# lmb-freiburg/flownet2

Measured on AMD Instinct MI355X. Metric: image-pairs/sec FlowNetC forward at 448x320, higher is better.
Workload: dtype f32

## Files before the change

### flownet2_amd/_lib.py

```python
from __future__ import annotations

import ctypes as C
import os
import re

_HERE = os.path.dirname(os.path.abspath(__file__))
SO_PATH = os.path.join(_HERE, "libflownet2_hip.so")
INCLUDE_DIR = os.path.join(_HERE, "..", "include")

_SCALARS = {"int": C.c_int, "unsigned": C.c_uint, "float": C.c_float, "size_t": C.c_size_t, "long long": C.c_longlong, "unsigned long long": C.c_ulonglong,
            "char": C.c_char}
_POINTERS = {"float": C.c_void_p, "double": C.c_void_p, "void": C.c_void_p, "unsigned char": C.c_void_p, "char": C.c_char_p, "int": C.POINTER(C.c_int),
             "unsigned": C.POINTER(C.c_uint), "size_t": C.POINTER(C.c_size_t)}
_STRUCT_NAMES = {"fn2_l1loss_params": "L1LossParams", "fn2_l1loss_scale": "L1LossScale"}
_DECLARATOR = re.compile(r"^([\w\s*]*?)(\w+)\s*(?:\[(\d+)\])?$")
_FUNCTION = re.compile(r"^([\w\s*]+?)\b(fn2_\w+)\s*\(([^()]*)\)$")


class Fn2Error(RuntimeError):

    def __init__(self, status: int, message: str):
        super().__init__(f"[fn2 status {status}] {message}")
        self.status = status


def _ctype(spec, structs, where):
    words = [w for w in spec.replace("*", " ").split() if w != "const"]
    base, stars = " ".join(words), spec.count("*")
    if stars == 0 and base in _SCALARS:
        return _SCALARS[base]
    if stars == 1 and base in structs:
        return C.POINTER(structs[base])
    if stars == 1 and base in _POINTERS:
        return _POINTERS[base]
    if stars == 2 and base in ("float", "void"):
        return C.POINTER(C.c_void_p)
    raise ValueError(f"C header: unknown type `{spec.strip()}` in `{where}`")


def _declarator(text, structs, where):
    m = _DECLARATOR.match(text.strip())
    if not m or not m.group(1).strip():
        raise ValueError(f"C header: cannot read `{text.strip()}` in `{where}`")
    t = _ctype(m.group(1), structs, where)
    return m.group(2), (t * int(m.group(3)) if m.group(3) else t), m.group(1)


def parse_header(text, structs=None):
    structs = dict(structs or {})
    functions, constants = {}, {}
    text = re.sub(r"/\*.*?\*/", " ", text, flags=re.S)
    for name, value in re.findall(r"^[ \t]*#[ \t]*define[ \t]+(FN2_\w+)[ \t]+(-?(?:0[xX][0-9a-fA-F]+|\d+))[ \t]*$", text, flags=re.M):
        constants[name] = int(value, 0)
    text = re.sub(r"^[ \t]*#.*$", " ", text, flags=re.M)

    def enum(m):
        value = -1
        for item in filter(None, (s.strip() for s in m.group(1).split(","))):
            name, _, v = (s.strip() for s in item.partition("="))
            value = int(v, 0) if v else value + 1
            constants[name] = value
        return " "
    text = re.sub(r"(?:typedef\s+)?enum\s*\w*\s*\{([^{}]*)\}\s*\w*\s*;", enum, text)

    def struct(m):
        cname, fields = m.group(1), []
        for decl in filter(None, (s.strip() for s in m.group(2).split(";"))):
            first, *more = decl.split(",")
            name, t, spec = _declarator(first, structs, "struct " + cname)
            fields.append((name, t))
            fields += [_declarator(spec + " " + other, structs, "struct " + cname)[:2] for other in more]
        pyname = _STRUCT_NAMES.get(cname) or "".join(w.capitalize() for w in cname.split("_")[1:])
        structs[cname] = type(pyname, (C.Structure,), {"_fields_": fields, "__doc__": cname, "__module__": __name__})
        return " "
    text = re.sub(r"typedef\s+struct\s+(fn2_\w+)\s*\{([^{}]*)\}\s*\w+\s*;", struct, text)

    text = re.sub(r'extern\s*"C"\s*\{|\}', " ", text)
    for stmt in filter(None, (" ".join(s.split()) for s in text.split(";"))):
        m = _FUNCTION.match(stmt)
        if not m:
            raise ValueError(f"C header: cannot read the declaration `{stmt}`")
        params = m.group(3).strip()
        args = [] if params == "void" else [_declarator(p, structs, stmt)[1] for p in params.split(",")]
        functions[m.group(2)] = (_ctype(m.group(1), structs, stmt), args)
    return functions, structs, constants


def _parse_headers():
    per_header, structs, constants = [], {}, {}
    own = {"flownet2_hip_flow_metrics.h": {}, "flownet2_hip_flow_consistency.h": {}, "flownet2_hip_flow_visualize.h": {},
           "flownet2_hip_flow_track.h": {}}
    for h in ("flownet2_hip.h", "flownet2_hip_solver.h", "flownet2_hip_corr_route.h", "flownet2_hip_conv_general.h",
              "flownet2_hip_conv_geometry.h", "flownet2_hip_conv_volume.h", "flownet2_hip_lpq_loss.h", "flownet2_hip_flow_metrics.h",
              "flownet2_hip_flow_consistency.h", "flownet2_hip_flow_visualize.h", "flownet2_hip_flow_track.h"):
        with open(os.path.join(INCLUDE_DIR, h)) as f:
            functions, structs, c = parse_header(f.read(), structs)
        per_header.append(functions)
        own.get(h, constants).update(c)
    return (per_header, structs, constants, own["flownet2_hip_flow_metrics.h"], own["flownet2_hip_flow_consistency.h"],
            own["flownet2_hip_flow_visualize.h"], own["flownet2_hip_flow_track.h"])


(_PER_HEADER, _STRUCTS, CONSTANTS, FLOW_METRICS_CONSTANTS, FLOW_CONSISTENCY_CONSTANTS, FLOW_VISUALIZE_CONSTANTS,
 FLOW_TRACK_CONSTANTS) = _parse_headers()
(EXPORTS, SOLVER_EXPORTS, CORR_ROUTE_EXPORTS, CONV_GENERAL_EXPORTS, CONV_GEOMETRY_EXPORTS, CONV_VOLUME_EXPORTS, LPQ_LOSS_EXPORTS,
 FLOW_METRICS_EXPORTS, FLOW_CONSISTENCY_EXPORTS, FLOW_VISUALIZE_EXPORTS, FLOW_TRACK_EXPORTS) = (list(f) for f in _PER_HEADER)
PROTOTYPES = {name: proto for f in _PER_HEADER[:8] for name, proto in f.items()}
FLOW_CONSISTENCY_PROTOTYPES = dict(_PER_HEADER[8])
FLOW_VISUALIZE_PROTOTYPES = dict(_PER_HEADER[9])
FLOW_TRACK_PROTOTYPES = dict(_PER_HEADER[10])
globals().update({cls.__name__: cls for cls in _STRUCTS.values()})
_HOOKS = parse_header("""
    int fn2_debug_set_correlation_impl(int impl);
    int fn2_debug_correlation_units_plan(int N, int H, int W, int policy, unsigned* out_words, int max_words);
    int fn2_debug_set_resample_generic(int on);
    int fn2_debug_set_correlation_trace(void* device_buffer);""")[0]

_lib = None


def lib():
    global _lib
    if _lib is not None:
        return _lib
    if not os.path.exists(SO_PATH):
        raise RuntimeError(
            f"{SO_PATH} not found: the HIP extension is not built. Run `python -m flownet2_amd.build` "
            "(or __graft_entry__.build()). flownet2_amd has no CPU / PyTorch fallback.")
    L = C.CDLL(SO_PATH)
    for table, required in ((PROTOTYPES, True), (FLOW_CONSISTENCY_PROTOTYPES, True), (FLOW_VISUALIZE_PROTOTYPES, True),
                            (FLOW_TRACK_PROTOTYPES, True), (_HOOKS, False)):
        for name, (restype, argtypes) in table.items():
            if not hasattr(L, name):
                if required:
                    raise RuntimeError(f"{SO_PATH} does not export {name}")
                continue
            fn = getattr(L, name)
            fn.restype, fn.argtypes = restype, argtypes
    _lib = L
    return L


def check(status: int):
    if status != 0:
        raise Fn2Error(status, lib().fn2_last_error_string().decode())


def version() -> str:
    return lib().fn2_version().decode()
```

### flownet2_amd/csrc/conv_mfma.hip

```cpp
#include "mfma_tile.hpp"

namespace fn2 {
namespace cv {

using namespace mfma;

struct Args {
  const float* in; const float* wp; const float* bias; float* out;
  int N, Cin, Hin, Win, in_ctot, in_c0;
  int Cout, Hout, Wout, out_ctot, out_c0;
  int pad;
  int nchunks;
  int ksteps;
  int tx, ty;
  int ng;
  unsigned total;
  unsigned nbig;
  float slope; int relu;
};

template <int KS_, int S_, int MW_, int NP_, int WM_, int WNX_, int WNY_, int CQ_, int P16_ = 0, int PIN_ = 0>
struct Cfg : Window<((P16_ ? 1 : 4) * WNY_ - 1) * S_ + KS_,
                    ((P16_ ? 16 : 4) * NP_ * WNX_ - 1) * S_ + KS_ + 4,
                    CQ_, WM_ * WNX_ * WNY_> {
  static constexpr int KS = KS_, S = S_, MW = MW_, NP = NP_, WM = WM_, WNX = WNX_, WNY = WNY_, CQ = CQ_, P16 = P16_;
  static constexpr int PIN = PIN_;
  static constexpr int NW = WM * WNX * WNY, THREADS = 64 * NW;
  static constexpr int PADL = 4;
  static constexpr int TW = (P16 ? 16 : 4) * NP * WNX, TH = (P16 ? 1 : 4) * WNY;
  static_assert(!P16 || (KS == 1 && S == 1), "row tiles are for 1x1 kernels");
  static_assert(Cfg::WR == (TH - 1) * S + KS && Cfg::WC == (TW - 1) * S + KS + PADL, "window of the tile");
  static constexpr int KSC = CQ * KS * KS;
  static constexpr int NBUFA = ring_depth(KSC);
  static_assert(KSC % NBUFA == 0, "ring phase must repeat per chunk");
  static_assert(2 * Cfg::BUF * 4 <= 160 * 1024, "LDS");
};

template <class K>
__device__ __forceinline__ void conv_body(const Args& a, int g, int bx, int by, int n) {
  static_assert(K::THREADS == 256, "launch bounds");
  extern __shared__ __attribute__((aligned(16))) float smem[];
  constexpr int KS = K::KS, S = K::S, MW = K::MW, NP = K::NP;
  const int tid = threadIdx.x, lane = tid & 63;
  const int wave = __builtin_amdgcn_readfirstlane(tid >> 6);
  const int wm = wave % K::WM, wnx = (wave / K::WM) % K::WNX, wny = wave / (K::WM * K::WNX);
  const int x0 = bx * K::TW, y0 = by * K::TH;

  const size_t plane = (size_t)a.Hin * a.Win;
  const __amdgpu_buffer_rsrc_t rs = nchw_rsrc(a.in, n, a.in_ctot, a.in_c0, a.Cin, plane);
  unsigned voff[K::RPW];
  window_plan<K>(voff, wave, lane, S * y0 - a.pad, S * x0 - K::PADL, a.Hin, a.Win, plane);
  const unsigned lds_base = (unsigned)(uintptr_t)(lds_ptr_t)smem;
  const unsigned chunk_bytes = 4u * 4u * K::CQ * (unsigned)plane;
  auto stage = [&](int chunk, int buf) { stage_chunk<K>(rs, voff, lds_base + 4u * (unsigned)(buf * K::BUF), wave, (unsigned)chunk * chunk_bytes); };

  const int kq = lane >> 4, p16 = lane & 15, py = K::P16 ? 0 : p16 >> 2, px = K::P16 ? p16 : p16 & 3;
  constexpr int PW = K::P16 ? 16 : 4, PH = K::P16 ? 1 : 4;
  const int bbase = kq * K::CS + (S * (PH * wny + py)) * K::RS + S * (PW * NP * wnx + px) + K::PADL - a.pad;
  using WV = typename WVec<MW>::T;
  const int cg0 = (g * K::WM + wm) * MW;
  const float* wb = a.wp + (size_t)(cg0 / 4) * a.ksteps * 256 + (cg0 % 4);
  const unsigned wlane = 16u * (unsigned)lane;

  f32x4 acc[MW][NP];
#pragma unroll
  for (int j = 0; j < MW; ++j)
#pragma unroll
    for (int p = 0; p < NP; ++p) acc[j][p] = f32x4{0.f, 0.f, 0.f, 0.f};

  constexpr int R = K::NBUFA - 1, DMA = K::NRUN / K::NW;
  static_assert(R + DMA <= 63, "vmcnt has 6 bits");
  WV wreg[K::NBUFA];
  stage(0, 0);
  if (a.nchunks > 0) {
#pragma unroll
    for (int i = 0; i < R; ++i) wreg[i] = weight_fetch<MW>(wb + (size_t)i * 256, wlane);
  }
  auto weight_step = [&](int ks0, int ks, int rest) -> WV {
    const float* wks = wb + (size_t)(ks0 + ks + R) * 256;
    if (ks + R < K::KSC) wreg[(ks + R) % K::NBUFA] = weight_fetch<MW>(wks, wlane);
    else wreg[(ks + R) % K::NBUFA] = weight_fetch_unless_last<MW>(rest, wks, wlane);
    const int left = K::KSC - 1 - ks < R ? K::KSC - 1 - ks : R;
    if (ks < R) ring_wait_either(rest, left, R + DMA);
    else if (left < R) ring_wait_either(rest, left, R);
    else ring_wait(R);
    weight_landed(wreg[ks % K::NBUFA]);
    return wreg[ks % K::NBUFA];
  };

  for (int c = 0; c < a.nchunks; ++c) {
    const int buf = c & 1;
    const int rest = a.nchunks - 1 - c;
    wait_vmcnt<R>();
    __builtin_amdgcn_s_barrier();
    if (rest) stage(c + 1, buf ^ 1);
    const float* win = smem + buf * K::BUF + bbase;
    const int ks0 = c * K::KSC;
    if constexpr (K::PIN) {
      float b[2][NP];
      auto tap_off = [](int ks) { const int cq = ks / (KS * KS), ky = (ks / KS) % KS, kx = ks % KS; return cq * 4 * K::CS + ky * K::RS + kx; };
#pragma unroll
      for (int p = 0; p < NP; ++p) b[0][p] = win[tap_off(0) + PW * S * p];
      __builtin_amdgcn_sched_barrier(0);
#pragma unroll
      for (int ks = 0; ks < K::KSC; ++ks) {
        const WV w = weight_step(ks0, ks, rest);
#pragma unroll
        for (int p = 0; p < NP; ++p) {
#pragma unroll
          for (int j = 0; j < MW; ++j) acc[j][p] = __builtin_amdgcn_mfma_f32_16x16x4f32(b[ks & 1][p], wget<MW>(w, j), acc[j][p], 0, 0, 0);
          if (ks + 1 < K::KSC) b[(ks + 1) & 1][p] = win[tap_off(ks + 1 < K::KSC ? ks + 1 : ks) + PW * S * p];
          __builtin_amdgcn_sched_barrier(0);
        }
      }
    } else {
#pragma unroll
    for (int ks = 0; ks < K::KSC; ++ks) {
      const WV w = weight_step(ks0, ks, rest);
      const int cq = ks / (KS * KS), ky = (ks / KS) % KS, kx = ks % KS;
      float b[NP];
#pragma unroll
      for (int p = 0; p < NP; ++p) b[p] = win[cq * 4 * K::CS + ky * K::RS + kx + PW * S * p];
#pragma unroll
      for (int j = 0; j < MW; ++j)
#pragma unroll
        for (int p = 0; p < NP; ++p) acc[j][p] = __builtin_amdgcn_mfma_f32_16x16x4f32(b[p], wget<MW>(w, j), acc[j][p], 0, 0, 0);
    }
    }
  }

  wait_vmcnt<0>();
  const int y = K::P16 ? y0 + wny : y0 + 4 * wny + (lane >> 4);
  if (y < a.Hout) {
#pragma unroll
    for (int j = 0; j < MW; ++j) {
      const int co = 16 * (cg0 + j) + (lane & 15);
      const float bv = a.bias ? a.bias[co] : 0.f;
      float* orow = a.out + (((size_t)n * a.out_ctot + a.out_c0 + co) * a.Hout + y) * a.Wout;
#pragma unroll
      for (int p = 0; p < NP; ++p) {
        const int x = K::P16 ? x0 + 16 * (NP * wnx + p) + 4 * (lane >> 4) : x0 + 4 * (NP * wnx + p);
        store_row4(orow, x, a.Wout, acc[j][p], bv, a.relu, a.slope);
      }
    }
  }
}

__device__ __forceinline__ void decode_tile(const Args& a, unsigned t, int& g, int& bx, int& by, int& n) {
  g = t % a.ng; t /= a.ng;
  bx = t % a.tx; t /= a.tx;
  by = t % a.ty;
  n = t / a.ty;
}

template <class K>
__global__ void __launch_bounds__(256, 2)
conv_mfma(Args a) {
  unsigned t;
  if (!xcd_task(blockIdx.x, a.total, t)) return;
  int g, bx, by, n;
  decode_tile(a, t, g, bx, by, n);
  conv_body<K>(a, g, bx, by, n);
}

template <class K>
__global__ void __launch_bounds__(256, 2)
conv_mfma_tail(Args a) {
  using KH = Cfg<K::KS, K::S, K::MW / 2, K::NP, K::WM, K::WNX, K::WNY, K::CQ, K::P16>;
  int g, bx, by, n;
  if (blockIdx.x < a.nbig) {
    const unsigned t = (blockIdx.x % 8) * (a.nbig / 8) + blockIdx.x / 8;
    decode_tile(a, t, g, bx, by, n);
    conv_body<K>(a, g, bx, by, n);
  } else {
    unsigned u;
    if (!xcd_task(blockIdx.x - a.nbig, 2 * (a.total - a.nbig), u)) return;
    decode_tile(a, a.nbig + u / 2, g, bx, by, n);
    conv_body<KH>(a, 2 * g + (int)(u & 1), bx, by, n);
  }
}

__global__ void pack_weights(const float* __restrict__ w, float* __restrict__ wp, int Cout, int Cin, int KS, int ksteps, int kalloc) {
  const long long total = (long long)((Cout + 63) / 64) * kalloc * 256;
  for (long long i = blockIdx.x * (long long)blockDim.x + threadIdx.x; i < total; i += (long long)gridDim.x * blockDim.x) {
    const int j = (int)(i & 3), lane = (int)((i >> 2) & 63);
    long long r = i >> 8;
    const int ks = (int)(r % kalloc), grp = (int)(r / kalloc);
    const int co = 64 * grp + 16 * j + (lane & 15), kq = lane >> 4;
    const int cq = ks / (KS * KS), tap = ks % (KS * KS);
    const int ci = 4 * cq + kq;
    float v = 0.f;
    if (ks < ksteps && ci < Cin && co < Cout) v = w[((size_t)co * Cin + ci) * KS * KS + tap];
    wp[i] = v;
  }
}

template <int KS> struct PackTile {
  static constexpr int T = KS * KS;
  static constexpr int QT = KS == 1 ? 8 : KS == 3 ? 3 : KS == 4 ? 2 : 1;
  static constexpr int CIL = 4 * QT, ROW = CIL * T + 1;
  static constexpr int LDS_FLOATS = 64 * ROW;
};

template <int KS, int ORDER>
__global__ void __launch_bounds__(256) pack_weights_view(const float* __restrict__ w, float* __restrict__ wp, int ksteps, int kalloc,
                                                         int src_co, int src_ci, long long s_co, long long s_ci, int flip) {
  using P = PackTile<KS>;
  constexpr int T = P::T, QT = P::QT, CIL = P::CIL, ROW = P::ROW;
  __shared__ float tile[P::LDS_FLOATS];
  const int grp = blockIdx.x, cq0 = blockIdx.y * QT;
  const int co0 = 64 * grp, ci0 = 4 * cq0;
  const int nquads = ksteps / T;
  constexpr int TOTAL = 64 * CIL * T;
  if constexpr (ORDER == 0) {
    const float* src = w + (size_t)co0 * s_co + (size_t)ci0 * T;
#pragma unroll
    for (int i = threadIdx.x; i < TOTAL; i += 256) {
      const int col = i / (CIL * T), e = i - col * (CIL * T), c = e / T;
      tile[col * ROW + e] = (co0 + col < src_co && ci0 + c < src_ci) ? src[(size_t)col * s_co + e] : 0.f;
    }
  } else if constexpr (ORDER == 1) {
    const float* src = w + (size_t)ci0 * s_ci + (size_t)co0 * T;
#pragma unroll
    for (int i = threadIdx.x; i < TOTAL; i += 256) {
      const int c = i / (64 * T), e = i - c * (64 * T), col = e / T, t = e - col * T;
      tile[col * ROW + c * T + t] = (co0 + col < src_co && ci0 + c < src_ci) ? src[(size_t)c * s_ci + e] : 0.f;
    }
  } else {
#pragma unroll
    for (int i = threadIdx.x; i < TOTAL; i += 256) {
      const int col = i / (CIL * T), e = i - col * (CIL * T), c = e / T, t = e - c * T;
      tile[col * ROW + e] = (co0 + col < src_co && ci0 + c < src_ci) ? w[(size_t)(co0 + col) * s_co + (size_t)(ci0 + c) * s_ci + t] : 0.f;
    }
  }
  __syncthreads();
  const int nq = min(QT, nquads - cq0);
  float* dst = wp + ((size_t)grp * kalloc + (size_t)cq0 * T) * 256;
  const int j = threadIdx.x & 3, lane = threadIdx.x >> 2;
  const float* trow = tile + (16 * j + (lane & 15)) * ROW + (lane >> 4) * T;
#pragma unroll
  for (int ks = 0; ks < QT * T; ++ks) {
    const int cq = ks / T, tap = ks - cq * T;
    if (cq < nq) dst[ks * 256 + threadIdx.x] = trow[4 * cq * T + (flip ? T - 1 - tap : tap)];
  }
  if (cq0 + QT >= nquads)
    for (int i = threadIdx.x; i < (kalloc - ksteps) * 256; i += 256) wp[((size_t)grp * kalloc + ksteps) * 256 + i] = 0.f;
}

template <int KS>
static void launch_pack_view(const float* w, float* wp, int Cout, int ksteps, int kalloc, int src_co, int src_ci, long long s_co, long long s_ci, int flip,
                             hipStream_t st) {
  using P = PackTile<KS>;
  const dim3 grid((unsigned)((Cout + 63) / 64), (unsigned)cdiv(ksteps / P::T, P::QT));
  if (s_ci == (long long)P::T) hipLaunchKernelGGL((pack_weights_view<KS, 0>), grid, dim3(256), 0, st, w, wp, ksteps, kalloc, src_co, src_ci, s_co, s_ci, flip);
  else if (s_co == (long long)P::T) hipLaunchKernelGGL((pack_weights_view<KS, 1>), grid, dim3(256), 0, st, w, wp, ksteps, kalloc, src_co, src_ci, s_co, s_ci, flip);
  else hipLaunchKernelGGL((pack_weights_view<KS, 2>), grid, dim3(256), 0, st, w, wp, ksteps, kalloc, src_co, src_ci, s_co, s_ci, flip);
}

constexpr int kSpare = 8;
constexpr int kChunkQuads = 2;

inline int chunk_quads(int KS) { return KS == 1 ? 8 : kChunkQuads; }
inline int ksteps_for(int Cin, int KS) { return cdiv(cdiv(Cin, 4), chunk_quads(KS)) * chunk_quads(KS) * KS * KS; }

template <class K>
static void set_geometry(Args& a) {
  if constexpr (K::P16) {
    a.Win *= a.Hin; a.Hin = 1; a.Wout *= a.Hout; a.Hout = 1;
  }
  a.tx = cdiv(a.Wout, K::TW); a.ty = cdiv(a.Hout, K::TH);
  a.ng = a.Cout / (16 * K::MW * K::WM);
  a.nchunks = cdiv(cdiv(a.Cin, 4), K::CQ);
}

inline long long tiles_of(const Args& a) { return (long long)a.N * a.tx * a.ty * a.ng; }

template <class K>
static int launch(const Args& base, hipStream_t st) {
  Args a = base;
  set_geometry<K>(a);
  a.nbig = (unsigned)tiles_of(a);
  return launch_tiles<&conv_mfma<K>>(a, tiles_of(a), K::THREADS, (int)(sizeof(float) * 2 * K::BUF), "conv_mfma", "conv_mfma_forward", st);
}

inline unsigned whole_rounds(long long tiles) { return (unsigned)(tiles / 256 * 256); }

template <class K>
static int launch_tail(const Args& base, hipStream_t st) {
  if constexpr (K::MW < 2) {
    return fail(FN2_ERR_UNSUPPORTED, "conv_mfma: variant has no split tail");
  } else {
    Args a = base;
    set_geometry<K>(a);
    if (tiles_of(a) > 0x1fffff00ll) return fail(FN2_ERR_UNSUPPORTED, "conv_mfma: grid too large");
    a.total = (unsigned)tiles_of(a); a.nbig = whole_rounds(a.total);
    const unsigned nsm = 2 * (a.total - a.nbig);
    const unsigned grid = a.nbig + 8 * ((nsm + 7) / 8);
    constexpr size_t lds = sizeof(float) * 2 * K::BUF;
    set_dynamic_lds_once<&conv_mfma_tail<K>>((int)lds);
    hipLaunchKernelGGL((conv_mfma_tail<K>), dim3(grid), dim3(K::THREADS), lds, st, a);
    return check_launch("conv_mfma_forward");
  }
}

struct Variant {
  int ks, s, mw, np, wm, wnx, wny, p16;
  int (*fn)(const Args&, hipStream_t);
  int (*fn_tail)(const Args&, hipStream_t);
};

#define FN2_CV_LIST(X) \
   \
  X(1, 1, 2, 7, 2, 2, 1, 8, 1) X(1, 1, 2, 7, 2, 1, 2, 8, 1) X(1, 1, 4, 7, 1, 2, 2, 8, 0) X(1, 1, 4, 7, 1, 1, 4, 8, 0) X(1, 1, 2, 6, 2, 2, 1, 8, 1) \
  X(1, 1, 2, 4, 2, 2, 1, 8, 1) X(1, 1, 2, 7, 1, 2, 2, 8, 0) X(1, 1, 2, 7, 1, 4, 1, 8, 0) X(1, 1, 2, 4, 1, 2, 2, 8, 0) X(1, 1, 4, 4, 1, 2, 2, 8, 0) \
   \
  X(3, 1, 2, 7, 2, 2, 1, 2, 1) X(3, 1, 2, 7, 2, 1, 2, 2, 1) X(3, 1, 4, 7, 1, 2, 2, 2, 0) X(3, 1, 4, 7, 1, 1, 4, 2, 0) \
  X(3, 1, 2, 6, 2, 2, 1, 2, 1) X(3, 1, 4, 6, 1, 2, 2, 2, 0) X(3, 1, 4, 4, 1, 2, 2, 2, 0) X(3, 1, 2, 4, 2, 2, 1, 2, 1) \
   \
  X(3, 2, 2, 7, 2, 1, 2, 2, 1) X(3, 2, 4, 7, 1, 1, 4, 2, 0) X(3, 2, 2, 6, 2, 2, 1, 2, 1) X(3, 2, 4, 6, 1, 2, 2, 2, 0) X(3, 2, 2, 4, 2, 2, 1, 2, 1) \
   \
  X(4, 2, 2, 7, 2, 2, 1, 2, 1) X(4, 2, 2, 7, 2, 1, 2, 2, 1) X(4, 2, 4, 7, 1, 2, 2, 2, 0) X(4, 2, 2, 6, 2, 2, 1, 2, 1) X(4, 2, 4, 4, 1, 2, 2, 2, 0) X(4, 2, 2, 4, 2, 2, 1, 2, 1) \
   \
  X(5, 2, 2, 7, 2, 2, 1, 1, 1) X(5, 2, 2, 7, 2, 1, 2, 1, 1) X(5, 2, 4, 7, 1, 2, 2, 1, 0) X(5, 2, 4, 7, 1, 1, 4, 1, 0) \
  X(5, 2, 2, 6, 2, 2, 1, 1, 1) X(5, 2, 4, 6, 1, 2, 2, 1, 0) X(5, 2, 4, 4, 1, 2, 2, 1, 0) \
   \
  X(7, 2, 2, 6, 2, 2, 1, 1, 1) X(7, 2, 2, 7, 2, 2, 1, 1, 1) X(7, 2, 4, 4, 1, 2, 2, 1, 0) X(7, 2, 4, 6, 1, 2, 2, 1, 0) X(7, 2, 2, 4, 2, 2, 1, 1, 1)

template <class K, int TAIL> struct TailFn { static constexpr int (*fn)(const Args&, hipStream_t) = nullptr; };
template <class K> struct TailFn<K, 1> { static constexpr int (*fn)(const Args&, hipStream_t) = &launch_tail<K>; };

#define FN2_CV_ROW(KS, S, MW, NP, WM, WNX, WNY, CQ, TAIL) \
  {KS, S, MW, NP, WM, WNX, WNY, 0, &launch<Cfg<KS, S, MW, NP, WM, WNX, WNY, CQ>>, TailFn<Cfg<KS, S, MW, NP, WM, WNX, WNY, CQ>, TAIL>::fn},
#define FN2_CV_ROW16(MW, NP, WM, WNX, WNY, TAIL) \
  {1, 1, MW, NP, WM, WNX, WNY, 1, &launch<Cfg<1, 1, MW, NP, WM, WNX, WNY, 8, 1>>, TailFn<Cfg<1, 1, MW, NP, WM, WNX, WNY, 8, 1>, TAIL>::fn},
#define FN2_CV_PIN(KS, S, MW, NP, WM, WNX, WNY, CQ, P16, TAIL) \
  {KS, S, MW, NP, WM, WNX, WNY, P16, &launch<Cfg<KS, S, MW, NP, WM, WNX, WNY, CQ, P16, 1>>, TailFn<Cfg<KS, S, MW, NP, WM, WNX, WNY, CQ, P16, 1>, TAIL>::fn},
static const Variant kVariants[] = {FN2_CV_LIST(FN2_CV_ROW)
  FN2_CV_ROW16(2, 7, 2, 2, 1, 1) FN2_CV_ROW16(2, 7, 4, 1, 1, 1) FN2_CV_ROW16(4, 7, 1, 4, 1, 0) FN2_CV_ROW16(4, 7, 2, 2, 1, 0) FN2_CV_ROW16(2, 5, 2, 2, 1, 1)
  FN2_CV_ROW16(2, 4, 2, 2, 1, 1) FN2_CV_ROW16(2, 7, 1, 4, 1, 0) FN2_CV_ROW16(2, 5, 1, 4, 1, 0) FN2_CV_ROW16(4, 5, 1, 4, 1, 0) FN2_CV_ROW16(2, 4, 1, 4, 1, 0)
  FN2_CV_ROW16(4, 5, 2, 2, 1, 0) FN2_CV_ROW16(4, 4, 2, 2, 1, 0)
  FN2_CV_ROW16(2, 9, 4, 1, 1, 1) FN2_CV_ROW16(2, 9, 2, 2, 1, 1) FN2_CV_ROW16(2, 3, 2, 2, 1, 1) FN2_CV_ROW16(4, 3, 1, 4, 1, 0)
  FN2_CV_ROW16(4, 9, 4, 1, 1, 0) FN2_CV_ROW16(4, 9, 2, 2, 1, 0) FN2_CV_ROW16(4, 7, 4, 1, 1, 0)
  FN2_CV_PIN(5, 2, 2, 7, 2, 2, 1, 1, 0, 1) FN2_CV_PIN(5, 2, 2, 7, 2, 1, 2, 1, 0, 1)
  FN2_CV_PIN(1, 1, 4, 9, 4, 1, 1, 8, 1, 0) FN2_CV_PIN(1, 1, 2, 9, 4, 1, 1, 8, 1, 1) FN2_CV_PIN(1, 1, 2, 5, 2, 2, 1, 8, 1, 1) FN2_CV_PIN(1, 1, 4, 7, 4, 1, 1, 8, 1, 0)
  FN2_CV_PIN(1, 1, 2, 7, 2, 2, 1, 8, 1, 1) FN2_CV_PIN(1, 1, 2, 3, 2, 2, 1, 8, 1, 1)
  FN2_CV_PIN(3, 1, 2, 7, 2, 2, 1, 2, 0, 1) FN2_CV_PIN(3, 1, 2, 6, 2, 2, 1, 2, 0, 1) FN2_CV_PIN(3, 2, 2, 7, 2, 1, 2, 2, 0, 1) FN2_CV_PIN(3, 2, 2, 6, 2, 2, 1, 2, 0, 1)
  FN2_CV_PIN(4, 2, 2, 7, 2, 2, 1, 2, 0, 1) FN2_CV_PIN(4, 2, 2, 6, 2, 2, 1, 2, 0, 1) FN2_CV_PIN(5, 2, 2, 6, 2, 2, 1, 1, 0, 1)
  FN2_CV_PIN(7, 2, 2, 6, 2, 2, 1, 1, 0, 1) FN2_CV_PIN(7, 2, 4, 6, 1, 2, 2, 1, 0, 0)};
constexpr int kNumVariants = sizeof(kVariants) / sizeof(kVariants[0]);

int g_forced_variant = -1;

static double variant_cost(const Variant& v, const Args& a, bool tail) {
  const int tw = (v.p16 ? 16 : 4) * v.np * v.wnx, th = (v.p16 ? 1 : 4) * v.wny;
  const long long wgs = v.p16 ? (long long)a.N * cdiv(a.Wout * a.Hout, tw) * (a.Cout / (16 * v.mw * v.wm))
                              : (long long)a.N * cdiv(a.Wout, tw) * cdiv(a.Hout, th) * (a.Cout / (16 * v.mw * v.wm));
  double rounds = (double)((wgs + 255) / 256);
  if (tail) {
    const long long r = wgs % 256;
    if (wgs < 256 || r == 0 || r > 128) return 1e30;
    rounds = (double)(wgs / 256) + 0.5 * 1.12;
  }
  const double eff = 1.0 / (1.0 + 0.08 * (4.0 / v.mw - 1.0) + 0.02 * (7.0 / v.np - 1.0));
  return rounds * v.mw * v.np / eff;
}

static bool variant_applies(const Variant& v, const Args& a, int KS, int S) {
  if (!v.p16 && a.Win % 4 != 0) return false;
  return v.ks == KS && v.s == S && a.Cout % (16 * v.mw * v.wm) == 0;
}

}
}

using namespace fn2;

FN2_API size_t fn2_conv_mfma_packed_floats(int Cout, int Cin, int kernel) {
  if (Cout <= 0 || Cout % 32 != 0 || Cin <= 0 || kernel <= 0) return 0;
  return (size_t)((Cout + 63) / 64) * (cv::ksteps_for(Cin, kernel) + cv::kSpare) * 256;
}

FN2_API int fn2_conv_mfma_pack_weights_view(const float* weight, float* packed, int Cout, int Cin, int kernel, int src_cout, int src_cin,
                                            long long stride_cout, long long stride_cin, int flip, void* stream);

FN2_API int fn2_conv_mfma_pack_weights(const float* weight, float* packed, int Cout, int Cin, int kernel, void* stream) {
  if (!weight || !packed) return fail(FN2_ERR_INVALID_ARG, "conv_mfma_pack_weights: null blob");
  if (Cout <= 0 || Cout % 32 != 0 || Cin <= 0 || (kernel != 1 && kernel != 3 && kernel != 4 && kernel != 5 && kernel != 7))
    return fail(FN2_ERR_UNSUPPORTED, "conv_mfma_pack_weights: needs Cout %% 32 == 0 and kernel_size 1, 3, 4, 5 or 7 (got Cout %d, kernel %d)", Cout, kernel);
  return fn2_conv_mfma_pack_weights_view(weight, packed, Cout, Cin, kernel, Cout, Cin, (long long)Cin * kernel * kernel, (long long)kernel * kernel, 0, stream);
}

FN2_API int fn2_conv_mfma_pack_weights_view(const float* weight, float* packed, int Cout, int Cin, int kernel, int src_cout, int src_cin,
                                            long long stride_cout, long long stride_cin, int flip, void* stream) {
  if (!weight || !packed) return fail(FN2_ERR_INVALID_ARG, "conv_mfma_pack_weights_view: null blob");
  if (Cout <= 0 || Cout % 32 != 0 || Cin <= 0 || (kernel != 1 && kernel != 3 && kernel != 4 && kernel != 5 && kernel != 7))
    return fail(FN2_ERR_UNSUPPORTED, "conv_mfma_pack_weights_view: needs Cout %% 32 == 0 and kernel_size 1, 3, 4, 5 or 7 (got Cout %d, kernel %d)", Cout, kernel);
  if (src_cout < 1 || src_cout > Cout || src_cin < 1 || src_cin > Cin || stride_cout < 1 || stride_cin < 1)
    return fail(FN2_ERR_INVALID_ARG, "conv_mfma_pack_weights_view: bad source view (%d of %d, %d of %d channels, strides %lld / %lld)", src_cout, Cout,
                src_cin, Cin, stride_cout, stride_cin);
  const int ksteps = cv::ksteps_for(Cin, kernel), kalloc = ksteps + cv::kSpare;
  hipStream_t st = as_stream(stream);
  switch (kernel) {
    case 1: cv::launch_pack_view<1>(weight, packed, Cout, ksteps, kalloc, src_cout, src_cin, stride_cout, stride_cin, flip ? 1 : 0, st); break;
    case 3: cv::launch_pack_view<3>(weight, packed, Cout, ksteps, kalloc, src_cout, src_cin, stride_cout, stride_cin, flip ? 1 : 0, st); break;
    case 4: cv::launch_pack_view<4>(weight, packed, Cout, ksteps, kalloc, src_cout, src_cin, stride_cout, stride_cin, flip ? 1 : 0, st); break;
    case 5: cv::launch_pack_view<5>(weight, packed, Cout, ksteps, kalloc, src_cout, src_cin, stride_cout, stride_cin, flip ? 1 : 0, st); break;
    default: cv::launch_pack_view<7>(weight, packed, Cout, ksteps, kalloc, src_cout, src_cin, stride_cout, stride_cin, flip ? 1 : 0, st); break;
  }
  return check_launch("conv_mfma_pack_weights_view");
}

FN2_API int fn2_conv_mfma_supported(int Cin, int Hin, int Win, int Cout, int kernel, int stride, int pad) {
  if (Cin <= 0 || Hin <= 0 || Win <= 0 || Cout <= 0 || Cout % 32 != 0) return 0;
  if (kernel == 1 ? ((long long)Hin * Win) % 4 != 0 : Win % 4 != 0) return 0;
  if (!((kernel == 1 && stride == 1) || (kernel == 3 && (stride == 1 || stride == 2)) || (kernel == 4 && stride == 2) || (kernel == 5 && stride == 2) || (kernel == 7 && stride == 2))) return 0;
  if (pad < 0 || pad > 4 || pad > kernel - 1) return 0;
  if ((long long)Cin * Hin * Win >= (1ll << 28)) return 0;
  const int Hout = (Hin + 2 * pad - kernel) / stride + 1, Wout = (Win + 2 * pad - kernel) / stride + 1;
  if (Hout < 1 || Wout < 1) return 0;
  cv::Args a{};
  a.Win = Win; a.Cout = Cout;
  for (int i = 0; i < cv::kNumVariants; ++i)
    if (cv::variant_applies(cv::kVariants[i], a, kernel, stride)) return 1;
  return 0;
}

FN2_API int fn2_debug_set_conv_variant(int v) { cv::g_forced_variant = v; return FN2_OK; }
FN2_API int fn2_conv_mfma_num_variants(void) { return cv::kNumVariants; }

FN2_API int fn2_conv_mfma_forward(const float* bottom, const float* packed_weight, const float* bias, float* top,
                                  int N, int Cin, int Hin, int Win, int bottom_channels, int bottom_c0,
                                  int Cout, int top_channels, int top_c0, int kernel, int stride, int pad,
                                  int relu, float negative_slope, void* stream) {
  if (N < 0) return fail(FN2_ERR_INVALID_ARG, "conv_mfma: bad batch");
  if (N == 0) return FN2_OK;
  if (const int rc = mfma::check_conv_args("conv_mfma", bottom, packed_weight, top, Cin, bottom_channels, bottom_c0, Cout, top_channels, top_c0, [&] {
        return fn2_conv_mfma_supported(Cin, Hin, Win, Cout, kernel, stride, pad) ? FN2_OK
            : fail(FN2_ERR_UNSUPPORTED, "conv_mfma: unsupported geometry (Cin %d, %dx%d, Cout %d, k %d s %d p %d)", Cin, Hin, Win, Cout, kernel, stride, pad);
      }))
    return rc;
  cv::Args a{};
  a.in = bottom; a.wp = packed_weight; a.bias = bias; a.out = top;
  a.N = N; a.Cin = Cin; a.Hin = Hin; a.Win = Win; a.in_ctot = bottom_channels; a.in_c0 = bottom_c0;
  a.Cout = Cout; a.Hout = (Hin + 2 * pad - kernel) / stride + 1; a.Wout = (Win + 2 * pad - kernel) / stride + 1;
  a.out_ctot = top_channels; a.out_c0 = top_c0; a.pad = pad;
  a.ksteps = cv::ksteps_for(Cin, kernel) + cv::kSpare;
  a.slope = negative_slope; a.relu = relu;
  hipStream_t st = as_stream(stream);
  static TuneCache cache("conv_mfma", cv::kNumVariants);
  const TuneKey key{N, Cin, Hin, Win, Cout, kernel, stride, pad, bottom_channels == Cin, top_channels == Cout};
  mfma::Pick p;
  if (const int rc = mfma::pick_variant(p, "conv_mfma", cv::g_forced_variant, cv::kNumVariants, true, cache, key, st,
                                        [&](int i) { return cv::variant_applies(cv::kVariants[i], a, kernel, stride); },
                                        [&](int i, bool tail) { return cv::variant_cost(cv::kVariants[i], a, tail); },
                                        [&](int i, bool tail) { return tail ? cv::kVariants[i].fn_tail(a, st) : cv::kVariants[i].fn(a, st); },
                                        [&](int i) { return cv::kVariants[i].fn_tail != nullptr; }))
    return rc;
  return p.tail ? cv::kVariants[p.variant].fn_tail(a, st) : cv::kVariants[p.variant].fn(a, st);
}
```

### flownet2_amd/csrc/flow_head.hip

```cpp
#include "fn2_common.hpp"

namespace fn2 {

constexpr int kHeadPix = 64;

template <int G>
__global__ void __launch_bounds__(kHeadPix* G) conv3x3_c2_taps(const float* __restrict__ in, const float* __restrict__ w,
                                                                float* __restrict__ P, int N, int C, int H, int W, int nsplit) {
  __shared__ float red[G][18][kHeadPix];
  const int lane_pix = threadIdx.x % kHeadPix;
  const int grp = __builtin_amdgcn_readfirstlane(threadIdx.x / kHeadPix);
  const size_t plane = (size_t)H * W;
  const long long total = (long long)N * H * W;
  const long long p = (long long)blockIdx.x * kHeadPix + lane_pix;
  const bool live = p < total;
  const int n = live ? (int)(p / (long long)plane) : 0;
  const unsigned pix = live ? (unsigned)(p - (long long)n * plane) : 0u;
  const float* src = in + (size_t)n * C * plane + pix;
  float a[18];
#pragma unroll
  for (int k = 0; k < 18; ++k) a[k] = 0.f;
  const int ngroups = G * nsplit;
  const int c_per = (C + ngroups - 1) / ngroups;
  const int c_lo = min(C, ((int)blockIdx.y * G + grp) * c_per), c_hi = min(C, c_lo + c_per);
  for (int c = c_lo; c < c_hi; c += 8) {
    float v[8];
#pragma unroll
    for (int cc = 0; cc < 8; ++cc) v[cc] = (c + cc < c_hi) ? src[(size_t)(c + cc) * plane] : 0.f;
    __builtin_amdgcn_sched_barrier(0);
#pragma unroll
    for (int cc = 0; cc < 8; ++cc) {
      if (c + cc < c_hi) {
        const float* w0 = w + (size_t)(c + cc) * 9;
        const float* w1 = w + ((size_t)C + c + cc) * 9;
#pragma unroll
        for (int t = 0; t < 9; ++t) {
          a[t] = fmaf(w0[t], v[cc], a[t]);
          a[9 + t] = fmaf(w1[t], v[cc], a[9 + t]);
        }
      }
    }
  }
#pragma unroll
  for (int k = 0; k < 18; ++k) red[grp][k][lane_pix] = a[k];
  __syncthreads();
  if (live) {
    float* dst = P + ((size_t)blockIdx.y * N + n) * 18 * plane + pix;
    for (int k = grp; k < 18; k += G) {
      float sacc = 0.f;
#pragma unroll
      for (int g = 0; g < G; ++g) sacc += red[g][k][lane_pix];
      dst[(size_t)k * plane] = sacc;
    }
  }
}

template <int NSPLIT>
__global__ void __launch_bounds__(256) conv3x3_c2_gather(const float* __restrict__ P, const float* __restrict__ bias,
                                                          float* __restrict__ out, int N, int H, int W) {
  const unsigned plane = (unsigned)H * W;
  const unsigned pix = blockIdx.x * 256u + threadIdx.x;
  if (pix >= plane) return;
  const int y = pix / W, x = pix - y * W;
  const unsigned no = blockIdx.y;
  const unsigned n = no >> 1, o = no & 1;
  float v[NSPLIT][9];
#pragma unroll
  for (int sp = 0; sp < NSPLIT; ++sp) {
    const float* Pn = P + (((size_t)sp * N + n) * 18 + o * 9) * plane;
#pragma unroll
    for (int dy = 0; dy < 3; ++dy)
#pragma unroll
      for (int dx = 0; dx < 3; ++dx) {
        const int yy = y + dy - 1, xx = x + dx - 1;
        const bool ok = yy >= 0 && yy < H && xx >= 0 && xx < W;
        v[sp][dy * 3 + dx] = ok ? Pn[(size_t)(dy * 3 + dx) * plane + (unsigned)yy * W + xx] : 0.f;
      }
  }
  float sacc = bias ? bias[o] : 0.f;
#pragma unroll
  for (int sp = 0; sp < NSPLIT; ++sp)
#pragma unroll
    for (int t = 0; t < 9; ++t) sacc += v[sp][t];
  out[(size_t)no * plane + pix] = sacc;
}

__global__ void __launch_bounds__(256) deconv4x4s2_c2(const float* __restrict__ in, const float* __restrict__ w,
                                                       const float* __restrict__ bias, float* __restrict__ out,
                                                       int N, int H, int W, int out_ctot, int out_c0) {
  const int Ho = 2 * H, Wo = 2 * W;
  const long long total = (long long)N * Ho * Wo;
  for (long long idx = blockIdx.x * (long long)blockDim.x + threadIdx.x; idx < total; idx += (long long)gridDim.x * blockDim.x) {
    const int X = (int)(idx % Wo), Y = (int)((idx / Wo) % Ho), n = (int)(idx / ((long long)Wo * Ho));
    float a0 = bias ? bias[0] : 0.f, a1 = bias ? bias[1] : 0.f;
#pragma unroll
    for (int ty = 0; ty < 2; ++ty) {
      const int ky = ((Y + 1) & 1) + 2 * ty;
      const int iy = (Y + 1 - ky) / 2;
      if (Y + 1 - ky < 0 || iy >= H) continue;
#pragma unroll
      for (int tx = 0; tx < 2; ++tx) {
        const int kx = ((X + 1) & 1) + 2 * tx;
        const int ix = (X + 1 - kx) / 2;
        if (X + 1 - kx < 0 || ix >= W) continue;
#pragma unroll
        for (int c = 0; c < 2; ++c) {
          const float v = in[(((size_t)n * 2 + c) * H + iy) * W + ix];
          a0 = fmaf(w[((c * 2 + 0) * 4 + ky) * 4 + kx], v, a0);
          a1 = fmaf(w[((c * 2 + 1) * 4 + ky) * 4 + kx], v, a1);
        }
      }
    }
    out[(((size_t)n * out_ctot + out_c0 + 0) * Ho + Y) * Wo + X] = a0;
    out[(((size_t)n * out_ctot + out_c0 + 1) * Ho + Y) * Wo + X] = a1;
  }
}

}

using namespace fn2;

constexpr int kHeadG = 16;

static int head_splits(int N, int C, int H, int W) {
  const long long blocks = ((long long)order_batch(N) * H * W + kHeadPix - 1) / kHeadPix;
  int nsplit = 1;
  while (nsplit < 8 && blocks * kHeadG * nsplit < 4096 && C >= 8 * kHeadG * nsplit * 2) nsplit *= 2;
  return nsplit;
}

FN2_API size_t fn2_predict_flow_conv_workspace_bytes(int N, int C, int H, int W) {
  if (N < 1 || C < 1 || H < 1 || W < 1) return 0;
  return sizeof(float) * (size_t)head_splits(N, C, H, W) * N * 18 * H * W;
}

FN2_API int fn2_predict_flow_conv_forward(const float* in, const float* weight, const float* bias, float* out,
                                          int N, int C, int H, int W, void* workspace, size_t workspace_bytes, void* stream) {
  if (N < 0 || C < 1 || H < 1 || W < 1) return fail(FN2_ERR_INVALID_ARG, "predict_flow_conv: bad shape [%d,%d,%d,%d]", N, C, H, W);
  if (N == 0) return FN2_OK;
  if (!in || !weight || !out) return fail(FN2_ERR_INVALID_ARG, "predict_flow_conv: NULL blob pointer");
  if ((long long)H * W >= (1ll << 31) || 2ll * N > 65535) return fail(FN2_ERR_UNSUPPORTED, "predict_flow_conv: blob too large");
  const size_t need = fn2_predict_flow_conv_workspace_bytes(N, C, H, W);
  if (!workspace || workspace_bytes < need) return fail(FN2_ERR_WORKSPACE, "predict_flow_conv: workspace too small (%zu < %zu)", workspace_bytes, need);
  const long long total = (long long)N * H * W;
  const unsigned blocks = (unsigned)((total + kHeadPix - 1) / kHeadPix);
  const int nsplit = head_splits(N, C, H, W);
  hipStream_t st = as_stream(stream);
  float* P = reinterpret_cast<float*>(workspace);
  hipLaunchKernelGGL(conv3x3_c2_taps<kHeadG>, dim3(blocks, nsplit), dim3(kHeadPix * kHeadG), 0, st, in, weight, P, N, C, H, W, nsplit);
  const dim3 g2(((unsigned)H * W + 255) / 256, 2 * N);
  switch (nsplit) {
    case 1: hipLaunchKernelGGL(conv3x3_c2_gather<1>, g2, dim3(256), 0, st, P, bias, out, N, H, W); break;
    case 2: hipLaunchKernelGGL(conv3x3_c2_gather<2>, g2, dim3(256), 0, st, P, bias, out, N, H, W); break;
    case 4: hipLaunchKernelGGL(conv3x3_c2_gather<4>, g2, dim3(256), 0, st, P, bias, out, N, H, W); break;
    default: hipLaunchKernelGGL(conv3x3_c2_gather<8>, g2, dim3(256), 0, st, P, bias, out, N, H, W); break;
  }
  return check_launch("predict_flow_conv_forward");
}

FN2_API int fn2_upsample_flow_deconv_forward(const float* in, const float* weight, const float* bias, float* out,
                                             int N, int H, int W, void* stream) {
  if (N < 0 || H < 1 || W < 1) return fail(FN2_ERR_INVALID_ARG, "upsample_flow_deconv: bad shape");
  if (N == 0) return FN2_OK;
  if (!in || !weight || !out) return fail(FN2_ERR_INVALID_ARG, "upsample_flow_deconv: NULL blob pointer");
  const long long total = (long long)N * 4 * H * W;
  hipLaunchKernelGGL(deconv4x4s2_c2, dim3(blocks_for(total, 256, 4096)), dim3(256), 0, as_stream(stream), in, weight, bias, out, N, H, W, 2, 0);
  return check_launch("upsample_flow_deconv_forward");
}

FN2_API int fn2_upsample_flow_deconv_forward_into(const float* in, const float* weight, const float* bias, float* top,
                                                  int N, int H, int W, int top_channels, int top_c0, void* stream) {
  if (N < 0 || H < 1 || W < 1) return fail(FN2_ERR_INVALID_ARG, "upsample_flow_deconv: bad shape");
  if (top_c0 < 0 || top_c0 + 2 > top_channels) return fail(FN2_ERR_INVALID_ARG, "upsample_flow_deconv: channel slice outside the blob");
  if (N == 0) return FN2_OK;
  if (!in || !weight || !top) return fail(FN2_ERR_INVALID_ARG, "upsample_flow_deconv: NULL blob pointer");
  const long long total = (long long)N * 4 * H * W;
  hipLaunchKernelGGL(deconv4x4s2_c2, dim3(blocks_for(total, 256, 4096)), dim3(256), 0, as_stream(stream), in, weight, bias, top, N, H, W, top_channels, top_c0);
  return check_launch("upsample_flow_deconv_forward_into");
}
```

### flownet2_amd/csrc/mfma_tile.hpp

```cpp
#pragma once

#include "autotune.hpp"
#include "fn2_common.hpp"

namespace fn2 {
namespace mfma {

using f32x4 = __attribute__((ext_vector_type(4))) float;
using f32x2 = __attribute__((ext_vector_type(2))) float;
using lds_ptr_t = __attribute__((address_space(3))) void*;

constexpr int cdiv(int a, int b) { return (a + b - 1) / b; }
constexpr int up_mod(int v, int r, int m) { return v + ((r - v % m) + m) % m; }

constexpr unsigned kOOB = 0x7ffffff0u;
constexpr int kRsrcWord3 = 0x00020000;

template <int N>
__device__ __forceinline__ void wait_vmcnt() {
  asm volatile("s_waitcnt vmcnt(%0)" ::"n"(N) : "memory");
}

__device__ __forceinline__ __amdgpu_buffer_rsrc_t nchw_rsrc(const float* blob, int n, int ctot, int c0, int C, size_t plane) {
  return __builtin_amdgcn_make_buffer_rsrc(const_cast<float*>(blob + ((size_t)n * ctot + c0) * plane), 0, (unsigned)(4u * C * plane), kRsrcWord3);
}

template <int MW> struct WVec;
template <> struct WVec<1> { using T = float; };
template <> struct WVec<2> { using T = f32x2; };
template <> struct WVec<4> { using T = f32x4; };

template <int MW>
__device__ __forceinline__ float wget(const typename WVec<MW>::T& v, int j) {
  if constexpr (MW == 1) return v; else return v[j];
}

template <int WR_, int WC_, int CQ_, int NW_>
struct Window {
  static constexpr int WR = WR_, WC = WC_;
  static constexpr int RS = up_mod(cdiv(WC, 4) * 4, 4, 16);
  static constexpr int CS = up_mod(WR * RS, 16, 32);
  static constexpr int SLOTS_C = CS / 4;
  static constexpr int SLOTS = 4 * CQ_ * SLOTS_C;
  static constexpr int NRUN = cdiv(SLOTS, 64);
  static constexpr int RPW = cdiv(NRUN, NW_);
  static constexpr int BUF = NRUN * 256;
};

constexpr int ring_depth(int KSC) { return (KSC % 6 == 0) ? 6 : (KSC % 5 == 0) ? 5 : (KSC % 7 == 0) ? 7 : (KSC % 4 == 0) ? 4 : 3; }

template <class K>
__device__ __forceinline__ void window_plan(unsigned (&voff)[K::RPW], int wave, int lane, int y_first, int x_first, int Hin, int Win, size_t plane) {
#pragma unroll
  for (int i = 0; i < K::RPW; ++i) {
    const int s = (i * K::NW + wave) * 64 + lane;
    voff[i] = kOOB;
    if (s < K::SLOTS) {
      const int c = s / K::SLOTS_C, rem = s % K::SLOTS_C;
      const int row = rem / (K::RS / 4), gq = rem % (K::RS / 4);
      const int yi = y_first + row, xi = x_first + 4 * gq;
      if (row < K::WR && 4 * gq < K::WC && yi >= 0 && yi < Hin && xi >= 0 && xi < Win)
        voff[i] = 4u * (unsigned)(c * plane + (size_t)yi * Win + xi);
    }
  }
}

template <class K>
__device__ __forceinline__ void stage_chunk(__amdgpu_buffer_rsrc_t rs, const unsigned (&voff)[K::RPW], unsigned dst, int wave, unsigned soff) {
#pragma unroll
  for (int i = 0; i < K::RPW; ++i) {
    const int r = i * K::NW + wave;
    if (r < K::NRUN)
      __builtin_amdgcn_raw_ptr_buffer_load_lds(rs, (lds_ptr_t)(uintptr_t)(dst + 1024u * (unsigned)r), 16, voff[i], soff, 0, 0);
  }
}

template <class K>
struct ChunkStage {
  const __amdgpu_buffer_rsrc_t& rs; const unsigned (&voff)[K::RPW]; const unsigned& chunk_bytes; const unsigned& dst; const int& wave;
  __device__ void operator()(int chunk) const {
    unsigned vc[K::RPW];
#pragma unroll
    for (int i = 0; i < K::RPW; ++i) vc[i] = voff[i] == kOOB ? kOOB : voff[i] + (unsigned)chunk * chunk_bytes;
    stage_chunk<K>(rs, vc, dst, wave, 0u);
  }
};

__device__ __forceinline__ const float* weight_lane(const float* wp, int cg0, int ksteps, int lane) {
  return wp + ((size_t)(cg0 / 4) * ksteps * 64 + lane) * 4 + (cg0 % 4);
}

template <int MW>
__device__ __forceinline__ typename WVec<MW>::T weight_load(const float* wl, int ks) {
  return *reinterpret_cast<const typename WVec<MW>::T*>(wl + (size_t)ks * 256);
}

template <int MW>
__device__ __forceinline__ typename WVec<MW>::T weight_fetch(const float* base, unsigned lane_bytes) {
  typename WVec<MW>::T w;
  if constexpr (MW == 1) asm volatile("global_load_dword %0, %1, %2" : "=v"(w) : "v"(lane_bytes), "s"(base));
  else if constexpr (MW == 2) asm volatile("global_load_dwordx2 %0, %1, %2" : "=v"(w) : "v"(lane_bytes), "s"(base));
  else asm volatile("global_load_dwordx4 %0, %1, %2" : "=v"(w) : "v"(lane_bytes), "s"(base));
  return w;
}

template <class T>
__device__ __forceinline__ void weight_landed(T& w) { asm volatile("" : "+v"(w)); }

constexpr int vmcnt_clamp(int n) { return n < 63 ? n : 63; }

__device__ __forceinline__ void ring_wait(int n) { asm volatile("s_waitcnt vmcnt(%0)" ::"i"(vmcnt_clamp(n))); }

__device__ __forceinline__ void ring_wait_either(int rest, int n_last, int n_else) {
  asm volatile(
      "s_cmp_eq_u32 %0, 0\n\t"
      "s_cbranch_scc1 .Lrwt_%=\n\t"
      "s_waitcnt vmcnt(%2)\n\t"
      "s_branch .Lrwe_%=\n"
      ".Lrwt_%=:\n\t"
      "s_waitcnt vmcnt(%1)\n"
      ".Lrwe_%=:"
      :
      : "s"(rest), "i"(vmcnt_clamp(n_last)), "i"(vmcnt_clamp(n_else))
      : "scc");
}

template <int MW>
__device__ __forceinline__ typename WVec<MW>::T weight_fetch_unless_last(int rest, const float* base, unsigned lane_bytes) {
  typename WVec<MW>::T w;
#define FN2_FETCH_UNLESS(INSN) \
  asm volatile("s_cmp_eq_u32 %3, 0\n\ts_cbranch_scc1 .Lwfs_%=\n\t" INSN " %0, %1, %2\n.Lwfs_%=:" : "=v"(w) : "v"(lane_bytes), "s"(base), "s"(rest) : "scc")
  if constexpr (MW == 1) FN2_FETCH_UNLESS("global_load_dword");
  else if constexpr (MW == 2) FN2_FETCH_UNLESS("global_load_dwordx2");
  else FN2_FETCH_UNLESS("global_load_dwordx4");
#undef FN2_FETCH_UNLESS
  return w;
}

__device__ __forceinline__ bool xcd_task(unsigned block, unsigned total, unsigned& task) {
  const unsigned per_xcd = (total + 7) / 8;
  task = (block % 8) * per_xcd + block / 8;
  return !(block / 8 >= per_xcd || task >= total);
}

__device__ __forceinline__ f32x4 bias_relu4(f32x4 v, float bias, int relu, float slope) {
#pragma unroll
  for (int r = 0; r < 4; ++r) {
    float s = v[r] + bias;
    if (relu) s = s > 0.f ? s : s * slope;
    v[r] = s;
  }
  return v;
}

__device__ __forceinline__ void store4(float* orow, int x, int Wout, f32x4 v) {
  if (x + 3 < Wout) *reinterpret_cast<f32x4*>(orow + x) = v;
  else {
#pragma unroll
    for (int r = 0; r < 4; ++r) if (x + r < Wout) orow[x + r] = v[r];
  }
}

__device__ __forceinline__ void store_row4(float* orow, int x, int Wout, f32x4 v, float bias, int relu, float slope) {
  store4(orow, x, Wout, bias_relu4(v, bias, relu, slope));
}

template <auto Kernel>
inline void set_dynamic_lds_once(int bytes) {
  static bool attr_set = false;
  if (!attr_set) {
    (void)hipFuncSetAttribute(reinterpret_cast<const void*>(Kernel), hipFuncAttributeMaxDynamicSharedMemorySize, bytes);
    attr_set = true;
  }
}

template <auto Kernel, class Args>
int launch_tiles(Args& a, long long tiles, int threads, int lds_bytes, const char* what, const char* checked, hipStream_t st) {
  if (tiles > 0x3fffff00ll) return fail(FN2_ERR_UNSUPPORTED, "%s: grid too large", what);
  a.total = (unsigned)tiles;
  set_dynamic_lds_once<Kernel>(lds_bytes);
  hipLaunchKernelGGL(Kernel, dim3(8 * ((a.total + 7) / 8)), dim3(threads), lds_bytes, st, a);
  return check_launch(checked);
}

template <class Geometry>
int check_conv_args(const char* what, const float* bottom, const float* packed, const float* top, int Cin, int bottom_channels, int bottom_c0,
                    int Cout, int top_channels, int top_c0, Geometry geometry) {
  if (!bottom || !packed || !top) return fail(FN2_ERR_INVALID_ARG, "%s: null blob", what);
  if (const int rc = geometry()) return rc;
  if (bottom_c0 < 0 || bottom_c0 + Cin > bottom_channels || top_c0 < 0 || top_c0 + Cout > top_channels)
    return fail(FN2_ERR_INVALID_ARG, "%s: channel slice outside the blob", what);
  if (((reinterpret_cast<uintptr_t>(bottom) | reinterpret_cast<uintptr_t>(top) | reinterpret_cast<uintptr_t>(packed)) & 15) != 0)
    return fail(FN2_ERR_UNSUPPORTED, "%s: blobs must be 16-byte aligned", what);
  return FN2_OK;
}

struct Pick { int variant = -1; bool tail = false; };

template <class Applies, class Cost, class Run, class HasTail>
int pick_variant(Pick& p, const char* what, int forced, int nvariants, bool split_tail, TuneCache& cache, const TuneKey& key, hipStream_t st,
                 Applies applies, Cost cost, Run run, HasTail has_tail) {
  p = Pick{};
  if (forced >= 0) {
    p.tail = split_tail && forced >= 1000;
    p.variant = split_tail ? forced % 1000 : forced;
    if (p.variant >= nvariants || !applies(p.variant) || (p.tail && !has_tail(p.variant)))
      return fail(FN2_ERR_UNSUPPORTED, "%s: forced variant %d does not apply", what, forced);
    return FN2_OK;
  }
  int picked = -1;
  if (autotune_enabled(st)) {
    auto usable = [&](int c) -> bool {
      const int i = split_tail ? c / 2 : c;
      return applies(i) && (!(split_tail && (c & 1)) || (has_tail(i) && cost(i, true) < 1e29));
    };
    picked = autotune_pick(cache, key, split_tail ? 2 * nvariants : nvariants, st, [&](int c) -> int {
      return usable(c) ? run(split_tail ? c / 2 : c, split_tail && (c & 1)) : FN2_ERR_UNSUPPORTED;
    }, usable);
  }
  if (picked >= 0) {
    p.variant = split_tail ? picked / 2 : picked;
    p.tail = split_tail && (picked & 1);
  } else {
    double bc = 0;
    for (int i = 0; i < nvariants; ++i) {
      if (!applies(i)) continue;
      for (int t = 0; t < (split_tail && has_tail(i) ? 2 : 1); ++t) {
        const double c = cost(i, t == 1);
        if (p.variant < 0 || c < bc) { p.variant = i; bc = c; p.tail = t == 1; }
      }
    }
  }
  if (p.variant < 0) return fail(FN2_ERR_UNSUPPORTED, "%s: no kernel variant for this geometry", what);
  return FN2_OK;
}

}
}
```

### flownet2_amd/functional.py

```python
from __future__ import annotations

import collections
import os

import torch

from . import ops


_BATCH_INVARIANT = [False]


def set_batch_invariant(on: bool = True):
    _BATCH_INVARIANT[0] = bool(on)
    ops.set_batch_invariant(bool(on))


def batch_invariant() -> bool:
    return _BATCH_INVARIANT[0]


LIBRARY_FALLBACKS = [0]


# ... 214 lines not shown

def downsample(x, top_height, top_width):
    with torch.no_grad():
        return ops.downsample_forward(x.detach().contiguous(), top_height, top_width)


def downsample_ahead(x, sizes):
    with torch.no_grad():
        x = x.detach().contiguous()
        many = (lambda: ops.downsample_forward_multi(x, sizes)) if ops.downsample_multi_supported(x.shape, sizes) and x.shape[0] > 0 else \
            (lambda: [ops.downsample_forward(x, h, w) for h, w in sizes])
        if not x.is_cuda:
            return [ops.downsample_forward(x, h, w) for h, w in sizes], None
        main = torch.cuda.current_stream(x.device)
        side = _WGRAD_SIDE["streams"].get(x.device)
        if side is None:
            side = _WGRAD_SIDE["streams"][x.device] = torch.cuda.Stream(device=x.device)
        side.wait_stream(main)
        with torch.cuda.stream(side):
            outs = many()
            ev = torch.cuda.Event()
            ev.record(side)
        x.record_stream(side)
        for t in outs:
            t.record_stream(main)
        return outs, ev


def wait_ahead(event):
    if event is not None:
        torch.cuda.current_stream().wait_event(event)


class _ChannelNorm(torch.autograd.Function):
    @staticmethod
    def forward(ctx, x):
        top = ops.channel_norm_forward(x)
        ctx.save_for_backward(x, top)
        return top

    @staticmethod
    def backward(ctx, g):
        x, top = ctx.saved_tensors
        return ops.channel_norm_backward(x, top, g.contiguous())


def channel_norm(x):
    return _ChannelNorm.apply(x.contiguous())


class _L1Loss(torch.autograd.Function):
    @staticmethod
    def forward(ctx, b0, b1, params):
        loss, ws = ops.l1loss_forward(params, b0, b1)
        ctx.params, ctx.ws = params, ws
        ctx.save_for_backward(b0, b1)
        return loss

    @staticmethod
    def backward(ctx, g):
        b0, b1 = ctx.saved_tensors
        d0, d1 = ops.l1loss_backward(ctx.params, b0, b1, float(g), ctx.ws)
        return (d0 if ctx.needs_input_grad[0] else None), (d1 if (b1 is not None and ctx.needs_input_grad[1]) else None), None


def l1_loss(b0, b1=None, l2_per_location=False, l2_prescale_by_channels=False, normalize_by_num_entries=False,
            epsilon=1e-2, plateau=0.0):
    p = ops.l1_params(l2_per_location, l2_prescale_by_channels, normalize_by_num_entries, epsilon, plateau)
    return _L1Loss.apply(b0.contiguous(), b1.contiguous() if b1 is not None else None, p)


class _L1LossMulti(torch.autograd.Function):

    @staticmethod
    def forward(ctx, params, weights, n, *blobs):
        b0, b1 = list(blobs[:n]), list(blobs[n:])
        total, losses, ws = ops.l1loss_forward_multi(params, b0, b1, weights)
        ctx.params, ctx.weights, ctx.n, ctx.ws = params, weights, n, ws
        ctx.save_for_backward(*blobs)
        ctx.mark_non_differentiable(losses)
        return total, losses

    @staticmethod
    def backward(ctx, g, _g_losses):
        n = ctx.n
        blobs = ctx.saved_tensors
        b0, b1 = list(blobs[:n]), list(blobs[n:])
        need1 = any(ctx.needs_input_grad[3 + n:])
        d0, d1 = ops.l1loss_backward_multi(ctx.params, b0, b1, ctx.weights, g.contiguous(), ctx.ws, need1=need1)
        grads = [d if ctx.needs_input_grad[3 + k] else None for k, d in enumerate(d0)]
        grads += [d if ctx.needs_input_grad[3 + n + k] else None for k, d in enumerate(d1)]
        return (None, None, None) + tuple(grads)


def l1_loss_multi(preds, targets, weights, l2_per_location=False, l2_prescale_by_channels=False, normalize_by_num_entries=False,
                  epsilon=1e-2, plateau=0.0):
    p = ops.l1_params(l2_per_location, l2_prescale_by_channels, normalize_by_num_entries, epsilon, plateau)
    blobs = [t.contiguous() for t in preds] + [t.contiguous() for t in targets]
    return _L1LossMulti.apply(p, tuple(float(w) for w in weights), len(preds), *blobs)


class _LpqLoss(torch.autograd.Function):
    @staticmethod
    def forward(ctx, b0, b1, params):
        loss, ws = ops.lpq_loss_forward(params, b0, b1)
        ctx.params, ctx.ws = params, ws
        ctx.save_for_backward(b0, b1)
        return loss

    @staticmethod
    def backward(ctx, g):
        b0, b1 = ctx.saved_tensors
        d0, d1 = ops.lpq_loss_backward(ctx.params, b0, b1, float(g), ctx.ws)
        return (d0 if ctx.needs_input_grad[0] else None), (d1 if (b1 is not None and ctx.needs_input_grad[1]) else None), None


def lpq_loss(b0, b1=None, p=1.0, q=1.0, p_epsilon=0.0, q_epsilon=1e-2, l2_prescale_by_channels=False, normalize_by_num_entries=False):
    params = ops.lpq_params(p, q, p_epsilon, q_epsilon, l2_prescale_by_channels, normalize_by_num_entries)
    return _LpqLoss.apply(b0.contiguous(), b1.contiguous() if b1 is not None else None, params)


class _LpqLossMulti(torch.autograd.Function):

    @staticmethod
    def forward(ctx, params, weights, n, *blobs):
        b0, b1 = list(blobs[:n]), list(blobs[n:])
        total, losses, ws = ops.lpq_loss_forward_multi(params, b0, b1, weights)
        ctx.params, ctx.weights, ctx.n, ctx.ws = params, weights, n, ws
        ctx.save_for_backward(*blobs)
        ctx.mark_non_differentiable(losses)
        return total, losses

    @staticmethod
    def backward(ctx, g, _g_losses):
        n = ctx.n
        blobs = ctx.saved_tensors
        b0, b1 = list(blobs[:n]), list(blobs[n:])
        need1 = any(ctx.needs_input_grad[3 + n:])
        d0, d1 = ops.lpq_loss_backward_multi(ctx.params, b0, b1, ctx.weights, g.contiguous(), ctx.ws, need1=need1)
        grads = [d if ctx.needs_input_grad[3 + k] else None for k, d in enumerate(d0)]
        grads += [d if ctx.needs_input_grad[3 + n + k] else None for k, d in enumerate(d1)]
        return (None, None, None) + tuple(grads)


def lpq_loss_multi(preds, targets, weights, p=1.0, q=1.0, p_epsilon=0.0, q_epsilon=1e-2, l2_prescale_by_channels=False,
                   normalize_by_num_entries=False):
    params = ops.lpq_params(p, q, p_epsilon, q_epsilon, l2_prescale_by_channels, normalize_by_num_entries)
    blobs = [t.contiguous() for t in preds] + [t.contiguous() for t in targets]
    return _LpqLossMulti.apply(params, tuple(float(w) for w in weights), len(preds), *blobs)


def flow_metrics(pred, gt, valid=None, occ=None, *, outlier=(3.0, 0.05), bands=(10.0, 40.0), epe_map=False):
    from .evaluate import FlowMetrics
    if torch.is_grad_enabled() and any(t is not None and t.requires_grad for t in (pred, gt, valid, occ)):
        raise RuntimeError("flow_metrics is not differentiable: detach the inputs or call it under torch.no_grad() (the training loss is "
                           "l1_loss / lpq_loss)")
    results, emap = ops.flow_metrics(pred, gt, valid, occ, outlier=outlier, bands=bands, epe_map=epe_map)
    return FlowMetrics(results[:-1].cpu().numpy(), epe_map=emap)


def flow_consistency(fw, bw, *, alpha=(0.01, 0.5), beta=(0.01, 0.002), flags=False, err=False, warped=False):
    from .evaluate import FlowConsistency
    if torch.is_grad_enabled() and any(isinstance(t, torch.Tensor) and t.requires_grad for t in (fw, bw)):
        raise RuntimeError("flow_consistency is not differentiable: detach the inputs or call it under torch.no_grad()")
    results, occ, fl, er, wa = ops.flow_consistency(fw, bw, alpha=alpha, beta=beta, flags=flags, err=err, warped=warped)
    rows = results[:, :-1].cpu().numpy()
    return FlowConsistency(rows[0], rows[1], occ=occ, flags=fl, err=er, warped=wa, alpha=alpha, beta=beta)


def _no_grad_inputs(what, tensors):
    if torch.is_grad_enabled() and any(isinstance(t, torch.Tensor) and t.requires_grad for t in tensors):
        raise RuntimeError(f"{what} is not differentiable: detach the inputs or call it under torch.no_grad()")


def flow_track_grid(N, H, W, cell=1, device=None):
    P = -(-int(H) // int(cell)) * -(-int(W) // int(cell))
    device = torch.device("cuda", torch.cuda.current_device()) if device is None else device
    points = torch.zeros((int(N), 2, P), dtype=torch.float32, device=device)
    state = torch.ones((int(N), P), dtype=torch.uint8, device=device)
    ops.flow_track_reseed(points, state, (H, W), cell, born=False)
    return points


def flow_track_reseed(points, state, size, cell):
    _no_grad_inputs("flow_track_reseed", (points,))
    return ops.flow_track_reseed(points, state, size, cell, born=True)


def flow_track(fw, bw, points=None, state=None, stop=None, stop_mask=None, alpha=(0.01, 0.5), tracks=True):
    from .evaluate import CONSISTENCY_FLAGS, FlowTracks
    _no_grad_inputs("flow_track", (fw, bw, points))
    if isinstance(fw, torch.Tensor) and fw.dim() == 4:
        fw = fw.unsqueeze(1)
    if isinstance(bw, torch.Tensor) and bw.dim() == 4:
        bw = bw.unsqueeze(1)
    if isinstance(stop, torch.Tensor) and stop.dim() == 4:
        stop = stop.unsqueeze(1)
    if not isinstance(fw, torch.Tensor) or fw.dim() != 5:
        raise ValueError("flow_track: fw must be [N,T,2,H,W] or [N,2,H,W]")
    N, T, _, H, W = fw.shape
    if points is None:
        ops._chk(fw, "fw", 5)
        points = flow_track_grid(N, H, W, 1, device=fw.device)
    elif isinstance(points, torch.Tensor) and points.dim() == 4:
        points = points.reshape(points.shape[0], points.shape[1], -1)
    mask = CONSISTENCY_FLAGS["BOUNDARY"] if stop_mask is None else int(stop_mask)
    results, tr, p_out, s_out, st = ops.flow_track(fw, bw, points, state=state, stop=stop, stop_mask=mask, alpha=alpha, tracks=tracks)
    return FlowTracks(results[:-1].cpu().numpy(), tracks=tr, points=p_out, state=s_out, steps=st, start=points.contiguous(), size=(H, W), alpha=alpha)


def flow_to_color(flow, max_flow=None, norm="sample"):
    _no_grad_inputs("flow_to_color", (flow,))
    if norm not in ("sample", "batch"):
        raise ValueError(f"flow_to_color: norm must be 'sample' or 'batch', got {norm!r}")
    return ops.flow_color(flow, norm="fixed" if max_flow is not None else norm, max_flow=max_flow)[0]


def flow_error_map(pred, gt, valid=None, occ=None, abs_thresh=3.0, rel_thresh=0.05):
    _no_grad_inputs("flow_error_map", (pred, gt, valid, occ))
    return ops.flow_error_map(pred, gt, valid, occ, abs_thresh=abs_thresh, rel_thresh=rel_thresh)


def add_loss_flags(ap):
    ap.add_argument("--loss", choices=("l1", "lpq"), default="l1", help="l1: L1Loss{l2_per_location} (the default); lpq: LpqLoss with --lpq-p / --lpq-q")
    ap.add_argument("--lpq-p", type=float, nargs="+", default=[2.0], metavar="P", help="p of every episode (one value: constant)")
    ap.add_argument("--lpq-q", type=float, nargs="+", default=[0.2], metavar="Q", help="q of every episode")
    ap.add_argument("--lpq-starts", type=int, nargs="+", default=[], metavar="ITER", help="iteration at which each episode starts (the first is 0)")
    ap.add_argument("--lpq-p-epsilon", type=float, default=0.0)
    ap.add_argument("--lpq-q-epsilon", type=float, default=1e-2)


def loss_schedule(args):
    from .lpq_schedule import LpqSchedule
    return LpqSchedule(args.lpq_starts, args.lpq_p, args.lpq_q) if args.loss == "lpq" else None


class _PredictFlow(torch.autograd.Function):

    @staticmethod
    def forward(ctx, x, weight, bias):
        ctx.save_for_backward(x, weight)
        ctx.has_bias = bias is not None
        return ops.predict_flow_conv_forward(x.contiguous(), weight.contiguous(), bias)

    @staticmethod
    def backward(ctx, g):
        x, w = ctx.saved_tensors
        blob, c0 = _channel_slice(x)
        g = g.contiguous()
        need_x, need_w, need_b = ctx.needs_input_grad[0], ctx.needs_input_grad[1], ctx.has_bias and ctx.needs_input_grad[2]
        side = _wgrad_side_stream(g, x, w) if (need_w or need_b) and need_x else None
        if side is None:
            return ops.predict_flow_conv_backward((blob, c0, x.shape[1]), w, g, need_x, need_w, need_b)
        dx, _, _ = ops.predict_flow_conv_backward((blob, c0, x.shape[1]), w, g, True, False, False)
        main = torch.cuda.current_stream(g.device)
        side.wait_stream(main)
        with torch.cuda.stream(side):
            _, dw, db = ops.predict_flow_conv_backward((blob, c0, x.shape[1]), w, g, False, need_w, need_b)
        for t in (g, blob):
            t.record_stream(side)
        for t in (dw, db):
            if t is not None:
                t.record_stream(main)
        if dw is not None:
            _SIDE_PENDING.append((w, dw.data_ptr()))
        return dx, dw, db


class _UpsampleFlow(torch.autograd.Function):

    @staticmethod
    def forward(ctx, x, weight, bias, into=None):
        ctx.save_for_backward(x, weight)
        ctx.has_bias = bias is not None
        if into is None:
            return ops.upsample_flow_deconv_forward(x.contiguous(), weight.contiguous(), bias)
        ops.upsample_flow_deconv_forward(x.contiguous(), weight.contiguous(), bias, out=into[0], out_c0=into[1])
        return into[0][:, into[1]:into[1] + 2]

    @staticmethod
    def backward(ctx, g):
        x, w = ctx.saved_tensors
        dx, dw, db = ops.upsample_flow_deconv_backward(x.contiguous(), w, g.contiguous(), ctx.needs_input_grad[0], ctx.needs_input_grad[1],
                                                       ctx.has_bias and ctx.needs_input_grad[2])
        return dx, dw, db, None


def predict_flow_conv(x, weight, bias=None):
    run = lambda xx, ww, bb: ops.predict_flow_conv_forward(xx.contiguous(), ww.contiguous(), bb)
    if _needs_grad(x, weight, bias):
        if ops.predict_flow_conv_backward_supported(x.shape[0], x.shape[1], x.shape[2], x.shape[3]):
            return _PredictFlow.apply(x, weight, bias)
        return _OwnForwardConv.apply(x, weight, bias, run, 1, 1, 0.0, False, False)
    return run(x, weight, bias)


def upsample_flow_deconv(x, weight, bias=None, out=None, out_c0=0):
    if out is not None and not _needs_grad(x, weight, bias):
        return ops.upsample_flow_deconv_forward(x.contiguous(), weight.contiguous(), bias, out=out, out_c0=out_c0)
    run = lambda xx, ww, bb: ops.upsample_flow_deconv_forward(xx.contiguous(), ww.contiguous(), bb)
    if _needs_grad(x, weight, bias):
        return _UpsampleFlow.apply(x, weight, bias, None if out is None else (out, out_c0))
    return run(x, weight, bias)


class _BiasLeakyReLU(torch.autograd.Function):

    @staticmethod
    def forward(ctx, y, bias, negative_slope):
        ctx.mark_dirty(y)
        ops.bias_leaky_relu_(y, bias, negative_slope)
        ctx.slope = negative_slope
        ctx.has_bias = bias is not None
        ctx.save_for_backward(y)
        return y

    @staticmethod
    def backward(ctx, g):
        (y,) = ctx.saved_tensors
        d, db = ops.bias_leaky_relu_backward(y, g.contiguous(), ctx.slope, ctx.has_bias and ctx.needs_input_grad[1])
        return d, db, None


def conv_bias_leaky_relu(y, bias, negative_slope=0.1):
    if not y.is_contiguous():
        if bias is not None:
            y = y + bias.view(1, -1, 1, 1)
        return torch.nn.functional.leaky_relu(y, negative_slope)
    if torch.is_grad_enabled() and (y.requires_grad or (bias is not None and bias.requires_grad)):
        return _BiasLeakyReLU.apply(y, bias, negative_slope)
    return ops.bias_leaky_relu_(y, bias, negative_slope)


def invalidate_weight_caches():
    _bump_weight_generation()
    _PACKED_T.clear()


_WEIGHT_GENERATION = [0]


def weight_generation() -> int:
    return _WEIGHT_GENERATION[0]


def _bump_weight_generation(*_a, **_k):
    _WEIGHT_GENERATION[0] += 1


try:
    from torch.optim.optimizer import register_optimizer_step_post_hook as _reg_step_hook
    _reg_step_hook(_bump_weight_generation)
    _HAVE_STEP_HOOK = True
except Exception:
    _HAVE_STEP_HOOK = False


def _cached(cache, key, w, make):
    import weakref
    if w.requires_grad and (not _HAVE_STEP_HOOK or (w.is_cuda and torch.cuda.is_current_stream_capturing())):
        cache.pop(key, None)
        return make()
    gen = _WEIGHT_GENERATION[0] if w.requires_grad else -1
    hit = cache.get(key)
    if hit is None or hit[0]() is not w or hit[1] != w._version or hit[3] != gen:
        hit = (weakref.ref(w, lambda _r, k=key: cache.pop(k, None)), w._version, make(), gen)
        cache[key] = hit
    return hit[2]


_ROUTE_FORCE = [False]


def set_route_force(on: bool = True):
    _ROUTE_FORCE[0] = bool(on)


ArithSwitch = collections.namedtuple("ArithSwitch", "key env setter getter what of report covers")
ARITH_SWITCHES = (
    ArithSwitch("conv", "FN2_CONV_ARITH", "set_conv_arithmetic", "conv_arithmetic", "conv", "convolution forward", "convolution forward",
                "split-bf16 on the direct 5x5 / 2 layers"),
    ArithSwitch("deconv", "FN2_DECONV_ARITH", "set_deconv_arithmetic", "deconv_arithmetic", "deconv", "deconvolution forward", "deconvolution forward",
                "split-bf16 in the GEMM of the 4x4 / 2 layers"),
    ArithSwitch("wino", "FN2_WINO_ARITH", "set_winograd_arithmetic", "winograd_arithmetic", "winograd", "Winograd 3x3 forward", "winograd forward",
                "split-bf16 on the 3x3 / 1 layers with Cout % 64 == 0"),
    ArithSwitch("corr", "FN2_CORR_ARITH", "set_correlation_arithmetic", "correlation_arithmetic", "correlation", "correlation forward", "correlation forward",
                "split-bf16 in the FlowNetC correlation (same fp64 bound as the exact kernel; measured times: profiles/corr_bf16x3_bench.md)"),
    ArithSwitch("dgrad", "FN2_DGRAD_ARITH", "set_conv_backward_arithmetic", "conv_backward_arithmetic", "conv backward", "convolution data gradient",
                "data-gradient", "split-bf16 on the 5x5 / 2 layers"),
    ArithSwitch("wgrad", "FN2_WGRAD_ARITH", "set_conv_weight_gradient_arithmetic", "conv_weight_gradient_arithmetic", "conv weight gradient",
                "convolution weight gradient", "weight-gradient", "split-bf16 on the 5x5 / 2 layers"),
)
_CONV_ARITHMETICS = ("fp32", "bf16x3")
_ARITH_SWITCH = {s.key: s for s in ARITH_SWITCHES}
_ARITH = {s.key: "fp32" for s in ARITH_SWITCHES}


def _set_arithmetic(key: str, name: str):
    if name not in _CONV_ARITHMETICS:
        raise ValueError("%s arithmetic must be one of %s, got %r" % (_ARITH_SWITCH[key].what, ", ".join(_CONV_ARITHMETICS), name))
    _ARITH[key] = name


def arithmetic(key: str) -> str:
    return _ARITH[key]


def _bf16x3(key: str) -> bool:
    return _ARITH[key] == "bf16x3"


for _s in ARITH_SWITCHES:
    if os.environ.get(_s.env):
        _set_arithmetic(_s.key, os.environ[_s.env])


def set_conv_arithmetic(name: str = "fp32"):
    _set_arithmetic("conv", name)


def conv_arithmetic() -> str:
    return arithmetic("conv")


def set_deconv_arithmetic(name: str = "fp32"):
    _set_arithmetic("deconv", name)


def deconv_arithmetic() -> str:
    return arithmetic("deconv")


def set_winograd_arithmetic(name: str = "fp32"):
    _set_arithmetic("wino", name)


def winograd_arithmetic() -> str:
    return arithmetic("wino")


get_winograd_arithmetic = winograd_arithmetic


def set_conv_backward_arithmetic(name: str):
    _set_arithmetic("dgrad", name)


def conv_backward_arithmetic() -> str:
    return arithmetic("dgrad")


def set_conv_weight_gradient_arithmetic(name: str):
    _set_arithmetic("wgrad", name)


def conv_weight_gradient_arithmetic() -> str:
    return arithmetic("wgrad")


def set_correlation_arithmetic(name: str = "fp32"):
    _set_arithmetic("corr", name)


def correlation_arithmetic() -> str:
    return arithmetic("corr")


def arithmetic_flags(keys=None):
    return ["--%s-arith" % s.key for s in ARITH_SWITCHES if keys is None or s.key in keys]


def add_arithmetic_flags(ap, keys, notes=None):
    for key in keys:
        s = _ARITH_SWITCH[key]
        text = "arithmetic of the %s (default: $%s, else fp32); bf16x3: %s%s" % (s.of, s.env, s.covers, (notes or {}).get(key, ""))
        ap.add_argument("--%s-arith" % key, choices=list(_CONV_ARITHMETICS), default=None, help=text.replace("%", "%%"))


def apply_arithmetic_flags(args, keys):
    for key in keys:
        name = getattr(args, "%s_arith" % key)
        if name:
            _set_arithmetic(key, name)


def print_arithmetics(keys):
    for key in keys:
        print("%s arithmetic: %s" % (_ARITH_SWITCH[key].report, _ARITH[key]))


def _channel_slice(x):
    if x.is_contiguous():
        return x, 0
    b = x._base
    if (b is not None and b.dim() == 4 and b.is_contiguous() and x.dim() == 4 and x.stride() == b.stride() and x.shape[0] == b.shape[0]
            and x.shape[2:] == b.shape[2:]):
        plane = b.shape[2] * b.shape[3]
        off = x.storage_offset() - b.storage_offset()
        if off % plane == 0 and 0 <= off // plane and off // plane + x.shape[1] <= b.shape[1]:
            return b, off // plane
    return x.contiguous(), 0


class _OwnForwardConv(torch.autograd.Function):

    @staticmethod
    def forward(ctx, x, weight, bias, runner, stride, pad, negative_slope, act, transposed, into=None, relu_chain=None):
        if into is None:
            y = runner(x, weight, bias)
        else:
            runner(x, weight, bias, into[0], into[1])
            co = weight.shape[1] if transposed else weight.shape[0]
            y = into[0][:, into[1]:into[1] + co]
        ctx.cfg = (stride, pad, negative_slope, act, bias is not None, transposed)
        ctx.into = into
        ctx.relu_chain, ctx.chain_cell = (int(relu_chain[0]), relu_chain[1]) if relu_chain else (0, None)
        if ctx.relu_chain & 1:
            ctx.chain_cell["armed"] = True
        elif ctx.relu_chain & 2 and not ctx.chain_cell.get("armed"):
            raise RuntimeError("relu_chain: the layer in front of this one is not a chain producer (it would undo its ReLU twice)")
        ctx.save_for_backward(x, weight, (into[0] if into is not None else y) if act else None)
        return y

    @staticmethod
    def backward(ctx, g):
        x, w, y = ctx.saved_tensors
        stride, pad, slope, act, has_bias, transposed = ctx.cfg
        if act and ctx.into is not None:
            y = (y, ctx.into[1], w.shape[1] if transposed else w.shape[0])
        premasked = False
        if ctx.relu_chain & 1:
            if not ctx.chain_cell.get("masked"):
                raise RuntimeError("relu_chain: the consumer of this layer did not fold the ReLU derivative into its data gradient")
            ctx.chain_cell["masked"] = False
            premasked = True
        gx, gw, db = conv_backward(x, w, y if act else None, g, stride, pad, slope, transposed, bool(ctx.needs_input_grad[0]),
                                   bool(ctx.needs_input_grad[1]), has_bias and ctx.needs_input_grad[2], premasked=premasked,
                                   mask_bottom=(ctx.chain_cell["slope"] if (ctx.relu_chain & 2) else None))
        if ctx.relu_chain & 2:
            ctx.chain_cell["masked"] = True
        return (gx, gw, db) + (None,) * (len(ctx.needs_input_grad) - 3)


_GRAD_SLOT = [None]


def set_grad_slots(fn=None):
    _GRAD_SLOT[0] = fn


def _grad_slot(w):
    fn = _GRAD_SLOT[0]
    if fn is None or w.grad is not None:
        return None
    return fn(w)


_WGRAD_SIDE = {"pixels": 0, "streams": {}}
_SIDE_TASK = [-1]
_SIDE_PENDING = []


def set_wgrad_side_stream(max_pixels: int = 0):
    _WGRAD_SIDE["pixels"] = int(max_pixels)


def side_stream_for_collective(device):
    if not _WGRAD_SIDE["pixels"]:
        return None
    st = _WGRAD_SIDE["streams"].get(device)
    if st is None:
        return None
    st.wait_stream(torch.cuda.current_stream(device))
    return st


def _wgrad_side_stream(d, x, w):
    if not _WGRAD_SIDE["pixels"] or not d.is_cuda or w.grad is not None or max(d.shape[2] * d.shape[3], x.shape[2] * x.shape[3]) > _WGRAD_SIDE["pixels"]:
        return None
    task = torch._C._current_graph_task_id()
    if task < 0:
        return None
    if task != _SIDE_TASK[0]:
        if _SIDE_PENDING:
            _SIDE_PENDING.clear()
            for dev, st in _WGRAD_SIDE["streams"].items():
                torch.cuda.current_stream(dev).wait_stream(st)
        torch.autograd.Variable._execution_engine.queue_callback(join_side_streams)
        _SIDE_TASK[0] = task
    st = _WGRAD_SIDE["streams"].get(d.device)
    if st is None:
        st = _WGRAD_SIDE["streams"][d.device] = torch.cuda.Stream(device=d.device)
    return st


def join_side_streams():
    _SIDE_TASK[0] = -1
    if not _SIDE_PENDING:
        return
    for dev, st in _WGRAD_SIDE["streams"].items():
        torch.cuda.current_stream(dev).wait_stream(st)
    pending = list(_SIDE_PENDING)
    _SIDE_PENDING.clear()
    if _GRAD_SLOT[0] is not None:
        return
    for w, ptr in pending:
# ... 217 lines not shown
```

### flownet2_amd/graph_backend.py

```python
from __future__ import annotations

import contextlib
import types

import torch.nn.functional as F

NEG_SLOPE = 0.1

_LISTENERS = []


@contextlib.contextmanager
def listening(fn):
    _LISTENERS.append(fn)
    try:
        yield fn
    finally:
        _LISTENERS.remove(fn)


def _declines(*args, **kwargs):
    return None


class GraphBackend:
    FORWARDED = ("correlation", "resample", "flow_warp", "channel_norm", "downsample", "l1_loss", "scale_shift", "resample_slices",
                 "flow_warp_slices", "channel_norm_slices", "l1_loss_multi", "downsample_ahead", "wait_ahead", "lpq_loss", "lpq_loss_multi")

    def __init__(self, obj):
        get = lambda name: getattr(obj, name, None)
        self.obj = obj
        for name in self.FORWARDED:
            if get(name) is not None:
                setattr(self, name, get(name))
        self.own_conv, self.own_deconv = get("conv_mfma_relu") or _declines, get("deconv_relu") or _declines
        self.own_correlation_relu_into = get("correlation_relu_into") or _declines
        self._predict, self._upsample = get("predict_flow_conv"), get("upsample_flow_deconv")
        self._bias_act = get("conv_bias_leaky_relu")
        self._conv2d = get("lib_conv2d") or (lambda x, w, b, s, p: F.conv2d(x, w, b, stride=s, padding=p))
        self._deconv2d = get("lib_conv_transpose2d") or (lambda x, w, b, s, p: F.conv_transpose2d(x, w, b, stride=s, padding=p))
        self._act = get("leaky_relu") or (lambda y, slope, name: F.leaky_relu(y, slope))
        self.conv_route_name, self.relu_chain_supported = get("conv_route_name"), get("relu_chain_supported")
        self.writes_slices = self.own_conv is not _declines
        self.fuses_correlation = self.own_correlation_relu_into is not _declines
        self.has_slices = get("resample_slices") is not None
        self.has_scale_shift = get("scale_shift") is not None
        self.trains_in_place = get("conv_backward") is not None
        self.has_stem_chain = self.trains_in_place and self.conv_route_name is not None and self.relu_chain_supported is not None
        self.has_multi_loss = get("l1_loss_multi") is not None
        self.has_multi_lpq_loss = get("lpq_loss_multi") is not None
        self.targets_ahead = get("downsample_ahead") is not None

    def __getattr__(self, name):
        if name in self.FORWARDED:
            return getattr(self.obj, name)
        raise AttributeError(name)

    def _ran(self, name, y, **info):
        for fn in list(_LISTENERS):
            fn(name, y, dict(info, backend=self))

    def wrote(self, kind, name, y, out, out_c0, channels, x, w=None, stride=1, pad=0):
        if _LISTENERS:
            self._ran(name, y if y.requires_grad else out[:, out_c0:out_c0 + channels], kind=kind, act=True, x=x, w=w, stride=stride, pad=pad,
                      own=True, into=True)

    def conv_wb(self, x, w, b, stride, pad, act=True, slope=NEG_SLOPE, name=None, relu_chain=None):
        y = self.own_conv(x, w, b, stride, pad, slope, act, relu_chain=relu_chain)
        own = y is not None
        if not own:
            if relu_chain is not None:
                raise RuntimeError("relu_chain: no own kernel takes this layer (its consumer was told the stem kernel would)")
            if act and self._bias_act is not None:
                y = self._bias_act(self._conv2d(x, w, None, stride, pad), b, slope)
            else:
                y = self._conv2d(x, w, b, stride, pad)
                if act:
                    y = self._act(y, slope, name)
        if _LISTENERS:
            self._ran(name, y, kind="conv", act=act, x=x, w=w, stride=stride, pad=pad, own=own, into=False)
        return y

    def conv(self, x, P, name, stride, pad, act=True, relu_chain=None):
        return self.conv_wb(x, P[name + ".w"], P[name + ".b"], stride, pad, act, NEG_SLOPE, name, relu_chain)

    def deconv_wb(self, x, w, b, act=True, slope=NEG_SLOPE, name=None):
        y = self.own_deconv(x, w, b, slope, act)
        own = y is not None
        if not own:
            if act and self._bias_act is not None:
                y = self._bias_act(self._deconv2d(x, w, None, 2, 1), b, slope)
            else:
                y = self._deconv2d(x, w, b, 2, 1)
                if act:
                    y = self._act(y, slope, name)
        if _LISTENERS:
            self._ran(name, y, kind="deconv", act=act, x=x, w=w, stride=2, pad=1, own=own, into=False)
        return y

    def deconv(self, x, P, name, act=True):
        return self.deconv_wb(x, P[name + ".w"], P[name + ".b"], act, NEG_SLOPE, name)

    def predict_flow(self, x, P, name):
        if self._predict is not None:
            return self._predict(x, P[name + ".w"], P[name + ".b"])
        return self.conv(x, P, name, 1, 1, act=False)

    def upsample_flow(self, x, P, name, out=None, out_c0=0):
        if self._upsample is None:
            return None if out is not None else self.deconv(x, P, name, act=False)
        if out is not None:
            return self._upsample(x, P[name + ".w"], P[name + ".b"], out=out, out_c0=out_c0)
        return self._upsample(x, P[name + ".w"], P[name + ".b"])

    def leaky_relu(self, x, name, slope=NEG_SLOPE):
        y = self._act(x, slope, name)
        if _LISTENERS:
            self._ran(name, y, kind="relu", act=True, x=x, own=False, into=False)
        return y


_MODULE_ADAPTERS = {}


def backend_of(obj) -> GraphBackend:
    if isinstance(obj, GraphBackend):
        return obj
    if obj is None or isinstance(obj, types.ModuleType):
        be = _MODULE_ADAPTERS.get(obj)
        if be is None:
            be = _MODULE_ADAPTERS[obj] = GraphBackend(obj)
        return be
    return GraphBackend(obj)
```

### flownet2_amd/nets.py

```python
from __future__ import annotations

import math
import os
from typing import Dict, Optional

import torch

from .graph_backend import NEG_SLOPE, GraphBackend, backend_of, listening

FLOW_SCALE = 20.0
SD_FLOW_SCALE = 0.05
LOSS_WEIGHTS = {6: 0.32, 5: 0.08, 4: 0.02, 3: 0.01, 2: 0.005}

_ENC_TAIL = [("conv4", 256, 512, 3, 2, 1), ("conv4_1", 512, 512, 3, 1, 1), ("conv5", 512, 512, 3, 2, 1),
             ("conv5_1", 512, 512, 3, 1, 1), ("conv6", 512, 1024, 3, 2, 1), ("conv6_1", 1024, 1024, 3, 1, 1)]
_DEC = [("Convolution1", "conv", 1024, 2), ("deconv5", "deconv", 1024, 512), ("upsample_flow6to5", "deconv", 2, 2),
        ("Convolution2", "conv", 1026, 2), ("deconv4", "deconv", 1026, 256), ("upsample_flow5to4", "deconv", 2, 2),
        ("Convolution3", "conv", 770, 2), ("deconv3", "deconv", 770, 128), ("upsample_flow4to3", "deconv", 2, 2),
        ("Convolution4", "conv", 386, 2), ("deconv2", "deconv", 386, 64), ("upsample_flow3to2", "deconv", 2, 2),
        ("Convolution5", "conv", 194, 2)]


def layer_table(kind: str = "C", in_channels: int = 6):
    t = []
    if kind == "C":
        t += [("conv1", "conv", 3, 64, 7, 2, 3), ("conv2", "conv", 64, 128, 5, 2, 2), ("conv3", "conv", 128, 256, 5, 2, 2),
              ("conv_redir", "conv", 256, 32, 1, 1, 0), ("conv3_1", "conv", 473, 256, 3, 1, 1)]
    else:
        t += [("conv1", "conv", in_channels, 64, 7, 2, 3), ("conv2", "conv", 64, 128, 5, 2, 2), ("conv3", "conv", 128, 256, 5, 2, 2),
              ("conv3_1", "conv", 256, 256, 3, 1, 1)]
    t += [(n, "conv", ci, co, k, s, p) for (n, ci, co, k, s, p) in _ENC_TAIL]
    for (n, k, ci, co) in _DEC:
        t.append((n, k, ci, co, 3, 1, 1) if k == "conv" else (n, k, ci, co, 4, 2, 1))
    return t


def init_params(kind: str = "C", seed: int = 0, device="cpu", in_channels: int = 6) -> Dict[str, torch.Tensor]:
    g = torch.Generator().manual_seed(seed)
    params = {}
    for (name, k, ci, co, ks, s, p) in layer_table(kind, in_channels):
        shape = (co, ci, ks, ks) if k == "conv" else (ci, co, ks, ks)
        fan_in = ci * ks * ks if k == "conv" else ci * ks * ks / (s * s)
        std = math.sqrt(2.0 / ((1 + NEG_SLOPE ** 2) * fan_in))
        if name.startswith("Convolution"):
            std *= 0.5
        if name.startswith("upsample_flow"):
            std = 0.25
        params[name + ".w"] = (torch.randn(shape, generator=g) * std).to(device)
        params[name + ".b"] = torch.zeros(co).to(device)
    return params


def num_params(params) -> int:
    return sum(int(v.numel()) for v in params.values())


def conv_forward(x, w, b, stride, pad, act, backend, slope=None, relu_chain=None):
    return backend_of(backend).conv_wb(x, w, b, stride, pad, act, NEG_SLOPE if slope is None else slope, relu_chain=relu_chain)


_LAST_ROUTE = [""]


def _note_route(name, y, info):
    if info["kind"] != "conv":
        return
    be, x, w = info["backend"], info["x"], info["w"]
    if not info["own"]:
        _LAST_ROUTE[0] = "library conv2d"
    elif be.conv_route_name is None:
        _LAST_ROUTE[0] = "own kernel"
    else:
        _LAST_ROUTE[0] = "fn2 %s" % be.conv_route_name(x.shape, w, info["stride"], info["pad"], info["act"], not info["into"])


def _trace_route(name, y, info):
    if info["kind"] == "conv":
        _note_route(name, y, info)
        print("conv route %-16s in %-22s k%d s%d act=%d -> %s%s" % (name, tuple(info["x"].shape), info["w"].shape[2], info["stride"], info["act"],
                                                                  _LAST_ROUTE[0], " (into its Concat blob)" if info["into"] else ""))


if os.environ.get("FN2_TRACE_CONV") == "1":
    listening(_trace_route).__enter__()


_CONSTS: Dict[tuple, torch.Tensor] = {}


def _const(device, values):
    key = (str(device), tuple(float(v) for v in values))
    if key not in _CONSTS:
        _CONSTS[key] = torch.tensor(key[1], device=device, dtype=torch.float32)
    return _CONSTS[key]


def deconv_forward(x, w, b, act=True, backend=None, slope=None):
    return backend_of(backend).deconv_wb(x, w, b, act, NEG_SLOPE if slope is None else slope)


def _conv_into_concat(x, P, name, stride, pad, extra_channels, be, relu_chain=None):
    w = P[name + ".w"]
    training = torch.is_grad_enabled() and (x.requires_grad or _any_requires_grad(P))
    if be.writes_slices and w.shape[2] in (3, 5) and (be.trains_in_place or not training):
        k = w.shape[2]
        ho, wo = (x.shape[2] + 2 * pad - k) // stride + 1, (x.shape[3] + 2 * pad - k) // stride + 1
        blob = torch.empty((x.shape[0], w.shape[0] + extra_channels, ho, wo), device=x.device, dtype=x.dtype)
        y = be.own_conv(x, w, P[name + ".b"], stride, pad, NEG_SLOPE, True, out=blob, out_c0=0, relu_chain=relu_chain)
        if y is not None:
            be.wrote("conv", name, y, blob, 0, w.shape[0], x, w, stride, pad)
            return blob, (y if (training and y.requires_grad) else blob[:, :w.shape[0]])
    if relu_chain is not None:
        raise RuntimeError("relu_chain: conv '%s' left the own-kernel route after its producer was told it would fold the ReLU derivative" % name)
    return None, be.conv(x, P, name, stride, pad)


def _any_requires_grad(P) -> bool:
    vals = P.P.values() if isinstance(P, _Prefixed) else P.values()
    return any(v.requires_grad for v in vals)


def _refine_stage(P, skip, x, dname, flow, uname, be):
    blob, s = skip if isinstance(skip, tuple) else (None, skip)
    if blob is None:
        return torch.cat([s, be.deconv(x, P, dname), be.upsample_flow(flow, P, uname)], 1)
    wd, bd = P[dname + ".w"], P[dname + ".b"]
    cs, cd = s.shape[1], wd.shape[1]
    assert blob.shape[1] == cs + cd + 2
    d = be.own_deconv(x, wd, bd, NEG_SLOPE, True, out=blob, out_c0=cs)
    if d is not None:
        be.wrote("deconv", dname, d, blob, cs, cd, x, wd, 2, 1)
    stage_params = [wd, bd, P[uname + ".w"], P[uname + ".b"]]
    if torch.is_grad_enabled() and (s.requires_grad or x.requires_grad or flow.requires_grad or any(p.requires_grad for p in stage_params)):
        u = be.upsample_flow(flow, P, uname, out=blob, out_c0=cs + cd) if d is not None else None
        if d is None or u is None:
            return torch.cat([s, be.deconv(x, P, dname), be.upsample_flow(flow, P, uname)], 1)
        part = lambda t, c0, c: t if t.requires_grad else blob[:, c0:c0 + c]
        return _ConcatInPlace.apply(blob, s, part(d, cs, cd), part(u, cs + cd, 2))
    if d is None:
        blob[:, cs:cs + cd].copy_(be.deconv(x, P, dname))
    if be.upsample_flow(flow, P, uname, out=blob, out_c0=cs + cd) is None:
        blob[:, cs + cd:].copy_(be.upsample_flow(flow, P, uname))
    return blob


def _decoder(P, conv6_1, conv5_1, conv4_1, conv3_1, conv2, be):
    flow6 = be.predict_flow(conv6_1, P, "Convolution1")
    c5 = _refine_stage(P, conv5_1, conv6_1, "deconv5", flow6, "upsample_flow6to5", be)
    flow5 = be.predict_flow(c5, P, "Convolution2")
    c4 = _refine_stage(P, conv4_1, c5, "deconv4", flow5, "upsample_flow5to4", be)
    flow4 = be.predict_flow(c4, P, "Convolution3")
    c3 = _refine_stage(P, conv3_1, c4, "deconv3", flow4, "upsample_flow4to3", be)
    flow3 = be.predict_flow(c3, P, "Convolution4")
    c2 = _refine_stage(P, conv2, c3, "deconv2", flow3, "upsample_flow3to2", be)
    flow2 = be.predict_flow(c2, P, "Convolution5")
    return {2: flow2, 3: flow3, 4: flow4, 5: flow5, 6: flow6}


def _skip_conv(x, P, name, stride, pad, dname, be, relu_chain=None):
    return _conv_into_concat(x, P, name, stride, pad, P[dname + ".w"].shape[1] + 2, be, relu_chain=relu_chain)


RELU_CHAIN = [True]


def _stem_chain(P, x, be):
    if not (RELU_CHAIN[0] and be.has_stem_chain and torch.is_grad_enabled() and x.is_cuda):
        return None, None
    w1, w2 = P["conv1.w"], P["conv2.w"]
    if not (w1.requires_grad and w2.requires_grad and P["conv1.b"].requires_grad) or x.requires_grad:
        return None, None
    if be.conv_route_name(x.shape, w1, 2, 3) != "stem":
        return None, None
    c1_shape = (x.shape[0], w1.shape[0], (x.shape[2] - 1) // 2 + 1, (x.shape[3] - 1) // 2 + 1)
    if not be.relu_chain_supported(c1_shape, w2, 2, 2):
        return None, None
    cell = {"masked": False, "slope": NEG_SLOPE}
    return (1, cell), (2, cell)


class _ConcatInPlace(torch.autograd.Function):

    @staticmethod
    def forward(ctx, blob, *parts):
        ctx.cuts = [p.shape[1] for p in parts]
        assert sum(ctx.cuts) == blob.shape[1] and all(p.data_ptr() >= blob.data_ptr() for p in parts)
        return blob.view_as(blob)

    @staticmethod
    def backward(ctx, g):
        out, c0 = [None], 0
        for c in ctx.cuts:
            out.append(g[:, c0:c0 + c])
            c0 += c
        return tuple(out)


class _SplitTowers(torch.autograd.Function):

    @staticmethod
    def forward(ctx, x):
        n = x.shape[0] // 2
        return x[:n], x[n:]

    @staticmethod
    def backward(ctx, ga, gb):
        return torch.cat([ga, gb], 0)


class _StackedAndFirstTower(torch.autograd.Function):

    @staticmethod
    def forward(ctx, x):
        return x.view_as(x), x[:x.shape[0] // 2]

    @staticmethod
    def backward(ctx, g_all, g_first):
        if g_all._base is not None or not g_all.is_contiguous():
            g_all = g_all.clone(memory_format=torch.contiguous_format)
        g_all[:g_first.shape[0]].add_(g_first)
        return g_all


_CORR = dict(pad=20, kernel_size=1, max_displacement=20, stride_1=1, stride_2=2)


def flownet_c_core(P, img0, img1, backend, towers=None):
    be = backend_of(backend)
    x = towers if towers is not None else torch.cat([img0, img1], 0)
    n = x.shape[0] // 2
    chain1, chain2 = _stem_chain(P, x, be)
    c1 = be.conv(x, P, "conv1", 2, 3, relu_chain=chain1)
    blob2, c2 = _skip_conv(c1, P, "conv2", 2, 2, "deconv2", be, relu_chain=chain2)
    training = torch.is_grad_enabled() and c2.requires_grad
    c2_first = None
    if training:
        c2, c2_first = _StackedAndFirstTower.apply(c2)
    c3 = be.conv(c2, P, "conv3", 2, 2)
    c3a, c3b = _SplitTowers.apply(c3) if (training and c3.requires_grad) else (c3[:n], c3[n:])
    wr, br = P["conv_redir.w"], P["conv_redir.b"]
    cr = wr.shape[0]
    cat = None
    if be.fuses_correlation:
        cat = torch.empty((n, cr + 441, c3a.shape[2], c3a.shape[3]), device=c3a.device, dtype=c3a.dtype)
        if be.trains_in_place and torch.is_grad_enabled() and (c3a.requires_grad or c3b.requires_grad):
            redir = be.own_conv(c3a, wr, br, 1, 0, NEG_SLOPE, True, out=cat, out_c0=0)
            if redir is not None:
                be.wrote("conv", "conv_redir", redir, cat, 0, cr, c3a, wr, 1, 0)
            corr = be.own_correlation_relu_into(c3a, c3b, cat, cr, NEG_SLOPE, training=True, **_CORR)
            be.wrote("relu", "relu", corr, cat, cr, 441, c3a)
            if redir is not None and redir.requires_grad:
                cat = _ConcatInPlace.apply(cat, redir, corr)
            else:
                cat = torch.cat([be.conv(c3a, P, "conv_redir", 1, 0), corr], 1)
        else:
            corr = be.own_correlation_relu_into(c3a, c3b, cat, cr, NEG_SLOPE, **_CORR)
            if corr is None:
                cat = None
            else:
                be.wrote("relu", "relu", corr, cat, cr, 441, c3a)
                redir = None
                if not (torch.is_grad_enabled() and _any_requires_grad(P)):
                    redir = be.own_conv(c3a, wr, br, 1, 0, NEG_SLOPE, True, out=cat, out_c0=0)
                if redir is None:
                    cat[:, :cr].copy_(be.conv(c3a, P, "conv_redir", 1, 0))
                else:
                    be.wrote("conv", "conv_redir", redir, cat, 0, cr, c3a, wr, 1, 0)
    if cat is None:
        redir = be.conv(c3a, P, "conv_redir", 1, 0)
        corr = be.correlation(c3a, c3b, **_CORR)
        cat = torch.cat([redir, be.leaky_relu(corr, "relu")], 1)
    blob3, c31 = _skip_conv(cat, P, "conv3_1", 1, 1, "deconv3", be)
    c4 = be.conv(c31, P, "conv4", 2, 1)
    blob4, c41 = _skip_conv(c4, P, "conv4_1", 1, 1, "deconv4", be)
    c5 = be.conv(c41, P, "conv5", 2, 1)
    blob5, c51 = _skip_conv(c5, P, "conv5_1", 1, 1, "deconv5", be)
    c6 = be.conv(c51, P, "conv6", 2, 1)
    c61 = be.conv(c6, P, "conv6_1", 1, 1)
    c2s = c2_first if c2_first is not None else c2[:n]
    skip2 = (blob2[:n], c2s) if blob2 is not None else c2s
    return _decoder(P, c61, (blob5, c51), (blob4, c41), (blob3, c31), skip2, be)


def flownet_s_core(P, x, backend=None):
    be = backend_of(backend)
    c1 = be.conv(x, P, "conv1", 2, 3)
    blob2, c2 = _skip_conv(c1, P, "conv2", 2, 2, "deconv2", be)
    c3 = be.conv(c2, P, "conv3", 2, 2)
    blob3, c31 = _skip_conv(c3, P, "conv3_1", 1, 1, "deconv3", be)
    c4 = be.conv(c31, P, "conv4", 2, 1)
    blob4, c41 = _skip_conv(c4, P, "conv4_1", 1, 1, "deconv4", be)
    c5 = be.conv(c41, P, "conv5", 2, 1)
    blob5, c51 = _skip_conv(c5, P, "conv5_1", 1, 1, "deconv5", be)
    c6 = be.conv(c51, P, "conv6", 2, 1)
    c61 = be.conv(c6, P, "conv6_1", 1, 1)
    return _decoder(P, c61, (blob5, c51), (blob4, c41), (blob3, c31), (blob2, c2), be)


def adapted_size(h: int, w: int, divisor: int = 64):
    return int(math.ceil(h / divisor) * divisor), int(math.ceil(w / divisor) * divisor)


def deploy_forward(kind: str, P, img0, img1, backend, mean: Optional[torch.Tensor] = None):
    backend = backend_of(backend)
    N, _, H, W = img0.shape
    ah, aw = adapted_size(H, W)
    neg_default = mean is None
    if mean is None:
        mean = _const(img0.device, (0.411, 0.433, 0.45))
    if (ah, aw) == (H, W) and img0.is_cuda and not torch.is_grad_enabled() and backend.has_scale_shift:
        neg_mean = _const(img0.device, (-0.411, -0.433, -0.45)) if neg_default else (-mean).contiguous()
        if kind == "C":
            x = torch.empty((2 * N, 3, H, W), device=img0.device, dtype=torch.float32)
            backend.scale_shift(img0, 1.0 / 255.0, neg_mean, out=x[:N])
            backend.scale_shift(img1, 1.0 / 255.0, neg_mean, out=x[N:])
            flows = flownet_c_core(P, None, None, backend, towers=x)
        else:
            x = torch.empty((N, 6, H, W), device=img0.device, dtype=torch.float32)
            backend.scale_shift(img0, 1.0 / 255.0, neg_mean, out=x, out_c0=0)
            backend.scale_shift(img1, 1.0 / 255.0, neg_mean, out=x, out_c0=3)
            flows = flownet_s_core(P, x, backend)
    else:
        pre = []
        for im in (img0, img1):
            x = im * (1.0 / 255.0)
            if (ah, aw) != (H, W):
                x = backend.resample(x, ah, aw)
            pre.append(x - mean.view(1, 3, 1, 1))
        if kind == "C":
            flows = flownet_c_core(P, pre[0], pre[1], backend)
        else:
            flows = flownet_s_core(P, torch.cat(pre, 1), backend)
    if img0.is_cuda and not torch.is_grad_enabled() and backend.has_slices:
        flow = backend.resample_slices(flows[2], H, W, in_scale=FLOW_SCALE)
        if (ah, aw) == (H, W):
            return flow
    else:
        flow = flows[2] * FLOW_SCALE
        flow = backend.resample(flow, H, W)
    scale = _const(flow.device, (W / float(aw), H / float(ah)))
    return flow * scale.view(1, 2, 1, 1)


def loss_targets_ahead(gt_flow, backend, divisors=None):
    backend = backend_of(backend)
    if not (backend.targets_ahead and gt_flow.is_cuda):
        return None
    H, W = gt_flow.shape[2], gt_flow.shape[3]
    divisors = divisors or {s: 2 ** s for s in LOSS_WEIGHTS}
    gt = gt_flow * (1.0 / FLOW_SCALE)
    sizes = [(H // divisors[s], W // divisors[s]) for s in LOSS_WEIGHTS]
    tgts, ev = backend.downsample_ahead(gt, sizes)
    return {"targets": dict(zip(LOSS_WEIGHTS, tgts)), "event": ev, "sizes": dict(zip(LOSS_WEIGHTS, sizes))}


FINAL_FLOW_GT_SCALE = {"SD": 1.0 / SD_FLOW_SCALE, "fusion": 1.0}


def _lpq_kwargs(loss):
    if not (isinstance(loss, (tuple, list)) and 3 <= len(loss) <= 5 and loss[0] == "lpq"):
        raise ValueError('loss: None or ("lpq", p, q[, p_epsilon[, q_epsilon]]), got %r' % (loss,))
    p_eps, q_eps = (tuple(loss[3:]) + (0.0, 1e-2)[len(loss) - 3:])
    return dict(p=float(loss[1]), q=float(loss[2]), p_epsilon=float(p_eps), q_epsilon=float(q_eps), normalize_by_num_entries=True)


def final_flow_loss(flow, gt_flow, backend, scale, loss=None):
    backend = backend_of(backend)
    tgt = backend.downsample(gt_flow * scale, flow.shape[2], flow.shape[3])
    if loss is not None:
        return backend.lpq_loss(flow, tgt, **_lpq_kwargs(loss))
    return backend.l1_loss(flow, tgt, l2_per_location=True, normalize_by_num_entries=True)


def multiscale_loss(flows, gt_flow, backend, targets=None, loss=None):
    backend = backend_of(backend)
    lpq = _lpq_kwargs(loss) if loss is not None else None
    if (backend.has_multi_loss if lpq is None else backend.has_multi_lpq_loss) and gt_flow.is_cuda:
        scales = list(LOSS_WEIGHTS.items())
        preds = [flows[s] for s, _ in scales]
        if targets is not None and all(tuple(targets["sizes"][s]) == tuple(flows[s].shape[2:]) for s, _ in scales):
            backend.wait_ahead(targets["event"])
            tgts = [targets["targets"][s] for s, _ in scales]
        else:
            gt = gt_flow * (1.0 / FLOW_SCALE)
            tgts = [backend.downsample(gt, p.shape[2], p.shape[3]) for p in preds]
        if lpq is not None:
            return backend.lpq_loss_multi(preds, tgts, [w for _, w in scales], **lpq)[0]
        return backend.l1_loss_multi(preds, tgts, [w for _, w in scales], l2_per_location=True, normalize_by_num_entries=True)[0]
    gt = gt_flow * (1.0 / FLOW_SCALE)
    total = 0.0
    for s, w in LOSS_WEIGHTS.items():
        pred = flows[s]
        tgt = backend.downsample(gt, pred.shape[2], pred.shape[3])
        if lpq is not None:
            total = total + w * backend.lpq_loss(pred, tgt, **lpq)
        else:
            total = total + w * backend.l1_loss(pred, tgt, l2_per_location=True, normalize_by_num_entries=True)
    return total


def conv_flops(kind: str, h: int, w: int, in_channels: int = 6) -> float:
    fl = 0.0
    size = {}
    hh, ww = h, w
    res = {"conv1": 2, "conv2": 4, "conv3": 8, "conv_redir": 8, "conv3_1": 8, "conv4": 16, "conv4_1": 16, "conv5": 32, "conv5_1": 32,
           "conv6": 64, "conv6_1": 64, "Convolution1": 64, "deconv5": 32, "upsample_flow6to5": 32, "Convolution2": 32,
           "deconv4": 16, "upsample_flow5to4": 16, "Convolution3": 16, "deconv3": 8, "upsample_flow4to3": 8, "Convolution4": 8,
           "deconv2": 4, "upsample_flow3to2": 4, "Convolution5": 4}
    for (name, k, ci, co, ks, s, p) in layer_table(kind, in_channels):
        oh, ow = hh // res[name], ww // res[name]
        macs = oh * ow * co * ci * ks * ks if k == "conv" else (oh // 2) * (ow // 2) * ci * co * ks * ks
        mult = 2 if (kind == "C" and name in ("conv1", "conv2", "conv3")) else 1
        fl += 2.0 * macs * mult
    return fl


_SD_TABLE = [("conv0", "conv", 6, 64, 3, 1, 1), ("conv1", "conv", 64, 64, 3, 2, 1), ("conv1_1", "conv", 64, 128, 3, 1, 1),
             ("conv2", "conv", 128, 128, 3, 2, 1), ("conv2_1", "conv", 128, 128, 3, 1, 1), ("conv3", "conv", 128, 256, 3, 2, 1),
             ("conv3_1", "conv", 256, 256, 3, 1, 1), ("conv4", "conv", 256, 512, 3, 2, 1), ("conv4_1", "conv", 512, 512, 3, 1, 1),
             ("conv5", "conv", 512, 512, 3, 2, 1), ("conv5_1", "conv", 512, 512, 3, 1, 1), ("conv6", "conv", 512, 1024, 3, 2, 1),
             ("conv6_1", "conv", 1024, 1024, 3, 1, 1),
             ("Convolution1", "conv", 1024, 2, 3, 1, 1), ("deconv5", "deconv", 1024, 512, 4, 2, 1), ("upsample_flow6to5", "deconv", 2, 2, 4, 2, 1),
             ("interconv5", "conv", 1026, 512, 3, 1, 1), ("Convolution2", "conv", 512, 2, 3, 1, 1),
             ("deconv4", "deconv", 1026, 256, 4, 2, 1), ("upsample_flow5to4", "deconv", 2, 2, 4, 2, 1),
             ("interconv4", "conv", 770, 256, 3, 1, 1), ("Convolution3", "conv", 256, 2, 3, 1, 1),
             ("deconv3", "deconv", 770, 128, 4, 2, 1), ("upsample_flow4to3", "deconv", 2, 2, 4, 2, 1),
             ("interconv3", "conv", 386, 128, 3, 1, 1), ("Convolution4", "conv", 128, 2, 3, 1, 1),
             ("deconv2", "deconv", 386, 64, 4, 2, 1), ("upsample_flow3to2", "deconv", 2, 2, 4, 2, 1),
             ("interconv2", "conv", 194, 64, 3, 1, 1), ("Convolution5", "conv", 64, 2, 3, 1, 1)]
_FUSE_TABLE = [("conv0", "conv", 11, 64, 3, 1, 1), ("conv1", "conv", 64, 64, 3, 2, 1), ("conv1_1", "conv", 64, 128, 3, 1, 1),
               ("conv2", "conv", 128, 128, 3, 2, 1), ("conv2_1", "conv", 128, 128, 3, 1, 1),
               ("Convolution5", "conv", 128, 2, 3, 1, 1), ("deconv1", "deconv", 128, 32, 4, 2, 1), ("upsample_flow2to1", "deconv", 2, 2, 4, 2, 1),
               ("interconv1", "conv", 162, 32, 3, 1, 1), ("Convolution6", "conv", 32, 2, 3, 1, 1),
               ("deconv0", "deconv", 162, 16, 4, 2, 1), ("upsample_flow1to0", "deconv", 2, 2, 4, 2, 1),
               ("interconv0", "conv", 82, 16, 3, 1, 1), ("Convolution7", "conv", 16, 2, 3, 1, 1)]


_SD_RES = {"conv0": 1, "conv1": 2, "conv1_1": 2, "conv2": 4, "conv2_1": 4, "conv3": 8, "conv3_1": 8, "conv4": 16, "conv4_1": 16, "conv5": 32,
           "conv5_1": 32, "conv6": 64, "conv6_1": 64, "Convolution1": 64, "deconv5": 32, "upsample_flow6to5": 32, "interconv5": 32,
           "Convolution2": 32, "deconv4": 16, "upsample_flow5to4": 16, "interconv4": 16, "Convolution3": 16, "deconv3": 8,
           "upsample_flow4to3": 8, "interconv3": 8, "Convolution4": 8, "deconv2": 4, "upsample_flow3to2": 4, "interconv2": 4, "Convolution5": 4}
_FUSE_RES = {"conv0": 1, "conv1": 2, "conv1_1": 2, "conv2": 4, "conv2_1": 4, "Convolution5": 4, "deconv1": 2, "upsample_flow2to1": 2,
             "interconv1": 2, "Convolution6": 2, "deconv0": 1, "upsample_flow1to0": 1, "interconv0": 1, "Convolution7": 1}


def _table_flops(table, res, h, w):
    fl = 0.0
    for (name, k, ci, co, ks, s, p) in table:
        oh, ow = h // res[name], w // res[name]
        fl += 2.0 * (oh * ow * co * ci * ks * ks if k == "conv" else (oh // 2) * (ow // 2) * ci * co * ks * ks)
    return fl


def flownet2_conv_flops(h: int, w: int) -> float:
    return conv_flops("C", h, w) + 2 * conv_flops("S", h, w, 12) + _table_flops(_SD_TABLE, _SD_RES, h, w) + _table_flops(_FUSE_TABLE, _FUSE_RES, h, w)


# ... 217 lines not shown
```

### flownet2_amd/ops.py

```python
from __future__ import annotations

import ctypes as C

import torch

from . import _lib
from ._lib import CorrParams, L1LossParams, check


def _consts(*names):
    return tuple(_lib.CONSTANTS["FN2_" + n] for n in names)


MULTIPLY, SUBTRACT = _consts("CORR_MULTIPLY", "CORR_SUBTRACT")
FILL_ZERO, FILL_NAN = _consts("FILL_ZERO", "FILL_NAN")
NEAREST, LINEAR, CUBIC, AREA = _consts("RESAMPLE_NEAREST", "RESAMPLE_LINEAR", "RESAMPLE_CUBIC", "RESAMPLE_AREA")


def _stream():
    return C.c_void_p(torch.cuda.current_stream().cuda_stream)


def _chk(t: torch.Tensor, name: str, ndim: int = 4):
    if not isinstance(t, torch.Tensor) or not t.is_cuda:
# ... 312 lines not shown
    b1 = _chk_opt(bottom1, "bottom[1]")
    N, Cc, H, W = b0.shape
    d0 = torch.empty_like(b0)
    d1 = torch.empty_like(b0) if b1 is not None else None
    check(_lib.lib().fn2_lpq_loss_backward(_ptr(b0), _ptr(b1), C.c_float(float(top_diff)), _ptr(d0), _ptr(d1), N, Cc, H, W, *params,
                                           _ptr(workspace), workspace.numel(), _stream()))
    return d0, d1


_LPQ_SYNC = {}


def _lpq_scales(bottoms0, bottoms1, weights):
    n = len(bottoms0)
    b0s = [_chk(b, "bottom[0]") for b in bottoms0]
    b1s = [_chk_opt(bottoms1[k], "bottom[1]") if bottoms1 is not None else None for k in range(n)]
    for b0, b1 in zip(b0s, b1s):
        if b1 is not None and b1.shape != b0.shape:
            raise ValueError("LpqLoss: bottom blobs must have the same shape")
    shapes = (C.c_int * (4 * n))(*[int(d) for b in b0s for d in b.shape])
    return _ptr_array(b0s), _ptr_array(b1s), shapes, (C.c_float * n)(*[float(w) for w in weights]), b0s, b1s


def _ptr_array(tensors):
    return (C.c_void_p * len(tensors))(*[t.data_ptr() if t is not None else None for t in tensors])


def lpq_loss_forward_multi(params, bottoms0, bottoms1, weights):
    n = len(bottoms0)
    dev = bottoms0[0].device
    _, ws_bytes, sync_bytes = lpq_loss_sizes(n)
    ws = torch.empty(ws_bytes, dtype=torch.uint8, device=dev)
    key = (dev.index, int(torch.cuda.current_stream().cuda_stream))
    sync = _LPQ_SYNC.get(key)
    if sync is None:
        sync = _LPQ_SYNC[key] = torch.zeros(sync_bytes, dtype=torch.uint8, device=dev)
    losses = torch.empty((n,), device=dev, dtype=torch.float32)
    total = torch.empty((), device=dev, dtype=torch.float32)
    p0, p1, shapes, lw, _b0s, _b1s = _lpq_scales(bottoms0, bottoms1, weights)
    check(_lib.lib().fn2_lpq_loss_forward_multi(n, p0, p1, shapes, lw, *params, _ptr(losses), _ptr(total), _ptr(ws), ws.numel(), _ptr(sync),
                                                _stream()))
    return total, losses, ws


def lpq_loss_backward_multi(params, bottoms0, bottoms1, weights, total_diff, workspace, need1=False):
    n = len(bottoms0)
    p0, p1, shapes, lw, b0s, b1s = _lpq_scales(bottoms0, bottoms1, weights)
    d0 = [torch.empty_like(b) for b in b0s]
    d1 = [torch.empty_like(b) if (need1 and b1s[k] is not None) else None for k, b in enumerate(b0s)]
    td = _chk(total_diff.reshape(1), "total_diff", ndim=1) if total_diff is not None else None
    check(_lib.lib().fn2_lpq_loss_backward_multi(n, p0, p1, _ptr_array(d0), _ptr_array(d1), shapes, lw, *params, _ptr(td), _ptr(workspace),
                                                 workspace.numel(), _stream()))
    return d0, d1


_FLOW_METRICS_K = _lib.FLOW_METRICS_CONSTANTS["FN2_FLOW_METRICS_K"]


def flow_metrics_sizes(N: int, H: int, W: int):
    nbytes, k = C.c_size_t(), C.c_int()
    check(_lib.lib().fn2_flow_metrics_sizes(int(N), int(H), int(W), C.byref(nbytes), C.byref(k)))
    return nbytes.value, k.value


def flow_metrics(pred, gt, valid=None, occ=None, outlier=(3.0, 0.05), bands=(10.0, 40.0), epe_map=False):
    p, g = _chk(pred, "pred"), _chk(gt, "gt")
    if p.shape != g.shape or p.shape[1] != 2:
        raise ValueError(f"flow_metrics: pred {tuple(p.shape)} and gt {tuple(g.shape)} must both be [N,2,H,W]")
    N, _, H, W = p.shape
    v, o = _chk_opt(valid, "valid"), _chk_opt(occ, "occ")
    for name, m in (("valid", v), ("occ", o)):
        if m is not None and tuple(m.shape) != (N, 1, H, W):
            raise ValueError(f"flow_metrics: {name} {tuple(m.shape)} must be [{N},1,{H},{W}]")
    ws = torch.empty(flow_metrics_sizes(N, H, W)[0], dtype=torch.uint8, device=p.device)
    results = torch.empty((N + 1, _FLOW_METRICS_K), dtype=torch.float64, device=p.device)
    emap = torch.empty((N, 1, H, W), dtype=torch.float32, device=p.device) if epe_map else None
    check(_lib.lib().fn2_flow_metrics(_ptr(p), _ptr(g), _ptr(v), _ptr(o), N, H, W, C.c_float(float(outlier[0])), C.c_float(float(outlier[1])),
                                      C.c_float(float(bands[0])), C.c_float(float(bands[1])), _ptr(results), _ptr(emap), _ptr(ws), ws.numel(),
                                      _stream()))
    return results, emap


_FLOW_CONSISTENCY_K = _lib.FLOW_CONSISTENCY_CONSTANTS["FN2_FLOW_CONSISTENCY_K"]


def flow_consistency_sizes(N: int, H: int, W: int):
    nbytes, k = C.c_size_t(), C.c_int()
    check(_lib.lib().fn2_flow_consistency_sizes(int(N), int(H), int(W), C.byref(nbytes), C.byref(k)))
    return nbytes.value, k.value


def flow_consistency(fw, bw, alpha=(0.01, 0.5), beta=(0.01, 0.002), flags=False, err=False, warped=False):
    f, b = _chk(fw, "fw"), _chk(bw, "bw")
    if f.shape != b.shape or f.shape[1] != 2:
        raise ValueError(f"flow_consistency: fw {tuple(f.shape)} and bw {tuple(b.shape)} must both be [N,2,H,W]")
    if f.device != b.device:
        raise ValueError(f"flow_consistency: fw on {f.device}, bw on {b.device}")
    N, _, H, W = f.shape
    ws = torch.empty(flow_consistency_sizes(N, H, W)[0], dtype=torch.uint8, device=f.device)
    results = torch.empty((2, N + 1, _FLOW_CONSISTENCY_K), dtype=torch.float64, device=f.device)
    pair = lambda want, ch, dtype: tuple(torch.empty((N, ch, H, W), dtype=dtype, device=f.device) for _ in range(2)) if want else None
    occ, fl, er, wa = pair(True, 1, torch.float32), pair(flags, 1, torch.uint8), pair(err, 1, torch.float32), pair(warped, 2, torch.float32)
    two = lambda p: (_ptr(p[0]), _ptr(p[1])) if p is not None else (_ptr(None), _ptr(None))
    check(_lib.lib().fn2_flow_consistency(_ptr(f), _ptr(b), N, H, W, C.c_float(float(alpha[0])), C.c_float(float(alpha[1])),
                                          C.c_float(float(beta[0])), C.c_float(float(beta[1])), _ptr(results), *two(fl), *two(occ), *two(er),
                                          *two(wa), _ptr(ws), ws.numel(), _stream()))
    return results, occ, fl, er, wa


_FLOW_TRACK_K = _lib.FLOW_TRACK_CONSTANTS["FN2_FLOW_TRACK_K"]


def flow_track_sizes(N: int, T: int, H: int, W: int, P: int):
    nbytes, k = C.c_size_t(), C.c_int()
    check(_lib.lib().fn2_flow_track_sizes(int(N), int(T), int(H), int(W), int(P), C.byref(nbytes), C.byref(k)))
    return nbytes.value, k.value


def _chk_bytes(t, name: str, shape):
    if not isinstance(t, torch.Tensor) or not t.is_cuda:
        raise ValueError(f"{name}: expected a CUDA (HIP) tensor; flownet2_amd has no CPU path")
    if t.dtype != torch.uint8 or tuple(t.shape) != tuple(shape):
        raise ValueError(f"{name}: expected uint8 {list(shape)}, got {t.dtype} {list(t.shape)}")
    return t.contiguous()


def flow_track(fw, bw, points, state=None, stop=None, stop_mask=8, alpha=(0.01, 0.5), tracks=True, steps=True):
    f, b = _chk(fw, "fw", 5), _chk(bw, "bw", 5)
    if f.shape != b.shape or f.shape[2] != 2:
        raise ValueError(f"flow_track: fw {tuple(f.shape)} and bw {tuple(b.shape)} must both be [N,T,2,H,W]")
    N, T, _, H, W = f.shape
    p = _chk(points, "points", None)
    if p.dim() < 3 or p.shape[0] != N or p.shape[1] != 2:
        raise ValueError(f"flow_track: points {tuple(p.shape)} must be [{N},2,P]")
    if f.device != b.device or f.device != p.device:
        raise ValueError(f"flow_track: fw on {f.device}, bw on {b.device}, points on {p.device}")
    P = p[0, 0].numel()
    s_in = _chk_bytes(state, "state", (N, P)) if state is not None else None
    s_map = _chk_bytes(stop, "stop", (N, T, 1, H, W)) if stop is not None else None
    ws = torch.empty(flow_track_sizes(N, T, H, W, P)[0], dtype=torch.uint8, device=f.device)
    results = torch.empty((N + 1, _FLOW_TRACK_K), dtype=torch.float64, device=f.device)
    tr = torch.empty((N, T + 1, 2, P), dtype=torch.float32, device=f.device) if tracks else None
    p_out = torch.empty((N, 2, P), dtype=torch.float32, device=f.device)
    s_out = torch.empty((N, P), dtype=torch.uint8, device=f.device)
    st = torch.empty((N, P), dtype=torch.int32, device=f.device) if steps else None
    check(_lib.lib().fn2_flow_track(_ptr(f), _ptr(b), _ptr(s_map), int(stop_mask), _ptr(p), _ptr(s_in), N, T, H, W, P, C.c_float(float(alpha[0])),
                                    C.c_float(float(alpha[1])), _ptr(results), _ptr(tr), _ptr(p_out), _ptr(s_out),
                                    C.cast(_ptr(st), C.POINTER(C.c_int)), _ptr(ws), ws.numel(), _stream()))
    return results, tr, p_out, s_out, st


def flow_track_reseed(points, state, size, cell, born=True):
    H, W = int(size[0]), int(size[1])
    cell = int(cell)
    if cell < 1 or H < 1 or W < 1:
        raise ValueError(f"flow_track_reseed: bad size ({H}, {W}) or cell {cell}")
    P = -(-H // cell) * -(-W // cell)
    if not isinstance(points, torch.Tensor) or not points.is_cuda:
        raise ValueError("points: expected a CUDA (HIP) tensor; flownet2_amd has no CPU path")
    N = points.shape[0]
    if points.dtype != torch.float32 or tuple(points.shape) != (N, 2, P) or not points.is_contiguous():
        raise ValueError(f"flow_track_reseed: points must be contiguous float32 [N,2,{P}] for size ({H}, {W}) and cell {cell}, got {tuple(points.shape)}")
    if not isinstance(state, torch.Tensor) or state.dtype != torch.uint8 or tuple(state.shape) != (N, P) or not state.is_contiguous() \
            or state.device != points.device:
        raise ValueError(f"flow_track_reseed: state must be contiguous uint8 [{N},{P}] on {points.device}")
    ws = torch.empty(max(N * P, 1), dtype=torch.uint8, device=points.device)
    b = torch.empty((N, P), dtype=torch.uint8, device=points.device) if born else None
    check(_lib.lib().fn2_flow_track_reseed(_ptr(points), _ptr(state), _ptr(b), N, H, W, cell, _ptr(ws), ws.numel(), _stream()))
    return b


_FLOW_COLOR_NORMS = {n[len("FN2_FLOW_COLOR_NORM_"):].lower(): v for n, v in _lib.FLOW_VISUALIZE_CONSTANTS.items()}


def flow_visualize_sizes(N: int, H: int, W: int):
    nbytes = C.c_size_t()
    check(_lib.lib().fn2_flow_visualize_sizes(int(N), int(H), int(W), C.byref(nbytes)))
    return nbytes.value


def flow_color(flow, norm="sample", max_flow=None, maxrad=False):
    f = _chk(flow, "flow")
    if f.shape[1] != 2:
        raise ValueError(f"flow_color: flow {tuple(f.shape)} must be [N,2,H,W]")
    if norm not in _FLOW_COLOR_NORMS:
        raise ValueError(f"flow_color: norm must be one of {sorted(_FLOW_COLOR_NORMS)}, got {norm!r}")
    fixed = norm == "fixed"
    if fixed and max_flow is None:
        raise ValueError("flow_color: norm='fixed' needs max_flow")
    N, _, H, W = f.shape
    ws = None if fixed else torch.empty(flow_visualize_sizes(N, H, W), dtype=torch.uint8, device=f.device)
    rgb = torch.empty((N, H, W, 3), dtype=torch.uint8, device=f.device)
    used = torch.empty((N,), dtype=torch.float32, device=f.device) if maxrad else None
    check(_lib.lib().fn2_flow_color(_ptr(f), N, H, W, _FLOW_COLOR_NORMS[norm], C.c_float(float(max_flow) if fixed else 0.0), _ptr(rgb), _ptr(used),
                                    _ptr(ws), ws.numel() if ws is not None else 0, _stream()))
    return rgb, used


def flow_error_map(pred, gt, valid=None, occ=None, abs_thresh=3.0, rel_thresh=0.05):
    p, g = _chk(pred, "pred"), _chk(gt, "gt")
    if p.shape != g.shape or p.shape[1] != 2:
        raise ValueError(f"flow_error_map: pred {tuple(p.shape)} and gt {tuple(g.shape)} must both be [N,2,H,W]")
    if p.device != g.device:
        raise ValueError(f"flow_error_map: pred on {p.device}, gt on {g.device}")
    N, _, H, W = p.shape
    v, o = _chk_opt(valid, "valid"), _chk_opt(occ, "occ")
    for name, m in (("valid", v), ("occ", o)):
        if m is not None and tuple(m.shape) != (N, 1, H, W):
            raise ValueError(f"flow_error_map: {name} {tuple(m.shape)} must be [{N},1,{H},{W}]")
    rgb = torch.empty((N, H, W, 3), dtype=torch.uint8, device=p.device)
    check(_lib.lib().fn2_flow_error_map(_ptr(p), _ptr(g), _ptr(v), _ptr(o), N, H, W, C.c_float(float(abs_thresh)), C.c_float(float(rel_thresh)),
                                        _ptr(rgb), _stream()))
    return rgb


def channel_norm_forward(x):
    x = _chk(x, "bottom[0]")
    N, Cc, H, W = x.shape
    out = torch.empty((N, 1, H, W), device=x.device, dtype=torch.float32)
    check(_lib.lib().fn2_channel_norm_forward(_ptr(x), _ptr(out), N, Cc, H, W, _stream()))
    return out


def channel_norm_forward_slices(x, minus=None, out=None):
    b, bctot, bc0, Cc = _as_slice(x, "bottom[0]")
    N, _, H, W = b.shape
    m, mctot, mc0 = None, 0, 0
    if minus is not None:
        m, mctot, mc0, Cm = _as_slice(minus, "bottom[1]")
        if Cm != Cc or tuple(m.shape[2:]) != (H, W) or m.shape[0] != N:
            raise ValueError("channel_norm: the subtrahend does not match the bottom")
    if out is None:
        out = torch.empty((N, 1, H, W), device=b.device, dtype=torch.float32)
    top, tctot, tc0, Ct = _as_slice(out, "top[0]")
    if Ct != 1 or top.shape[0] != N or tuple(top.shape[2:]) != (H, W):
        raise ValueError("channel_norm: top slice must be one channel of the bottom's size")
    check(_lib.lib().fn2_channel_norm_forward_slices(_ptr(b), bctot, bc0, _ptr(m), mctot, mc0, _ptr(top), tctot, tc0, N, Cc, H, W, _stream()))
    return top


def channel_norm_backward(x, top, top_diff):
    x, top, td = _chk(x, "bottom[0]"), _chk(top, "top"), _chk(top_diff, "top.diff")
    N, Cc, H, W = x.shape
    d = torch.empty_like(x)
    check(_lib.lib().fn2_channel_norm_backward(_ptr(x), _ptr(top), _ptr(td), _ptr(d), N, Cc, H, W, _stream()))
    return d


def downsample_forward(x, top_height, top_width):
    x = _chk(x, "bottom[0]")
    N, Cc, H, W = x.shape
    if top_height < 1 or top_width < 1:
        raise ValueError("DownsampleLayer must have top_height > 0 and top_width > 0")
    out = torch.empty((N, Cc, int(top_height), int(top_width)), device=x.device, dtype=torch.float32)
    check(_lib.lib().fn2_downsample_forward(_ptr(x), _ptr(out), N, Cc, H, W, int(top_height), int(top_width), _stream()))
    return out


def downsample_forward_multi(x, sizes):
    x = _chk(x, "bottom[0]")
    N, Cc, H, W = x.shape
    sizes = [(int(h), int(w)) for h, w in sizes]
    outs = [torch.empty((N, Cc, h, w), device=x.device, dtype=torch.float32) for h, w in sizes]
    n = len(sizes)
    ptrs = (C.c_void_p * n)(*[_ptr(o) for o in outs])
    hs, ws = (C.c_int * n)(*[h for h, _ in sizes]), (C.c_int * n)(*[w for _, w in sizes])
    check(_lib.lib().fn2_downsample_forward_multi(_ptr(x), ptrs, hs, ws, n, N, Cc, H, W, _stream()))
    return outs


def downsample_multi_supported(x_shape, sizes) -> bool:
    H, W = int(x_shape[2]), int(x_shape[3])
    return 1 <= len(sizes) <= 8 and all(int(h) >= 2 and int(w) >= 2 and (int(h), int(w)) != (H, W) for h, w in sizes)


def predict_flow_conv_forward(x, weight, bias=None):
    x, w = _chk(x, "bottom[0]"), _chk(weight, "weight")
    N, Cc, H, W = x.shape
    if tuple(w.shape) != (2, Cc, 3, 3):
        raise ValueError(f"predict_flow weight must be [2,{Cc},3,3], got {tuple(w.shape)}")
    b = _chk(bias, "bias", ndim=1) if bias is not None else None
    out = torch.empty((N, 2, H, W), device=x.device, dtype=torch.float32)
    nbytes = _lib.lib().fn2_predict_flow_conv_workspace_bytes(N, Cc, H, W)
    ws = torch.empty(nbytes, dtype=torch.uint8, device=x.device) if nbytes else None
    check(_lib.lib().fn2_predict_flow_conv_forward(_ptr(x), _ptr(w), _ptr(b), _ptr(out), N, Cc, H, W, _ptr(ws), nbytes, _stream()))
    return out


def upsample_flow_deconv_forward(x, weight, bias=None, out=None, out_c0=0):
    x, w = _chk(x, "bottom[0]"), _chk(weight, "weight")
    N, Cc, H, W = x.shape
    if Cc != 2 or tuple(w.shape) != (2, 2, 4, 4):
        raise ValueError("upsample_flow expects a 2-channel flow and a [2,2,4,4] weight")
    b = _chk(bias, "bias", ndim=1) if bias is not None else None
    if out is not None:
        _chk(out, "top[0]")
        if out.shape[0] != N or tuple(out.shape[2:]) != (2 * H, 2 * W):
            raise ValueError(f"upsample_flow: top blob {tuple(out.shape)} does not match [{N},*,{2 * H},{2 * W}]")
        check(_lib.lib().fn2_upsample_flow_deconv_forward_into(_ptr(x), _ptr(w), _ptr(b), _ptr(out), N, H, W, out.shape[1], int(out_c0), _stream()))
        return out[:, out_c0:out_c0 + 2]
    out = torch.empty((N, 2, 2 * H, 2 * W), device=x.device, dtype=torch.float32)
    check(_lib.lib().fn2_upsample_flow_deconv_forward(_ptr(x), _ptr(w), _ptr(b), _ptr(out), N, H, W, _stream()))
    return out


def bias_leaky_relu_(x, bias=None, negative_slope=0.1):
    if not (isinstance(x, torch.Tensor) and x.is_cuda and x.dtype == torch.float32 and x.dim() == 4 and x.is_contiguous()):
        raise ValueError("bias_leaky_relu_: expected a contiguous float32 CUDA (HIP) NCHW tensor")
    N, Cc, H, W = x.shape
    b = _chk_opt(bias, "bias", 1)
    if b is not None and b.numel() != Cc:
        raise ValueError(f"bias must have {Cc} entries, got {b.numel()}")
    check(_lib.lib().fn2_bias_leaky_relu_forward(_ptr(x), _ptr(b), N, Cc, H, W, C.c_float(float(negative_slope)), _stream()))
    return x


def scale_shift_forward(x, scale, shift=None, out=None, out_c0=0):
    x = _chk(x, "bottom[0]")
    N, Cc, H, W = x.shape
    if out is None:
        out = torch.empty_like(x)
    else:
        _chk(out, "top[0]")
        if out.shape[0] != N or tuple(out.shape[2:]) != (H, W):
            raise ValueError("scale_shift: top blob does not match the bottom")
    s = _chk_opt(shift, "shift", 1)
    check(_lib.lib().fn2_scale_shift_forward(_ptr(x), _ptr(out), _ptr(s), N, Cc, H, W, out.shape[1], out_c0, C.c_float(float(scale)), _stream()))
    return out


def predict_flow_conv_backward_supported(N, C, H, W) -> bool:
    return bool(_lib.lib().fn2_predict_flow_conv_backward_supported(int(N), int(C), int(H), int(W)))


def _head_diffs(what, out, needs, shapes, device):
    if out is None:
        return tuple(torch.empty(s, device=device, dtype=torch.float32) if need else None for need, s in zip(needs, shapes))
    if len(out) != 3:
        raise ValueError(what + ": out must be (bottom_diff, weight_diff, bias_diff)")
    for t, need, s, name in zip(out, needs, shapes, ("bottom.diff", "weight.diff", "bias.diff")):
        if (t is not None) != bool(need):
            raise ValueError(f"{what}: out holds a {name} exactly where that gradient is needed")
        if t is not None and (_chk(t, name, ndim=len(s)) is not t or tuple(t.shape) != tuple(s)):
            raise ValueError(f"{what}: {name} must be a contiguous {list(s)} blob")
    return tuple(out)


def predict_flow_conv_backward(x, weight, top_diff, need_x=True, need_w=True, need_b=True, out=None, accumulate=False):
    xb, xctot, xc0, Cc = _as_slice(x, "bottom[0]")
    w, g = _chk(weight, "weight"), _chk(top_diff, "top.diff")
    N, _, H, W = xb.shape
    if tuple(w.shape) != (2, Cc, 3, 3) or tuple(g.shape) != (N, 2, H, W):
        raise ValueError("predict_flow_conv_backward: weight must be [2,C,3,3] and top_diff [N,2,H,W]")
    if accumulate and out is None:
        raise ValueError("predict_flow_conv_backward: accumulate needs the gradients to add to (out)")
    dx, dw, db = _head_diffs("predict_flow_conv_backward", out, (need_x, need_w, need_b), ((N, Cc, H, W), tuple(w.shape), (2,)), g.device)
    nbytes = _lib.lib().fn2_predict_flow_conv_backward_workspace_bytes(N, Cc, H, W) if (need_w or need_b) else 0
    ws = torch.empty(max(nbytes, 4), dtype=torch.uint8, device=g.device)
    check(_lib.lib().fn2_predict_flow_conv_backward(_ptr(xb), xctot, xc0, _ptr(w), _ptr(g), _ptr(dx), _ptr(dw), _ptr(db), N, Cc, H, W,
                                                    int(bool(accumulate)), _ptr(ws), nbytes, _stream()))
    return dx, dw, db


def upsample_flow_deconv_backward(x, weight, top_diff, need_x=True, need_w=True, need_b=True, out=None, accumulate=False):
    x, w, g = _chk(x, "bottom[0]"), _chk(weight, "weight"), _chk(top_diff, "top.diff")
    N, Cc, H, W = x.shape
    if Cc != 2 or tuple(w.shape) != (2, 2, 4, 4) or tuple(g.shape) != (N, 2, 2 * H, 2 * W):
        raise ValueError("upsample_flow_deconv_backward: bottom [N,2,H,W], weight [2,2,4,4], top_diff [N,2,2H,2W]")
    if accumulate and out is None:
        raise ValueError("upsample_flow_deconv_backward: accumulate needs the gradients to add to (out)")
    dx, dw, db = _head_diffs("upsample_flow_deconv_backward", out, (need_x, need_w, need_b), (tuple(x.shape), (2, 2, 4, 4), (2,)), g.device)
    nbytes = _lib.lib().fn2_upsample_flow_deconv_backward_workspace_bytes(N, H, W) if (need_w or need_b) else 0
    ws = torch.empty(max(nbytes, 4), dtype=torch.uint8, device=g.device)
    check(_lib.lib().fn2_upsample_flow_deconv_backward(_ptr(x), _ptr(w), _ptr(g), _ptr(dx), _ptr(dw), _ptr(db), N, H, W, int(bool(accumulate)),
                                                       _ptr(ws), nbytes, _stream()))
    return dx, dw, db


def conv_k7s2_relu_supported(Cin, Hin, Win, Cout) -> bool:
    return bool(_lib.lib().fn2_conv_k7s2_relu_supported(int(Cin), int(Hin), int(Win), int(Cout)))


def conv_k7s2_wgrad_supported(N, Cin, Hin, Win, Cout) -> bool:
    return bool(_lib.lib().fn2_conv_k7s2_wgrad_supported(int(N), int(Cin), int(Hin), int(Win), int(Cout)))


def conv_k7s2_wgrad_ksplit(N, Cin, Hin, Win, Cout) -> int:
    return int(_lib.lib().fn2_conv_k7s2_wgrad_ksplit(int(N), int(Cin), int(Hin), int(Win), int(Cout)))


def conv_k7s2_wgrad(top_diff, bottom):
    d, x = _chk(top_diff, "top.diff"), _chk(bottom, "bottom[0]")
    N, Cin, H, W = x.shape
    Cout = d.shape[1]
    if tuple(d.shape) != (N, Cout, (H - 1) // 2 + 1, (W - 1) // 2 + 1):
        raise ValueError(f"conv_k7s2_wgrad: top_diff {tuple(d.shape)} does not belong to a bottom of {tuple(x.shape)}")
    dw = torch.empty((Cout, Cin, 7, 7), device=x.device, dtype=torch.float32)
    ws, need = _scratch(x.device, _lib.lib().fn2_conv_k7s2_wgrad_workspace_bytes(N, Cin, H, W, Cout))
    check(_lib.lib().fn2_conv_k7s2_wgrad(_ptr(d), _ptr(x), _ptr(dw), N, Cin, H, W, Cout, 0, _ptr(ws), need, _stream()))
    return dw


def conv_k7s2_relu_forward(x, weight, bias=None, negative_slope=0.1):
    x, w = _chk(x, "bottom[0]"), _chk(weight, "weight")
    N, Cin, H, W = x.shape
    Cout = w.shape[0]
    if tuple(w.shape) != (Cout, Cin, 7, 7):
        raise ValueError(f"stem weight must be [Cout,{Cin},7,7], got {tuple(w.shape)}")
    b = _chk_opt(bias, "bias", 1)
    out = torch.empty((N, Cout, (H - 1) // 2 + 1, (W - 1) // 2 + 1), device=x.device, dtype=torch.float32)
    check(_lib.lib().fn2_conv_k7s2_relu_forward(_ptr(x), _ptr(w), _ptr(b), _ptr(out), N, Cin, H, W, Cout,
                                                C.c_float(float(negative_slope)), _stream()))
    return out


CONV_ROUTE_NONE, CONV_ROUTE_DIRECT, CONV_ROUTE_WINOGRAD, CONV_ROUTE_PLANE, CONV_ROUTE_STEM, CONV_ROUTE_HEAD = _consts(
    "CONV_ROUTE_NONE", "CONV_ROUTE_DIRECT", "CONV_ROUTE_WINOGRAD", "CONV_ROUTE_PLANE", "CONV_ROUTE_STEM", "CONV_ROUTE_HEAD")
DECONV_ROUTE_NONE, DECONV_ROUTE_GEMM, DECONV_ROUTE_PLANE, DECONV_ROUTE_HEAD = _consts("DECONV_ROUTE_NONE", "DECONV_ROUTE_GEMM", "DECONV_ROUTE_PLANE",
                                                                                      "DECONV_ROUTE_HEAD")
ROUTE_FORCE, ROUTE_BF16X3, ROUTE_WINO_BF16X3 = _consts("ROUTE_FORCE", "ROUTE_BF16X3", "ROUTE_WINO_BF16X3")
CONV_ARITH_BF16X3, = _consts("CONV_ARITH_BF16X3")
CONV_FWD_ROUTES = {0: None, 1: "direct", 2: "wino", 3: "plane", 4: "stem", 5: "head"}
DECONV_FWD_ROUTES = {0: None, 1: "gemm", 2: "plane", 3: "head"}
CONV_ROUTES = {0: None, 1: "direct", 2: "wino", 3: "plane", 4: None, 5: None}
DECONV_ROUTES = {0: None, 1: "gemm", 2: "plane", 3: None}


def conv_route(N, Cin, Hin, Win, Cout, kernel, stride, pad, force=False):
    return CONV_ROUTES[conv_forward_route(conv_desc(N, Cin, Hin, Win, Cout, kernel, stride, pad), force)]


def deconv_route(N, Cin, Hin, Win, Cout, kernel=4, stride=2, pad=1):
    return DECONV_ROUTES[deconv_forward_route(conv_desc(N, Cin, Hin, Win, Cout, kernel, stride, pad))]


BWD_ROUTES = {0: None, 1: "wino", 2: "tconv", 3: "plane", 4: "direct", 5: "deconv_plane"}


def conv_desc(N, Cin, Hin, Win, Cout, kernel, stride, pad):
    return _lib.ConvDesc(int(N), int(Cin), int(Hin), int(Win), int(Cout), int(kernel), int(stride), int(pad))


def conv_forward_route(desc, force=False, bf16x3=False, wino_bf16x3=False) -> int:
    flags = (ROUTE_FORCE if force else 0) | (ROUTE_BF16X3 if bf16x3 else 0) | (ROUTE_WINO_BF16X3 if wino_bf16x3 else 0)
    return int(_lib.lib().fn2_conv_route(C.byref(desc), flags))


def deconv_forward_route(desc, bf16x3=False) -> int:
    return int(_lib.lib().fn2_deconv_route(C.byref(desc), ROUTE_BF16X3 if bf16x3 else 0))


def conv_pack_weights(weight, desc, route, transposed=False):
    w = _chk(weight, "weight")
    L = _lib.lib()
    floats, pack = (L.fn2_deconv_packed_weight_floats, L.fn2_deconv_pack_weights) if transposed else (L.fn2_conv_packed_weight_floats, L.fn2_conv_pack_weights)
    n = int(floats(C.byref(desc), int(route)))
    k = desc.kernel
    if n == 0 or tuple(w.shape) != ((desc.Cin, desc.Cout, k, k) if transposed else (desc.Cout, desc.Cin, k, k)):
        raise ValueError("conv_pack_weights: route %d has no operand for a weight of shape %s" % (route, tuple(w.shape)))
    packed = torch.empty(n, device=w.device, dtype=torch.float32)
    check(pack(C.byref(desc), int(route), _ptr(w), _ptr(packed), _stream()))
    return packed


def conv_forward(x, packed, bias, desc, route, transposed=False, relu=True, negative_slope=0.1, out=None, out_c0=0, in_c0=0):
    x = _chk(x, "bottom[0]")
    N, Ctot, H, W = x.shape
    k, s, p = desc.kernel, desc.stride, desc.pad
    if (N, H, W) != (desc.N, desc.Hin, desc.Win) or in_c0 < 0 or in_c0 + desc.Cin > Ctot:
        raise ValueError(f"conv_forward: bottom blob {tuple(x.shape)} does not hold the layer's [{desc.N},{desc.Cin},{desc.Hin},{desc.Win}] at channel {in_c0}")
    Ho, Wo = (2 * H, 2 * W) if transposed else ((H + 2 * p - k) // s + 1, (W + 2 * p - k) // s + 1)
    if out is None:
        out = torch.empty((N, desc.Cout, Ho, Wo), device=x.device, dtype=torch.float32)
    else:
        _chk(out, "top[0]")
        if not out.is_contiguous() or out.shape[0] != N or tuple(out.shape[2:]) != (Ho, Wo) or out_c0 < 0 or out_c0 + desc.Cout > out.shape[1]:
            raise ValueError(f"conv_forward: top blob {tuple(out.shape)} does not match [{N},>={out_c0 + desc.Cout},{Ho},{Wo}]")
    b = _chk(bias, "bias", ndim=1) if bias is not None else None
    pw = _chk(packed, "packed weight", ndim=None)
    L = _lib.lib()
    if pw.numel() != int((L.fn2_deconv_packed_weight_floats if transposed else L.fn2_conv_packed_weight_floats)(C.byref(desc), int(route))):
        raise ValueError("conv_forward: the operand has %d floats, not what route %d reads for this layer" % (pw.numel(), route))
    need = int((L.fn2_deconv_workspace_bytes if transposed else L.fn2_conv_workspace_bytes)(C.byref(desc), int(route)))
    if transposed and (route & ~CONV_ARITH_BF16X3) == DECONV_ROUTE_GEMM:
        ws = torch.empty((need + 3) // 4, device=x.device, dtype=torch.float32)
    else:
        ws = _plane_workspace(x.device, need) if need else None
    check((L.fn2_deconv_forward if transposed else L.fn2_conv_forward)(
        C.byref(desc), int(route), _ptr(x), Ctot, int(in_c0), _ptr(pw), _ptr(b), _ptr(out), out.shape[1], int(out_c0),
        int(bool(relu)), C.c_float(float(negative_slope)), _ptr(ws), need, _stream()))
    return out


def conv_backward_data_route(desc, transposed=False, bf16x3=False) -> int:
    if not bf16x3:
        return int(_lib.lib().fn2_conv_backward_data_route(C.byref(desc), int(bool(transposed))))
    return int(_lib.lib().fn2_conv_backward_data_route_flags(C.byref(desc), int(bool(transposed)), ROUTE_BF16X3))


def _check_dgrad_operand(what, packed, desc, tr, route):
    n = int(_lib.lib().fn2_conv_backward_data_packed_weight_floats(C.byref(desc), tr, int(route)))
    if n == 0:
        raise ValueError("%s: route %d is not this layer's" % (what, route))
    if packed.numel() != n:
        raise ValueError("%s: the operand has %d floats, route %d of this layer needs %d (packed for another route?)" % (what, packed.numel(), route, n))


def conv_backward_data_pack_weights(weight, desc, transposed, route):
    w = _chk(weight, "weight")
    L, tr = _lib.lib(), int(bool(transposed))
    n = int(L.fn2_conv_backward_data_packed_weight_floats(C.byref(desc), tr, int(route)))
    if n == 0:
        raise ValueError("conv_backward_data_pack_weights: route %d is not this layer's" % route)
    packed = torch.empty(n, device=w.device, dtype=torch.float32)
    need = int(L.fn2_conv_backward_data_pack_workspace_bytes(C.byref(desc), tr, int(route)))
    ws = torch.empty(need // 4, device=w.device, dtype=torch.float32) if need else None
    check(L.fn2_conv_backward_data_pack_weights(C.byref(desc), tr, int(route), _ptr(w), _ptr(packed), _ptr(ws), need, _stream()))
    return packed


def conv_backward_data(top_diff, packed_weight, desc, transposed, route, top_c0=0):
    d = _chk(top_diff, "top_diff")
    L, tr = _lib.lib(), int(bool(transposed))
    Cp = int(L.fn2_conv_backward_data_computed_channels(C.byref(desc), tr, int(route)))
    if Cp == 0:
        raise ValueError("conv_backward_data: route %d is not this layer's" % route)
    _check_dgrad_operand("conv_backward_data", packed_weight, desc, tr, route)
    out = torch.empty((desc.N, Cp, desc.Hin, desc.Win), device=d.device, dtype=torch.float32)
    need = int(L.fn2_conv_backward_data_workspace_bytes_with_room(C.byref(desc), tr, int(route), Cp))
    ws = _plane_workspace(d.device, need) if need else None
    check(L.fn2_conv_backward_data(C.byref(desc), tr, int(route), _ptr(d), d.shape[1], int(top_c0), _ptr(packed_weight), _ptr(out), Cp, 0, Cp,
                                   _ptr(ws), need, _stream()))
    return out[:, :desc.Cin] if Cp != desc.Cin else out


def conv_backward_weights_supported(desc, transposed=False) -> bool:
    return bool(_lib.lib().fn2_conv_backward_weights_supported(C.byref(desc), int(bool(transposed))))


def conv_backward_weights_arith(desc, transposed=False, bf16x3=False) -> int:
    return int(_lib.lib().fn2_conv_backward_weights_arith(C.byref(desc), int(bool(transposed)), ROUTE_BF16X3 if bf16x3 else 0))


def conv_backward_weights(bottom, top_diff, desc, transposed=False, out=None, accumulate=False, bottom_c0=0, top_c0=0, bf16x3=False):
    x, d = _chk(bottom, "bottom"), _chk(top_diff, "top_diff")
    L, tr = _lib.lib(), int(bool(transposed))
    k = desc.kernel
    shape = (desc.Cin, desc.Cout, k, k) if transposed else (desc.Cout, desc.Cin, k, k)
    if out is None:
        out = torch.empty(shape, device=x.device, dtype=torch.float32)
        accumulate = False
    else:
        out = _chk(out, "weight diff")
        if tuple(out.shape) != shape:
            raise ValueError("conv_backward_weights: weight diff has the wrong shape")
    arith = conv_backward_weights_arith(desc, transposed, True) if bf16x3 else 0
    if arith:
        need = int(L.fn2_conv_backward_weights_workspace_bytes_arith(C.byref(desc), tr, arith))
        ws = _plane_workspace(x.device, need) if need else None
        check(L.fn2_conv_backward_weights_arith_run(C.byref(desc), tr, arith, _ptr(x), x.shape[1], int(bottom_c0), _ptr(d), d.shape[1], int(top_c0),
                                                    _ptr(out), int(bool(accumulate)), _ptr(ws), need, _stream()))
        return out
    need = int(L.fn2_conv_backward_weights_workspace_bytes(C.byref(desc), tr))
    ws = _plane_workspace(x.device, need) if need else None
    check(L.fn2_conv_backward_weights(C.byref(desc), tr, _ptr(x), x.shape[1], int(bottom_c0), _ptr(d), d.shape[1], int(top_c0), _ptr(out),
                                      int(bool(accumulate)), _ptr(ws), need, _stream()))
    return out


def conv_backward_data_masked_supported(desc, transposed, route) -> bool:
    return bool(_lib.lib().fn2_conv_backward_data_masked_supported(C.byref(desc), int(bool(transposed)), int(route)))


def conv_backward_data_masked(top_diff, packed, desc, transposed, route, bottom_data, negative_slope, top_c0=0, data_c0=0):
    d, y = _chk(top_diff, "top_diff"), _chk(bottom_data, "bottom data")
    _check_dgrad_operand("conv_backward_data_masked", packed, desc, int(bool(transposed)), route)
    out = torch.empty((desc.N, desc.Cin, desc.Hin, desc.Win), device=d.device, dtype=torch.float32)
    check(_lib.lib().fn2_conv_backward_data_masked(C.byref(desc), int(bool(transposed)), int(route), _ptr(d), d.shape[1], int(top_c0), _ptr(packed),
                                                   _ptr(out), desc.Cin, 0, _ptr(y), y.shape[1], int(data_c0), C.c_float(float(negative_slope)), _stream()))
    return out


def conv_backward_weights_bias_fused(desc, transposed=False) -> bool:
    return bool(_lib.lib().fn2_conv_backward_weights_bias_fused(C.byref(desc), int(bool(transposed))))


def conv_backward_weights_bias(bottom, top_diff, desc, transposed=False, out=None):
    x, d = _chk(bottom, "bottom"), _chk(top_diff, "top_diff")
    L, tr = _lib.lib(), int(bool(transposed))
    k = desc.kernel
    dw = out if out is not None else torch.empty((desc.Cout, desc.Cin, k, k), device=x.device, dtype=torch.float32)
    db = torch.empty(desc.Cout, device=x.device, dtype=torch.float32)
    need = int(L.fn2_conv_backward_weights_workspace_bytes(C.byref(desc), tr))
    ws = _plane_workspace(x.device, need) if need else None
    check(L.fn2_conv_backward_weights_bias(C.byref(desc), tr, _ptr(x), _ptr(d), _ptr(dw), _ptr(db), 0, _ptr(ws), need, _stream()))
    return dw, db


def conv_backward_bias(top_diff, C_, top_c0=0, out=None, accumulate=False):
    d = _chk(top_diff, "top_diff")
    N, Ctot, H, W = d.shape
    if out is None:
        out = torch.empty(C_, device=d.device, dtype=torch.float32)
        accumulate = False
    need = int(_lib.lib().fn2_bias_leaky_relu_backward_workspace_bytes(N, C_, H, W))
    ws = _plane_workspace(d.device, need)
# ... 668 lines not shown
```

Before: 3597.

## Fuse flow prediction gather with 2x flow upsampling and add 1x1 conv tail handling

Adds a fused kernel that reduces the split 3x3 predict-flow partials and applies the 4x4 stride-2 flow upsampling deconvolution from a shared-memory tile, writing straight into the decoder concat blob. This removes one kernel launch and a global round trip of the low-resolution flow at each of four decoder stages. It also restructures the 1x1 MFMA conv path so the last partial K chunk is handled separately, with early exit and a predicated weight prefetch, and it registers several new tile variants. The added complexity in the inline-asm wait logic risks correctness or scheduling regressions.

```diff
diff --git a/flownet2_amd/_lib.py b/flownet2_amd/_lib.py
--- a/flownet2_amd/_lib.py
+++ b/flownet2_amd/_lib.py
@@ -92,7 +92,7 @@
            "flownet2_hip_flow_track.h": {}}
     for h in ("flownet2_hip.h", "flownet2_hip_solver.h", "flownet2_hip_corr_route.h", "flownet2_hip_conv_general.h",
               "flownet2_hip_conv_geometry.h", "flownet2_hip_conv_volume.h", "flownet2_hip_lpq_loss.h", "flownet2_hip_flow_metrics.h",
-              "flownet2_hip_flow_consistency.h", "flownet2_hip_flow_visualize.h", "flownet2_hip_flow_track.h"):
+              "flownet2_hip_flow_consistency.h", "flownet2_hip_flow_visualize.h", "flownet2_hip_flow_track.h", "flownet2_hip_flow_head.h"):
         with open(os.path.join(INCLUDE_DIR, h)) as f:
             functions, structs, c = parse_header(f.read(), structs)
         per_header.append(functions)
@@ -104,11 +104,12 @@
 (_PER_HEADER, _STRUCTS, CONSTANTS, FLOW_METRICS_CONSTANTS, FLOW_CONSISTENCY_CONSTANTS, FLOW_VISUALIZE_CONSTANTS,
  FLOW_TRACK_CONSTANTS) = _parse_headers()
 (EXPORTS, SOLVER_EXPORTS, CORR_ROUTE_EXPORTS, CONV_GENERAL_EXPORTS, CONV_GEOMETRY_EXPORTS, CONV_VOLUME_EXPORTS, LPQ_LOSS_EXPORTS,
- FLOW_METRICS_EXPORTS, FLOW_CONSISTENCY_EXPORTS, FLOW_VISUALIZE_EXPORTS, FLOW_TRACK_EXPORTS) = (list(f) for f in _PER_HEADER)
+ FLOW_METRICS_EXPORTS, FLOW_CONSISTENCY_EXPORTS, FLOW_VISUALIZE_EXPORTS, FLOW_TRACK_EXPORTS, FLOW_HEAD_EXPORTS) = (list(f) for f in _PER_HEADER)
 PROTOTYPES = {name: proto for f in _PER_HEADER[:8] for name, proto in f.items()}
 FLOW_CONSISTENCY_PROTOTYPES = dict(_PER_HEADER[8])
 FLOW_VISUALIZE_PROTOTYPES = dict(_PER_HEADER[9])
 FLOW_TRACK_PROTOTYPES = dict(_PER_HEADER[10])
+FLOW_HEAD_PROTOTYPES = dict(_PER_HEADER[11])
 globals().update({cls.__name__: cls for cls in _STRUCTS.values()})
 _HOOKS = parse_header("""
     int fn2_debug_set_correlation_impl(int impl);
@@ -129,7 +130,7 @@
             "(or __graft_entry__.build()). flownet2_amd has no CPU / PyTorch fallback.")
     L = C.CDLL(SO_PATH)
     for table, required in ((PROTOTYPES, True), (FLOW_CONSISTENCY_PROTOTYPES, True), (FLOW_VISUALIZE_PROTOTYPES, True),
-                            (FLOW_TRACK_PROTOTYPES, True), (_HOOKS, False)):
+                            (FLOW_TRACK_PROTOTYPES, True), (FLOW_HEAD_PROTOTYPES, True), (_HOOKS, False)):
         for name, (restype, argtypes) in table.items():
             if not hasattr(L, name):
                 if required:
diff --git a/flownet2_amd/csrc/conv_mfma.hip b/flownet2_amd/csrc/conv_mfma.hip
--- a/flownet2_amd/csrc/conv_mfma.hip
+++ b/flownet2_amd/csrc/conv_mfma.hip
@@ -11,6 +11,7 @@
   int Cout, Hout, Wout, out_ctot, out_c0;
   int pad;
   int nchunks;
+  int kquads;
   int ksteps;
   int tx, ty;
   int ng;
@@ -37,6 +38,90 @@
 };
 
 template <class K>
+__device__ __forceinline__ void gemm_chunk(f32x4 (&acc)[K::MW][K::NP], typename WVec<K::MW>::T (&wreg)[K::NBUFA], const float* win,
+                                           const float* wk, unsigned wlane, int ahead) {
+  static_assert(K::KS == 1 && K::S == 1, "1x1 tiles");
+  constexpr int MW = K::MW, NP = K::NP, KSC = K::KSC, PW = K::P16 ? 16 : 4;
+  constexpr int R = K::NBUFA - 1, DMA = K::NRUN / K::NW;
+  using WV = typename WVec<MW>::T;
+  auto weight_step = [&](int ks) -> WV {
+    const float* wks = wk + (size_t)(ks + R) * 256;
+    if (ks + R < KSC) wreg[(ks + R) % K::NBUFA] = weight_fetch<MW>(wks, wlane);
+    else wreg[(ks + R) % K::NBUFA] = weight_fetch_unless_last<MW>(ahead, ks + R - KSC, wks, wlane);
+    const int behind = ks < R ? R + DMA : R;
+    const int next = ks + R - KSC + 1;
+    if (next >= 2) ring_wait_either(ahead, R, behind - (next - 1), behind);
+    else ring_wait(behind);
+    weight_landed(wreg[ks % K::NBUFA]);
+    return wreg[ks % K::NBUFA];
+  };
+  if constexpr (K::PIN) {
+    float b[2][NP];
+#pragma unroll
+    for (int p = 0; p < NP; ++p) b[0][p] = win[PW * p];
+    __builtin_amdgcn_sched_barrier(0);
+#pragma unroll
+    for (int ks = 0; ks < KSC; ++ks) {
+      const WV w = weight_step(ks);
+#pragma unroll
+      for (int p = 0; p < NP; ++p) {
+#pragma unroll
+        for (int j = 0; j < MW; ++j) acc[j][p] = __builtin_amdgcn_mfma_f32_16x16x4f32(b[ks & 1][p], wget<MW>(w, j), acc[j][p], 0, 0, 0);
+        if (ks + 1 < KSC) b[(ks + 1) & 1][p] = win[(ks + 1 < KSC ? ks + 1 : ks) * 4 * K::CS + PW * p];
+        __builtin_amdgcn_sched_barrier(0);
+      }
+    }
+  } else {
+#pragma unroll
+    for (int ks = 0; ks < KSC; ++ks) {
+      const WV w = weight_step(ks);
+      float b[NP];
+#pragma unroll
+      for (int p = 0; p < NP; ++p) b[p] = win[ks * 4 * K::CS + PW * p];
+#pragma unroll
+      for (int j = 0; j < MW; ++j)
+#pragma unroll
+        for (int p = 0; p < NP; ++p) acc[j][p] = __builtin_amdgcn_mfma_f32_16x16x4f32(b[p], wget<MW>(w, j), acc[j][p], 0, 0, 0);
+    }
+  }
+}
+
+template <class K>
+__device__ __forceinline__ void gemm_last_chunk(f32x4 (&acc)[K::MW][K::NP], typename WVec<K::MW>::T (&wreg)[K::NBUFA], const float* win,
+                                                const float* wk, unsigned wlane, int live) {
+  static_assert(K::KS == 1 && K::S == 1, "1x1 tiles");
+  constexpr int MW = K::MW, NP = K::NP, KSC = K::KSC, PW = K::P16 ? 16 : 4;
+  constexpr int R = K::NBUFA - 1;
+  using WV = typename WVec<MW>::T;
+  const int last = live - 1;
+  wait_vmcnt<R>();
+#pragma unroll
+  for (int j = R - 1; j >= 1; --j) ring_wait_if_le(live, j, j);
+  __builtin_amdgcn_s_barrier();
+  float b[2][NP];
+#pragma unroll
+  for (int p = 0; p < NP; ++p) b[0][p] = win[PW * p];
+  if constexpr (K::PIN) __builtin_amdgcn_sched_barrier(0);
+#pragma unroll
+  for (int ks = 0; ks < KSC; ++ks) {
+    if (ks + R < KSC) wreg[(ks + R) % K::NBUFA] = weight_fetch_unless_last<MW>(live, ks + R, wk + (size_t)(ks + R) * 256, wlane);
+    ring_wait(KSC - 1 - ks < R ? KSC - 1 - ks : R);
+#pragma unroll
+    for (int j = (KSC - 1 - ks < R ? KSC - 1 - ks : R) - 1; j >= 0; --j) ring_wait_if_le(last, ks + j, j);
+    weight_landed(wreg[ks % K::NBUFA]);
+    const WV w = wreg[ks % K::NBUFA];
+#pragma unroll
+    for (int p = 0; p < NP; ++p) {
+#pragma unroll
+      for (int j = 0; j < MW; ++j) acc[j][p] = __builtin_amdgcn_mfma_f32_16x16x4f32(b[ks & 1][p], wget<MW>(w, j), acc[j][p], 0, 0, 0);
+      if (ks + 1 < KSC) b[(ks + 1) & 1][p] = win[(ks + 1 < KSC ? ks + 1 : ks) * 4 * K::CS + PW * p];
+      if constexpr (K::PIN) __builtin_amdgcn_sched_barrier(0);
+    }
+    if (ks + 1 < KSC && last == ks) return;
+  }
+}
+
+template <class K>
 __device__ __forceinline__ void conv_body(const Args& a, int g, int bx, int by, int n) {
   static_assert(K::THREADS == 256, "launch bounds");
   extern __shared__ __attribute__((aligned(16))) float smem[];
@@ -72,61 +157,77 @@
   static_assert(R + DMA <= 63, "vmcnt has 6 bits");
   WV wreg[K::NBUFA];
   stage(0, 0);
-  if (a.nchunks > 0) {
-#pragma unroll
-    for (int i = 0; i < R; ++i) wreg[i] = weight_fetch<MW>(wb + (size_t)i * 256, wlane);
-  }
-  auto weight_step = [&](int ks0, int ks, int rest) -> WV {
-    const float* wks = wb + (size_t)(ks0 + ks + R) * 256;
-    if (ks + R < K::KSC) wreg[(ks + R) % K::NBUFA] = weight_fetch<MW>(wks, wlane);
-    else wreg[(ks + R) % K::NBUFA] = weight_fetch_unless_last<MW>(rest, wks, wlane);
-    const int left = K::KSC - 1 - ks < R ? K::KSC - 1 - ks : R;
-    if (ks < R) ring_wait_either(rest, left, R + DMA);
-    else if (left < R) ring_wait_either(rest, left, R);
-    else ring_wait(R);
-    weight_landed(wreg[ks % K::NBUFA]);
-    return wreg[ks % K::NBUFA];
-  };
-
-  for (int c = 0; c < a.nchunks; ++c) {
-    const int buf = c & 1;
-    const int rest = a.nchunks - 1 - c;
-    wait_vmcnt<R>();
-    __builtin_amdgcn_s_barrier();
-    if (rest) stage(c + 1, buf ^ 1);
-    const float* win = smem + buf * K::BUF + bbase;
-    const int ks0 = c * K::KSC;
-    if constexpr (K::PIN) {
-      float b[2][NP];
-      auto tap_off = [](int ks) { const int cq = ks / (KS * KS), ky = (ks / KS) % KS, kx = ks % KS; return cq * 4 * K::CS + ky * K::RS + kx; };
-#pragma unroll
-      for (int p = 0; p < NP; ++p) b[0][p] = win[tap_off(0) + PW * S * p];
-      __builtin_amdgcn_sched_barrier(0);
+  if constexpr (KS == 1) {
+    const int nfull = a.nchunks - 1;
+    const int live = a.kquads - nfull * K::KSC;
+#pragma unroll
+    for (int i = 0; i < R; ++i) wreg[i] = weight_fetch_unless_last<MW>(nfull ? K::KSC : live, i, wb + (size_t)i * 256, wlane);
+    for (int c = 0; c < nfull; ++c) {
+      const int buf = c & 1;
+      wait_vmcnt<R>();
+      __builtin_amdgcn_s_barrier();
+      stage(c + 1, buf ^ 1);
+      gemm_chunk<K>(acc, wreg, smem + buf * K::BUF + bbase, wb + (size_t)c * K::KSC * 256, wlane, c + 1 < nfull ? K::KSC : live);
+    }
+    gemm_last_chunk<K>(acc, wreg, smem + (nfull & 1) * K::BUF + bbase, wb + (size_t)nfull * K::KSC * 256, wlane, live);
+  } else {
+    if (a.nchunks > 0) {
+#pragma unroll
+      for (int i = 0; i < R; ++i) wreg[i] = weight_fetch<MW>(wb + (size_t)i * 256, wlane);
+    }
+    auto weight_step = [&](int ks0, int ks, int rest) -> WV {
+      const float* wks = wb + (size_t)(ks0 + ks + R) * 256;
+      if (ks + R < K::KSC) wreg[(ks + R) % K::NBUFA] = weight_fetch<MW>(wks, wlane);
+      else wreg[(ks + R) % K::NBUFA] = weight_fetch_unless_last<MW>(rest, 0, wks, wlane);
+      const int left = K::KSC - 1 - ks < R ? K::KSC - 1 - ks : R;
+      if (ks < R) ring_wait_either(rest, 1, left, R + DMA);
+      else if (left < R) ring_wait_either(rest, 1, left, R);
+      else ring_wait(R);
+      weight_landed(wreg[ks % K::NBUFA]);
+      return wreg[ks % K::NBUFA];
+    };
+
+    for (int c = 0; c < a.nchunks; ++c) {
+      const int buf = c & 1;
+      const int rest = a.nchunks - 1 - c;
+      wait_vmcnt<R>();
+      __builtin_amdgcn_s_barrier();
+      if (rest) stage(c + 1, buf ^ 1);
+      const float* win = smem + buf * K::BUF + bbase;
+      const int ks0 = c * K::KSC;
+      if constexpr (K::PIN) {
+        float b[2][NP];
+        auto tap_off = [](int ks) { const int cq = ks / (KS * KS), ky = (ks / KS) % KS, kx = ks % KS; return cq * 4 * K::CS + ky * K::RS + kx; };
+#pragma unroll
+        for (int p = 0; p < NP; ++p) b[0][p] = win[tap_off(0) + PW * S * p];
+        __builtin_amdgcn_sched_barrier(0);
+#pragma unroll
+        for (int ks = 0; ks < K::KSC; ++ks) {
+          const WV w = weight_step(ks0, ks, rest);
+#pragma unroll
+          for (int p = 0; p < NP; ++p) {
+#pragma unroll
+            for (int j = 0; j < MW; ++j) acc[j][p] = __builtin_amdgcn_mfma_f32_16x16x4f32(b[ks & 1][p], wget<MW>(w, j), acc[j][p], 0, 0, 0);
+            if (ks + 1 < K::KSC) b[(ks + 1) & 1][p] = win[tap_off(ks + 1 < K::KSC ? ks + 1 : ks) + PW * S * p];
+            __builtin_amdgcn_sched_barrier(0);
+          }
+        }
+      } else {
 #pragma unroll
       for (int ks = 0; ks < K::KSC; ++ks) {
         const WV w = weight_step(ks0, ks, rest);
-#pragma unroll
-        for (int p = 0; p < NP; ++p) {
-#pragma unroll
-          for (int j = 0; j < MW; ++j) acc[j][p] = __builtin_amdgcn_mfma_f32_16x16x4f32(b[ks & 1][p], wget<MW>(w, j), acc[j][p], 0, 0, 0);
-          if (ks + 1 < K::KSC) b[(ks + 1) & 1][p] = win[tap_off(ks + 1 < K::KSC ? ks + 1 : ks) + PW * S * p];
-          __builtin_amdgcn_sched_barrier(0);
-        }
+        const int cq = ks / (KS * KS), ky = (ks / KS) % KS, kx = ks % KS;
+        float b[NP];
+#pragma unroll
+        for (int p = 0; p < NP; ++p) b[p] = win[cq * 4 * K::CS + ky * K::RS + kx + PW * S * p];
+#pragma unroll
+        for (int j = 0; j < MW; ++j)
+#pragma unroll
+          for (int p = 0; p < NP; ++p) acc[j][p] = __builtin_amdgcn_mfma_f32_16x16x4f32(b[p], wget<MW>(w, j), acc[j][p], 0, 0, 0);
       }
-    } else {
-#pragma unroll
-    for (int ks = 0; ks < K::KSC; ++ks) {
-      const WV w = weight_step(ks0, ks, rest);
-      const int cq = ks / (KS * KS), ky = (ks / KS) % KS, kx = ks % KS;
-      float b[NP];
-#pragma unroll
-      for (int p = 0; p < NP; ++p) b[p] = win[cq * 4 * K::CS + ky * K::RS + kx + PW * S * p];
-#pragma unroll
-      for (int j = 0; j < MW; ++j)
-#pragma unroll
-        for (int p = 0; p < NP; ++p) acc[j][p] = __builtin_amdgcn_mfma_f32_16x16x4f32(b[p], wget<MW>(w, j), acc[j][p], 0, 0, 0);
-    }
-    }
+      }
+    }
+
   }
 
   wait_vmcnt<0>();
@@ -270,7 +371,8 @@
   }
   a.tx = cdiv(a.Wout, K::TW); a.ty = cdiv(a.Hout, K::TH);
   a.ng = a.Cout / (16 * K::MW * K::WM);
-  a.nchunks = cdiv(cdiv(a.Cin, 4), K::CQ);
+  a.kquads = cdiv(a.Cin, 4);
+  a.nchunks = cdiv(a.kquads, K::CQ);
 }
 
 inline long long tiles_of(const Args& a) { return (long long)a.N * a.tx * a.ty * a.ng; }
@@ -346,7 +448,8 @@
   FN2_CV_PIN(1, 1, 2, 7, 2, 2, 1, 8, 1, 1) FN2_CV_PIN(1, 1, 2, 3, 2, 2, 1, 8, 1, 1)
   FN2_CV_PIN(3, 1, 2, 7, 2, 2, 1, 2, 0, 1) FN2_CV_PIN(3, 1, 2, 6, 2, 2, 1, 2, 0, 1) FN2_CV_PIN(3, 2, 2, 7, 2, 1, 2, 2, 0, 1) FN2_CV_PIN(3, 2, 2, 6, 2, 2, 1, 2, 0, 1)
   FN2_CV_PIN(4, 2, 2, 7, 2, 2, 1, 2, 0, 1) FN2_CV_PIN(4, 2, 2, 6, 2, 2, 1, 2, 0, 1) FN2_CV_PIN(5, 2, 2, 6, 2, 2, 1, 1, 0, 1)
-  FN2_CV_PIN(7, 2, 2, 6, 2, 2, 1, 1, 0, 1) FN2_CV_PIN(7, 2, 4, 6, 1, 2, 2, 1, 0, 0)};
+  FN2_CV_PIN(7, 2, 2, 6, 2, 2, 1, 1, 0, 1) FN2_CV_PIN(7, 2, 4, 6, 1, 2, 2, 1, 0, 0)
+  FN2_CV_ROW16(2, 1, 1, 4, 1, 0) FN2_CV_ROW16(2, 2, 1, 4, 1, 0) FN2_CV_PIN(1, 1, 2, 1, 1, 4, 1, 8, 1, 0) FN2_CV_PIN(1, 1, 2, 2, 1, 4, 1, 8, 1, 0)};
 constexpr int kNumVariants = sizeof(kVariants) / sizeof(kVariants[0]);
 
 int g_forced_variant = -1;
diff --git a/flownet2_amd/csrc/flow_head.hip b/flownet2_amd/csrc/flow_head.hip
--- a/flownet2_amd/csrc/flow_head.hip
+++ b/flownet2_amd/csrc/flow_head.hip
@@ -1,4 +1,5 @@
 #include "fn2_common.hpp"
+#include "../../include/flownet2_hip_flow_head.h"
 
 namespace fn2 {
 
@@ -56,6 +57,31 @@
 }
 
 template <int NSPLIT>
+__device__ __forceinline__ float gather_flow(const float* __restrict__ P, const float* __restrict__ bias, int N, int H, int W,
+                                             unsigned n, unsigned o, int y, int x) {
+  const unsigned plane = (unsigned)H * W;
+  float v[NSPLIT][9];
+#pragma unroll
+  for (int sp = 0; sp < NSPLIT; ++sp) {
+    const float* Pn = P + (((size_t)sp * N + n) * 18 + o * 9) * plane;
+#pragma unroll
+    for (int dy = 0; dy < 3; ++dy)
+#pragma unroll
+      for (int dx = 0; dx < 3; ++dx) {
+        const int yy = y + dy - 1, xx = x + dx - 1;
+        const bool ok = yy >= 0 && yy < H && xx >= 0 && xx < W;
+        v[sp][dy * 3 + dx] = ok ? Pn[(size_t)(dy * 3 + dx) * plane + (unsigned)yy * W + xx] : 0.f;
+      }
+  }
+  float sacc = bias ? bias[o] : 0.f;
+#pragma unroll
+  for (int sp = 0; sp < NSPLIT; ++sp)
+#pragma unroll
+    for (int t = 0; t < 9; ++t) sacc += v[sp][t];
+  return sacc;
+}
+
+template <int NSPLIT>
 __global__ void __launch_bounds__(256) conv3x3_c2_gather(const float* __restrict__ P, const float* __restrict__ bias,
                                                           float* __restrict__ out, int N, int H, int W) {
   const unsigned plane = (unsigned)H * W;
@@ -63,26 +89,7 @@
   if (pix >= plane) return;
   const int y = pix / W, x = pix - y * W;
   const unsigned no = blockIdx.y;
-  const unsigned n = no >> 1, o = no & 1;
-  float v[NSPLIT][9];
-#pragma unroll
-  for (int sp = 0; sp < NSPLIT; ++sp) {
-    const float* Pn = P + (((size_t)sp * N + n) * 18 + o * 9) * plane;
-#pragma unroll
-    for (int dy = 0; dy < 3; ++dy)
-#pragma unroll
-      for (int dx = 0; dx < 3; ++dx) {
-        const int yy = y + dy - 1, xx = x + dx - 1;
-        const bool ok = yy >= 0 && yy < H && xx >= 0 && xx < W;
-        v[sp][dy * 3 + dx] = ok ? Pn[(size_t)(dy * 3 + dx) * plane + (unsigned)yy * W + xx] : 0.f;
-      }
-  }
-  float sacc = bias ? bias[o] : 0.f;
-#pragma unroll
-  for (int sp = 0; sp < NSPLIT; ++sp)
-#pragma unroll
-    for (int t = 0; t < 9; ++t) sacc += v[sp][t];
-  out[(size_t)no * plane + pix] = sacc;
+  out[(size_t)no * plane + pix] = gather_flow<NSPLIT>(P, bias, N, H, W, no >> 1, no & 1, y, x);
 }
 
 __global__ void __launch_bounds__(256) deconv4x4s2_c2(const float* __restrict__ in, const float* __restrict__ w,
@@ -114,6 +121,55 @@
     out[(((size_t)n * out_ctot + out_c0 + 0) * Ho + Y) * Wo + X] = a0;
     out[(((size_t)n * out_ctot + out_c0 + 1) * Ho + Y) * Wo + X] = a1;
   }
+}
+
+constexpr int kFuseT = 8, kFuseB = kFuseT + 2;
+static_assert(2 * kFuseB * kFuseB <= 256 && 4 * kFuseT * kFuseT == 256, "one gather and one up-sampled pixel per thread");
+
+template <int NSPLIT>
+__global__ void __launch_bounds__(256) conv3x3_c2_gather_deconv4x4s2(const float* __restrict__ P, const float* __restrict__ bias,
+                                                                      const float* __restrict__ wup, const float* __restrict__ bias_up,
+                                                                      float* __restrict__ flow, float* __restrict__ up,
+                                                                      int N, int H, int W, int tiles_x, int up_ctot, int up_c0) {
+  __shared__ float sflow[2][kFuseB][kFuseB];
+  const int t = threadIdx.x;
+  const int y0 = (int)(blockIdx.x / tiles_x) * kFuseT, x0 = (int)(blockIdx.x % tiles_x) * kFuseT;
+  const unsigned n = blockIdx.y;
+  if (t < 2 * kFuseB * kFuseB) {
+    const int c = t / (kFuseB * kFuseB), r = t % (kFuseB * kFuseB), ly = r / kFuseB, lx = r % kFuseB;
+    const int iy = y0 - 1 + ly, ix = x0 - 1 + lx;
+    float v = 0.f;
+    if (iy >= 0 && iy < H && ix >= 0 && ix < W) {
+      v = gather_flow<NSPLIT>(P, bias, N, H, W, n, c, iy, ix);
+      if (ly >= 1 && ly <= kFuseT && lx >= 1 && lx <= kFuseT) flow[(((size_t)n * 2 + c) * H + iy) * W + ix] = v;
+    }
+    sflow[c][ly][lx] = v;
+  }
+  __syncthreads();
+  const int Ho = 2 * H, Wo = 2 * W;
+  const int Y = 2 * y0 + t / (2 * kFuseT), X = 2 * x0 + t % (2 * kFuseT);
+  if (Y >= Ho || X >= Wo) return;
+  float a0 = bias_up ? bias_up[0] : 0.f, a1 = bias_up ? bias_up[1] : 0.f;
+#pragma unroll
+  for (int ty = 0; ty < 2; ++ty) {
+    const int ky = ((Y + 1) & 1) + 2 * ty;
+    const int iy = (Y + 1 - ky) / 2;
+    if (Y + 1 - ky < 0 || iy >= H) continue;
+#pragma unroll
+    for (int tx = 0; tx < 2; ++tx) {
+      const int kx = ((X + 1) & 1) + 2 * tx;
+      const int ix = (X + 1 - kx) / 2;
+      if (X + 1 - kx < 0 || ix >= W) continue;
+#pragma unroll
+      for (int c = 0; c < 2; ++c) {
+        const float v = sflow[c][iy - y0 + 1][ix - x0 + 1];
+        a0 = fmaf(wup[((c * 2 + 0) * 4 + ky) * 4 + kx], v, a0);
+        a1 = fmaf(wup[((c * 2 + 1) * 4 + ky) * 4 + kx], v, a1);
+      }
+    }
+  }
+  up[(((size_t)n * up_ctot + up_c0 + 0) * Ho + Y) * Wo + X] = a0;
+  up[(((size_t)n * up_ctot + up_c0 + 1) * Ho + Y) * Wo + X] = a1;
 }
 
 }
@@ -178,3 +234,35 @@
   hipLaunchKernelGGL(deconv4x4s2_c2, dim3(blocks_for(total, 256, 4096)), dim3(256), 0, as_stream(stream), in, weight, bias, top, N, H, W, top_channels, top_c0);
   return check_launch("upsample_flow_deconv_forward_into");
 }
+
+FN2_API int fn2_predict_upsample_flow_supported(int N, int C, int H, int W) {
+  return N >= 1 && C >= 1 && H >= 1 && W >= 1 && 2ll * N <= 65535 && 4ll * H * W < (1ll << 31);
+}
+
+FN2_API int fn2_predict_upsample_flow_forward_into(const float* in, const float* weight, const float* bias, float* flow,
+                                                   const float* up_weight, const float* up_bias, float* top,
+                                                   int N, int C, int H, int W, int top_channels, int top_c0,
+                                                   void* workspace, size_t workspace_bytes, void* stream) {
+  if (N < 0 || C < 1 || H < 1 || W < 1) return fail(FN2_ERR_INVALID_ARG, "predict_upsample_flow: bad shape [%d,%d,%d,%d]", N, C, H, W);
+  if (top_c0 < 0 || top_c0 + 2 > top_channels) return fail(FN2_ERR_INVALID_ARG, "predict_upsample_flow: channel slice outside the blob");
+  if (N == 0) return FN2_OK;
+  if (!in || !weight || !flow || !up_weight || !top) return fail(FN2_ERR_INVALID_ARG, "predict_upsample_flow: NULL blob pointer");
+  if (!fn2_predict_upsample_flow_supported(N, C, H, W)) return fail(FN2_ERR_UNSUPPORTED, "predict_upsample_flow: blob too large");
+  const size_t need = fn2_predict_flow_conv_workspace_bytes(N, C, H, W);
+  if (!workspace || workspace_bytes < need) return fail(FN2_ERR_WORKSPACE, "predict_upsample_flow: workspace too small (%zu < %zu)", workspace_bytes, need);
+  const long long total = (long long)N * H * W;
+  const unsigned blocks = (unsigned)((total + kHeadPix - 1) / kHeadPix);
+  const int nsplit = head_splits(N, C, H, W);
+  hipStream_t st = as_stream(stream);
+  float* P = reinterpret_cast<float*>(workspace);
+  hipLaunchKernelGGL(conv3x3_c2_taps<kHeadG>, dim3(blocks, nsplit), dim3(kHeadPix * kHeadG), 0, st, in, weight, P, N, C, H, W, nsplit);
+  const int tiles_x = (W + kFuseT - 1) / kFuseT;
+  const dim3 g2((unsigned)tiles_x * ((H + kFuseT - 1) / kFuseT), N);
+  switch (nsplit) {
+    case 1: hipLaunchKernelGGL(conv3x3_c2_gather_deconv4x4s2<1>, g2, dim3(256), 0, st, P, bias, up_weight, up_bias, flow, top, N, H, W, tiles_x, top_channels, top_c0); break;
+    case 2: hipLaunchKernelGGL(conv3x3_c2_gather_deconv4x4s2<2>, g2, dim3(256), 0, st, P, bias, up_weight, up_bias, flow, top, N, H, W, tiles_x, top_channels, top_c0); break;
+    case 4: hipLaunchKernelGGL(conv3x3_c2_gather_deconv4x4s2<4>, g2, dim3(256), 0, st, P, bias, up_weight, up_bias, flow, top, N, H, W, tiles_x, top_channels, top_c0); break;
+    default: hipLaunchKernelGGL(conv3x3_c2_gather_deconv4x4s2<8>, g2, dim3(256), 0, st, P, bias, up_weight, up_bias, flow, top, N, H, W, tiles_x, top_channels, top_c0); break;
+  }
+  return check_launch("predict_upsample_flow_forward_into");
+}
diff --git a/flownet2_amd/csrc/mfma_tile.hpp b/flownet2_amd/csrc/mfma_tile.hpp
--- a/flownet2_amd/csrc/mfma_tile.hpp
+++ b/flownet2_amd/csrc/mfma_tile.hpp
@@ -111,25 +111,37 @@
 
 __device__ __forceinline__ void ring_wait(int n) { asm volatile("s_waitcnt vmcnt(%0)" ::"i"(vmcnt_clamp(n))); }
 
-__device__ __forceinline__ void ring_wait_either(int rest, int n_last, int n_else) {
+__device__ __forceinline__ void ring_wait_either(int s, int below, int n_short, int n_full) {
   asm volatile(
-      "s_cmp_eq_u32 %0, 0\n\t"
+      "s_cmp_lt_u32 %0, %1\n\t"
       "s_cbranch_scc1 .Lrwt_%=\n\t"
-      "s_waitcnt vmcnt(%2)\n\t"
+      "s_waitcnt vmcnt(%3)\n\t"
       "s_branch .Lrwe_%=\n"
       ".Lrwt_%=:\n\t"
-      "s_waitcnt vmcnt(%1)\n"
+      "s_waitcnt vmcnt(%2)\n"
       ".Lrwe_%=:"
       :
-      : "s"(rest), "i"(vmcnt_clamp(n_last)), "i"(vmcnt_clamp(n_else))
+      : "s"(s), "i"(below), "i"(vmcnt_clamp(n_short)), "i"(vmcnt_clamp(n_full))
       : "scc");
 }
 
-template <int MW>
-__device__ __forceinline__ typename WVec<MW>::T weight_fetch_unless_last(int rest, const float* base, unsigned lane_bytes) {
+__device__ __forceinline__ void ring_wait_if_le(int s, int most, int n) {
+  asm volatile(
+      "s_cmp_gt_u32 %0, %1\n\t"
+      "s_cbranch_scc1 .Lrwl_%=\n\t"
+      "s_waitcnt vmcnt(%2)\n"
+      ".Lrwl_%=:"
+      :
+      : "s"(s), "i"(most), "i"(vmcnt_clamp(n))
+      : "scc");
+}
+
+template <int MW>
+__device__ __forceinline__ typename WVec<MW>::T weight_fetch_unless_last(int ahead, int i, const float* base, unsigned lane_bytes) {
   typename WVec<MW>::T w;
 #define FN2_FETCH_UNLESS(INSN) \
-  asm volatile("s_cmp_eq_u32 %3, 0\n\ts_cbranch_scc1 .Lwfs_%=\n\t" INSN " %0, %1, %2\n.Lwfs_%=:" : "=v"(w) : "v"(lane_bytes), "s"(base), "s"(rest) : "scc")
+  asm volatile("s_cmp_le_u32 %3, %4\n\ts_cbranch_scc1 .Lwfs_%=\n\t" INSN " %0, %1, %2\n.Lwfs_%=:" \
+               : "=v"(w) : "v"(lane_bytes), "s"(base), "s"(ahead), "i"(i) : "scc")
   if constexpr (MW == 1) FN2_FETCH_UNLESS("global_load_dword");
   else if constexpr (MW == 2) FN2_FETCH_UNLESS("global_load_dwordx2");
   else FN2_FETCH_UNLESS("global_load_dwordx4");
diff --git a/flownet2_amd/functional.py b/flownet2_amd/functional.py
--- a/flownet2_amd/functional.py
+++ b/flownet2_amd/functional.py
@@ -540,6 +540,12 @@
     if _needs_grad(x, weight, bias):
         return _UpsampleFlow.apply(x, weight, bias, None if out is None else (out, out_c0))
     return run(x, weight, bias)
+
+
+def predict_upsample_flow(x, weight, bias, up_weight, up_bias, out, out_c0):
+    if _needs_grad(x, weight, bias) or _needs_grad(x, up_weight, up_bias):
+        return None
+    return ops.predict_upsample_flow_forward(x.contiguous(), weight.contiguous(), bias, up_weight.contiguous(), up_bias, out, out_c0)
 
 
 class _BiasLeakyReLU(torch.autograd.Function):
diff --git a/flownet2_amd/graph_backend.py b/flownet2_amd/graph_backend.py
--- a/flownet2_amd/graph_backend.py
+++ b/flownet2_amd/graph_backend.py
@@ -36,6 +36,7 @@
         self.own_conv, self.own_deconv = get("conv_mfma_relu") or _declines, get("deconv_relu") or _declines
         self.own_correlation_relu_into = get("correlation_relu_into") or _declines
         self._predict, self._upsample = get("predict_flow_conv"), get("upsample_flow_deconv")
+        self._predict_upsample = get("predict_upsample_flow")
         self._bias_act = get("conv_bias_leaky_relu")
         self._conv2d = get("lib_conv2d") or (lambda x, w, b, s, p: F.conv2d(x, w, b, stride=s, padding=p))
         self._deconv2d = get("lib_conv_transpose2d") or (lambda x, w, b, s, p: F.conv_transpose2d(x, w, b, stride=s, padding=p))
@@ -113,6 +114,14 @@
             return self._upsample(x, P[name + ".w"], P[name + ".b"], out=out, out_c0=out_c0)
         return self._upsample(x, P[name + ".w"], P[name + ".b"])
 
+    def predict_upsample_flow(self, x, P, pname, uname, out, out_c0):
+        if self._predict_upsample is not None:
+            flow = self._predict_upsample(x, P[pname + ".w"], P[pname + ".b"], P[uname + ".w"], P[uname + ".b"], out, out_c0)
+            if flow is not None:
+                return flow, True
+        flow = self.predict_flow(x, P, pname)
+        return flow, self.upsample_flow(flow, P, uname, out=out, out_c0=out_c0) is not None
+
     def leaky_relu(self, x, name, slope=NEG_SLOPE):
         y = self._act(x, slope, name)
         if _LISTENERS:
diff --git a/flownet2_amd/nets.py b/flownet2_amd/nets.py
--- a/flownet2_amd/nets.py
+++ b/flownet2_amd/nets.py
@@ -120,7 +120,7 @@
     return any(v.requires_grad for v in vals)
 
 
-def _refine_stage(P, skip, x, dname, flow, uname, be):
+def _refine_stage(P, skip, x, dname, flow, uname, be, upsampled=False):
     blob, s = skip if isinstance(skip, tuple) else (None, skip)
     if blob is None:
         return torch.cat([s, be.deconv(x, P, dname), be.upsample_flow(flow, P, uname)], 1)
@@ -139,20 +139,28 @@
         return _ConcatInPlace.apply(blob, s, part(d, cs, cd), part(u, cs + cd, 2))
     if d is None:
         blob[:, cs:cs + cd].copy_(be.deconv(x, P, dname))
-    if be.upsample_flow(flow, P, uname, out=blob, out_c0=cs + cd) is None:
+    if not upsampled and be.upsample_flow(flow, P, uname, out=blob, out_c0=cs + cd) is None:
         blob[:, cs + cd:].copy_(be.upsample_flow(flow, P, uname))
     return blob
 
 
+def _head_into_stage(P, x, pname, skip, dname, uname, be):
+    blob, s = skip if isinstance(skip, tuple) else (None, skip)
+    params = [P[n + k] for n in (pname, dname, uname) for k in (".w", ".b")]
+    if blob is None or (torch.is_grad_enabled() and (s.requires_grad or x.requires_grad or any(p.requires_grad for p in params))):
+        return be.predict_flow(x, P, pname), False
+    return be.predict_upsample_flow(x, P, pname, uname, blob, s.shape[1] + P[dname + ".w"].shape[1])
+
+
 def _decoder(P, conv6_1, conv5_1, conv4_1, conv3_1, conv2, be):
-    flow6 = be.predict_flow(conv6_1, P, "Convolution1")
-    c5 = _refine_stage(P, conv5_1, conv6_1, "deconv5", flow6, "upsample_flow6to5", be)
-    flow5 = be.predict_flow(c5, P, "Convolution2")
-    c4 = _refine_stage(P, conv4_1, c5, "deconv4", flow5, "upsample_flow5to4", be)
-    flow4 = be.predict_flow(c4, P, "Convolution3")
-    c3 = _refine_stage(P, conv3_1, c4, "deconv3", flow4, "upsample_flow4to3", be)
-    flow3 = be.predict_flow(c3, P, "Convolution4")
-    c2 = _refine_stage(P, conv2, c3, "deconv2", flow3, "upsample_flow3to2", be)
+    flow6, up = _head_into_stage(P, conv6_1, "Convolution1", conv5_1, "deconv5", "upsample_flow6to5", be)
+    c5 = _refine_stage(P, conv5_1, conv6_1, "deconv5", flow6, "upsample_flow6to5", be, up)
+    flow5, up = _head_into_stage(P, c5, "Convolution2", conv4_1, "deconv4", "upsample_flow5to4", be)
+    c4 = _refine_stage(P, conv4_1, c5, "deconv4", flow5, "upsample_flow5to4", be, up)
+    flow4, up = _head_into_stage(P, c4, "Convolution3", conv3_1, "deconv3", "upsample_flow4to3", be)
+    c3 = _refine_stage(P, conv3_1, c4, "deconv3", flow4, "upsample_flow4to3", be, up)
+    flow3, up = _head_into_stage(P, c3, "Convolution4", conv2, "deconv2", "upsample_flow3to2", be)
+    c2 = _refine_stage(P, conv2, c3, "deconv2", flow3, "upsample_flow3to2", be, up)
     flow2 = be.predict_flow(c2, P, "Convolution5")
     return {2: flow2, 3: flow3, 4: flow4, 5: flow5, 6: flow6}
 
diff --git a/flownet2_amd/ops.py b/flownet2_amd/ops.py
--- a/flownet2_amd/ops.py
+++ b/flownet2_amd/ops.py
@@ -638,6 +638,26 @@
     out = torch.empty((N, 2, 2 * H, 2 * W), device=x.device, dtype=torch.float32)
     check(_lib.lib().fn2_upsample_flow_deconv_forward(_ptr(x), _ptr(w), _ptr(b), _ptr(out), N, H, W, _stream()))
     return out
+
+
+def predict_upsample_flow_forward(x, weight, bias, up_weight, up_bias, out, out_c0):
+    x, w, uw = _chk(x, "bottom[0]"), _chk(weight, "weight"), _chk(up_weight, "upsample weight")
+    N, Cc, H, W = x.shape
+    if tuple(w.shape) != (2, Cc, 3, 3) or tuple(uw.shape) != (2, 2, 4, 4):
+        raise ValueError(f"predict_upsample_flow: weights must be [2,{Cc},3,3] and [2,2,4,4], got {tuple(w.shape)} and {tuple(uw.shape)}")
+    _chk(out, "top[0]")
+    if out.shape[0] != N or tuple(out.shape[2:]) != (2 * H, 2 * W):
+        raise ValueError(f"predict_upsample_flow: top blob {tuple(out.shape)} does not match [{N},*,{2 * H},{2 * W}]")
+    if not _lib.lib().fn2_predict_upsample_flow_supported(N, Cc, H, W):
+        return None
+    b = _chk(bias, "bias", ndim=1) if bias is not None else None
+    ub = _chk(up_bias, "upsample bias", ndim=1) if up_bias is not None else None
+    flow = torch.empty((N, 2, H, W), device=x.device, dtype=torch.float32)
+    nbytes = _lib.lib().fn2_predict_flow_conv_workspace_bytes(N, Cc, H, W)
+    ws = torch.empty(nbytes, dtype=torch.uint8, device=x.device) if nbytes else None
+    check(_lib.lib().fn2_predict_upsample_flow_forward_into(_ptr(x), _ptr(w), _ptr(b), _ptr(flow), _ptr(uw), _ptr(ub), _ptr(out), N, Cc, H, W,
+                                                            out.shape[1], int(out_c0), _ptr(ws), nbytes, _stream()))
+    return flow
 
 
 def bias_leaky_relu_(x, bias=None, negative_slope=0.1):
diff --git a/include/flownet2_hip_flow_head.h b/include/flownet2_hip_flow_head.h
--- /dev/null
+++ b/include/flownet2_hip_flow_head.h
@@ -0,0 +1,13 @@
+#pragma once
+#include "flownet2_hip.h"
+#ifdef __cplusplus
+extern "C" {
+#endif
+int fn2_predict_upsample_flow_supported(int N, int C, int H, int W);
+int fn2_predict_upsample_flow_forward_into(const float* in, const float* weight, const float* bias, float* flow,
+                                           const float* up_weight, const float* up_bias, float* top,
+                                           int N, int C, int H, int W, int top_channels, int top_c0,
+                                           void* workspace, size_t workspace_bytes, void* stream);
+#ifdef __cplusplus
+}
+#endif
```

Result: faster. 3662 (median of 6 runs) (+1.8%).
